# 1275468127/Medical-SAM2

Measured on AMD Instinct MI355X. Metric: slices/sec @1024^2 (Hiera-S), higher is better.
Workload: dtype bf16; 1 GPU; configs[1]: sam2_hiera_s 2D (train_2d SAM2 sub-sequence, forward), b=4 x 1024x1024 per GPU, 16-entry memory bank with 4 sampled memories per slice, one click per slice; forward_image -> memory_attention -> prompt encoder -> mask decoder -> memory encoder; hip_graph=True, weights=random name-keyed init

## Files before the change

include/msam2_hip.h:

```cpp
#ifndef MSAM2_HIP_H
#define MSAM2_HIP_H

#include <stddef.h>
#include <stdint.h>

#ifdef __cplusplus
extern "C" {
#endif

const char* msam2_last_error(void);

int msam2_version(void);

int msam2_operand_is_fp16(void);

int msam2_graph_begin(void* stream);

int msam2_graph_end(void* stream, void** graph_exec_out);

int msam2_graph_launch(void* graph_exec, void* stream);

int msam2_graph_destroy(void* graph_exec);

int msam2_event_create(void** ev);

int msam2_event_record(void* ev, void* stream);

int msam2_event_elapsed_ms(void* start, void* stop, float* ms);

int msam2_event_destroy(void* ev);

int msam2_gemm_nt(const void* A, int64_t lda, const void* B, int64_t ldb, const float* bias, const void* residual, int64_t ldr, void* C, int64_t ldc, int out_is_16bit, int64_t M, int64_t N, int64_t K, void* stream);

int msam2_gemm(const void* A, int64_t lda, const void* W, int64_t ldw, const float* bias, const float* colscale, const void* residual, int64_t ldr, int res_is_16bit, int64_t res_mod, void* C, int64_t ldc, int out_is_16bit, int64_t M, int64_t N, int64_t K, int act, void* stream);

int msam2_gemm_tokens(const float* A, int64_t lda, const float* A2, int64_t add_cols, const void* W, int64_t ldw, const float* bias, const float* residual, int64_t ldr, void* C, int64_t ldc, int out_is_16bit, int64_t M, int64_t N, int64_t K, int act, void* stream);

int msam2_gemm_pool2x2(const void* A, int64_t lda, const void* W, int64_t ldw, const float* bias, float* C, int64_t ldc, int64_t B, int64_t H, int64_t Wimg, int64_t N, int64_t K, void* stream);

int msam2_gemm_qkv_pool2x2(const void* A, int64_t lda, const void* W, int64_t ldw, const float* bias, void* QKV, int64_t ldc, void* Q2, int64_t ldq, int64_t B, int64_t H, int64_t Wimg, int64_t N, int64_t K, int64_t q_cols, void* stream);

int msam2_gemm_rope(const void* A, int64_t lda, const void* W, int64_t ldw, const float* bias, void* C, int64_t ldc, int64_t M, int64_t N, int64_t K, const float* rope_cos, const float* rope_sin, int64_t rope_cols, int64_t head_dim, int64_t rows_per_batch, int64_t n_rope, int64_t n_pos, void* stream);

int msam2_gemm_residual_layernorm_supported(int64_t N, int64_t K);

int msam2_gemm_residual_layernorm(const void* A, int64_t lda, const void* W, int64_t ldw, const float* bias, const float* R32, int64_t ldr, float* C32, int64_t ldc, const float* ln_w, const float* ln_b, float eps, void* Y16, int64_t ldy, int64_t M, int64_t N, int64_t K, void* stream);

size_t msam2_attention_workspace_bytes(int64_t Bz, int64_t H, int64_t Lq, int64_t D, int splits);

int msam2_attention_merge(void* o, const int64_t* o_strides, int64_t B, int64_t H, int64_t Lq, int64_t Lk, int64_t D, int splits, void* workspace, size_t workspace_bytes, void* stream);

int msam2_attention_fwd(const void* q, const int64_t* q_strides, const void* k, const int64_t* k_strides, const void* v, const int64_t* v_strides, void* o, const int64_t* o_strides, int64_t B, int64_t H, int64_t Lq, int64_t Lk, int64_t D, float scale, int splits, void* workspace, size_t workspace_bytes, void* stream);

int msam2_attention_fwd_lse(const void* q, const int64_t* q_strides, const void* k, const int64_t* k_strides, const void* v, const int64_t* v_strides, void* o, const int64_t* o_strides, int64_t B, int64_t H, int64_t Lq, int64_t Lk, int64_t D, float scale, int splits, void* workspace, size_t workspace_bytes, float* lse, void* stream);

int msam2_attention_fwd_lse_dropout(const void* q, const int64_t* q_strides, const void* k, const int64_t* k_strides, const void* v, const int64_t* v_strides, void* o, const int64_t* o_strides, int64_t B, int64_t H, int64_t Lq, int64_t Lk, int64_t D, float scale, int splits, void* workspace, size_t workspace_bytes, float* lse, float p, uint64_t seed, uint64_t offset, const void* seed_dev, void* stream);

int msam2_attention_kv64_fwd(const void* q, const int64_t* q_strides, const void* k, const int64_t* k_strides, const void* v, const int64_t* v_strides, void* o, const int64_t* o_strides, int64_t B, int64_t H, int64_t Lq, int64_t Lk, float scale, int splits, void* workspace, size_t workspace_bytes, void* stream);

int msam2_attention_effective_splits(int64_t Lk, int splits);

int msam2_attention_kv64_partial(const void* q, const int64_t* q_strides, const void* k, const int64_t* k_strides, const void* v, const int64_t* v_strides, int64_t B, int64_t H, int64_t Lq, int64_t Lk, float scale, int splits, int split_begin, int split_count, void* workspace, size_t workspace_bytes, void* stream);

int msam2_attention_kv64_dyn_fwd(const void* q, const int64_t* q_strides, const void* k, const int64_t* k_strides, const void* v, const int64_t* v_strides, void* o, const int64_t* o_strides, int64_t B, int64_t H, int64_t Lq, int64_t Lk, const void* key_count_dev, float scale, int splits, void* workspace, size_t workspace_bytes, void* stream);

int msam2_attention_kv64_dyn_partial(const void* q, const int64_t* q_strides, const void* k, const int64_t* k_strides, const void* v, const int64_t* v_strides, int64_t B, int64_t H, int64_t Lq, int64_t Lk, const void* key_count_dev, float scale, int splits, int split_begin, int split_count, void* workspace, size_t workspace_bytes, void* stream);

int msam2_window_attention_fwd(const void* q, int64_t q_token_stride, int64_t q_head_stride, int64_t hq, int64_t wq, int64_t ws_q, const void* k, const void* v, int64_t kv_token_stride, int64_t kv_head_stride, int64_t hk, int64_t wk, int64_t ws_k, const float* kpad, const float* vpad, void* o, int64_t o_token_stride, int64_t o_head_stride, int64_t B, int64_t H, int64_t D, float scale, void* stream);

int msam2_attention_small_fwd(const void* q, int64_t q_bs, int64_t q_ts, const void* k, int64_t k_bs, int64_t k_ts, const void* v, int64_t v_bs, int64_t v_ts, void* o, int64_t o_bs, int64_t o_ts, int64_t B, int64_t H, int64_t Lq, int64_t Lk, int64_t D, float scale, void* stream);

int msam2_window_qkv_attention_supported(int64_t dim, int64_t dim_out, int64_t heads, int64_t ws, int pool, int64_t H, int64_t W);

int msam2_window_qkv_attention_fwd(const void* xn, const void* w, const float* bias, void* o, int64_t B, int64_t H, int64_t W, int64_t dim, int64_t heads, int64_t ws, int pool, float scale, void* stream);

size_t msam2_attention_bwd_workspace_bytes(int64_t B, int64_t H, int64_t Lq, int64_t D);

int msam2_attention_bwd(const void* q, const int64_t* q_strides, const void* k, const int64_t* k_strides, const void* v, const int64_t* v_strides, const void* o, const int64_t* o_strides, const float* lse, const float* d_o, const int64_t* do_strides, float* dq, const int64_t* dq_strides, float* dk, const int64_t* dk_strides, float* dv, const int64_t* dv_strides, void* workspace, size_t workspace_bytes, int64_t B, int64_t H, int64_t Lq, int64_t Lk, int64_t D, float scale, void* stream);

int msam2_attention_bwd_dropout(const void* q, const int64_t* q_strides, const void* k, const int64_t* k_strides, const void* v, const int64_t* v_strides, const void* o, const int64_t* o_strides, const float* lse, const float* d_o, const int64_t* do_strides, float* dq, const int64_t* dq_strides, float* dk, const int64_t* dk_strides, float* dv, const int64_t* dv_strides, void* workspace, size_t workspace_bytes, int64_t B, int64_t H, int64_t Lq, int64_t Lk, int64_t D, float scale, float p, uint64_t seed, uint64_t offset, const void* seed_dev, void* stream);

int msam2_layernorm(const void* x, int in_is_16bit, int64_t ldx, const float* weight, const float* bias, void* y, int out_is_16bit, int64_t ldy, int64_t rows, int64_t C, float eps, int act, void* stream);

int msam2_layernorm_dual(const float* x, int64_t ldx, const float* weight, const float* bias, float* y, int64_t ldy, void* y16, int64_t ldy16, int64_t rows, int64_t C, float eps, void* stream);

int msam2_add_cast(const void* a, int a_is_16bit, int64_t a_s0, int64_t a_s1, const void* b, int b_is_16bit, int64_t b_s0, int64_t b_s1, float alpha, void* out, int out_is_16bit, int64_t D0, int64_t D1, int64_t C, void* stream);

int msam2_maxpool2x2(const void* x, int in_is_16bit, int64_t ldx, void* y, int out_is_16bit, int64_t ldy, int64_t B, int64_t H, int64_t W, int64_t C, void* stream);

int msam2_upsample2x_add(void* y, const void* top, int64_t B, int64_t H, int64_t W, int64_t C, void* stream);

int msam2_rope_table(float* cos_out, float* sin_out, int64_t side, int64_t D, float theta, void* stream);

int msam2_rope_inplace(void* x, int64_t batch_stride, int64_t ld, int64_t B, int64_t L, int64_t n_rope, int64_t n_pos, int64_t D, const float* cos_t, const float* sin_t, void* stream);

int msam2_bilinear_upsample(const float* x, float* y, int64_t planes, int64_t h, int64_t w, int64_t H, int64_t W, void* stream);

int msam2_sine_pos_2d(float* out, int64_t h, int64_t w, int64_t C, float temperature, void* stream);

int msam2_fourier_pe_grid(float* out, const float* gauss, int64_t h, int64_t w, int64_t C, void* stream);

int msam2_hiera_pos_embed(float* out, const float* pos_embed, const float* pos_embed_window, int64_t C, int64_t bh, int64_t bw, int64_t h, int64_t w, int64_t window, void* stream);

int msam2_aa_downsample(const float* x, float* y, int64_t planes, int64_t H, int64_t W, int64_t factor, float in_scale, float in_bias, void* stream);

int msam2_gate_rows(float* x, const float* score, float value, int64_t B, int64_t row_len, void* stream);

int msam2_any_positive(const float* x, float* out, int64_t B, int64_t row_len, void* stream);

int msam2_image_prep(const uint8_t* img_hwc, float* out_chw, int64_t H, int64_t W, int64_t S, const float* mean3, const float* std3, void* stream);

int msam2_non_overlap(const float* masks, float* out, int64_t n_obj, int64_t pixels, void* stream);

int msam2_seg_counts(const float* pred, const float* gt, const float* thresholds, int64_t n_thresholds, int64_t planes, int64_t pixels, int* counts, void* stream);

int msam2_im2col_patch7x7s4(const float* img, void* out, int64_t B, int64_t S, void* stream);

int msam2_patch_embed7x7s4(const float* img, const void* w_perm, const float* bias, const float* pos, float* out, int64_t B, int64_t S, int64_t E, void* stream);

int msam2_im2col3x3s2(const void* x, void* out, int64_t B, int64_t H, int64_t W, int64_t C, int64_t ld, void* stream);

int msam2_conv3x3s2_ln_gelu(const void* x, int in_is_16bit, const float* weight, const float* bias, const float* ln_w, const float* ln_b, void* y, int64_t B, int64_t H, int64_t W, int64_t Cin, int64_t Cout, int mask_mode, float mask_scale, float mask_bias, void* stream);

int msam2_dwconv7x7_ln(const float* x, const float* weight_tap_major, const float* bias, const float* ln_w, const float* ln_b, void* y, int64_t B, int64_t H, int64_t W, int64_t C, void* stream);

int msam2_convt2x2_shuffle(const void* gemm_out, const float* bias, const void* skip, const float* ln_w, const float* ln_b, void* y, int64_t B, int64_t h, int64_t w, int64_t C, void* stream);

int msam2_convt2x2_shuffle_f32skip(const void* gemm_out, const float* bias, const float* skip, const float* ln_w, const float* ln_b, void* y, int64_t B, int64_t h, int64_t w, int64_t C, void* stream);

int msam2_convt2x2_shuffle_shared(const void* gemm_out, const float* bias, const void* skip, int skip_is_16bit, const float* ln_w, const float* ln_b, void* y, int64_t B, int64_t h, int64_t w, int64_t C, int64_t skip_batch_stride, void* stream);

int msam2_hyper_masks(const float* hyper, const void* upscaled, float* masks, int64_t n, int64_t K, int64_t P, int64_t C, void* stream);

int msam2_prompt_points(const float* xy, const int* labels, const float* gauss, const float* point_emb, const float* not_a_point, float* out, int64_t n_points, int64_t C, float image_size, void* stream);

int msam2_prompt_points_padded(const float* xy, const int* labels, const float* gauss, const float* point_emb, const float* not_a_point, float* out, int64_t n_sets, int64_t P, int64_t n_pad, int64_t C, float image_size, void* stream);

int msam2_select_mask(const float* masks, const float* ious, const float* obj_scores, float* low_res, int* sel, float* iou_sel, int64_t n, int64_t P, int multimask, int dynamic_stability, float delta, float thresh, void* stream);

int msam2_gather_rows(const float* x, const int* sel, float* y, int64_t n, int64_t T, int64_t C, int64_t offset, void* stream);

int msam2_obj_ptr_mix(float* ptr, const float* obj_scores, const float* no_obj_ptr, int64_t n, int64_t C, void* stream);

int msam2_space_to_depth(const void* x, int in_is_16bit, void* out, int64_t B, int64_t H, int64_t W, int64_t C, int64_t k, int64_t ld, void* stream);

int msam2_token_mlp3(const float* hs, int64_t hs_batch_stride, int64_t hs_token_stride, const int* token_index, const void* w1, const float* b1, const void* w2, const float* b2, const void* w3, const float* b3, const int* out_dim, const int* sigmoid_flag, float* out, int64_t G, int64_t B, int64_t C, void* stream);

int msam2_token_mlp3_packed(const float* hs, int64_t hs_batch_stride, int64_t hs_token_stride, const int* token_index, const void* w1, const float* b1, const void* w2, const float* b2, const void* w3, const float* b3, const int* out_dim, const int* sigmoid_flag, float* out, const int* out_offset, const int* out_stride, int64_t G, int64_t B, int64_t C, void* stream);

int msam2_conv3x3s2_mfma_ln_gelu_supported(int64_t cin, int64_t cout);

int msam2_conv3x3s2_mfma_ln_gelu(const void* x, const void* w_packed, int64_t ldw, const float* bias, const float* ln_w, const float* ln_b, float eps, void* y, int64_t ldy, int64_t B, int64_t H, int64_t W, int64_t cin, int64_t cout, void* stream);

size_t msam2_cc_workspace_bytes(int64_t N, int64_t H, int64_t W);

int msam2_cc_label(const uint8_t* img, int32_t* labels, int32_t* counts, int64_t N, int64_t H, int64_t W, void* workspace, size_t workspace_bytes, void* stream);

size_t msam2_fill_holes_workspace_bytes(int64_t N, int64_t H, int64_t W);

int msam2_fill_components(float* mask, int64_t N, int64_t H, int64_t W, int max_area, float threshold, int above, float fill_value, void* workspace, size_t workspace_bytes, void* stream);

int msam2_fill_holes(float* mask, int64_t N, int64_t H, int64_t W, int max_area, void* workspace, size_t workspace_bytes, void* stream);

int msam2_transpose16(const void* in, int64_t ldi, void* out, int64_t ldo, int64_t rows, int64_t cols, void* stream);

int msam2_gemm_tt(const void* A, int64_t lda, const void* B, int64_t ldb, float* C, int64_t ldc, float* a_colsum, int64_t M, int64_t N, int64_t K, void* stream);

int msam2_gemm_tt_acc(const void* A, int64_t lda, const void* B, int64_t ldb, float* C, int64_t ldc, float* a_colsum, int64_t M, int64_t N, int64_t K, void* stream);

int msam2_colsum(const void* x, int x_is_16bit, int64_t ldx, float* out, int64_t rows, int64_t cols, void* stream);

int msam2_act_bwd(const void* pre, int pre_is_16bit, const void* dy, int dy_is_16bit, void* out, int64_t n, int act, void* stream);

int msam2_layernorm_bwd(const float* x, int64_t ldx, const void* dy, int dy_is_16bit, int64_t ldd, const float* gamma, float* dx, int64_t ldo, float* dgamma, float* dbeta, int64_t rows, int64_t C, float eps, const float* add, int64_t ld_add, void* stream);

int msam2_softmax_rows(const float* s, int64_t ld_s, void* p, int64_t ld_p, int64_t rows, int64_t cols, float scale, void* stream);

int msam2_softmax_bwd_rows(const void* p, int64_t ld_p, const float* dp, int64_t ld_dp, void* ds, int64_t ld_ds, int64_t rows, int64_t cols, float scale, void* stream);

int msam2_convt2x2_gather(const void* gemm_out, const float* bias, const void* skip, float* z, int64_t B, int64_t h, int64_t w, int64_t C, void* stream);

int msam2_convt2x2_scatter_grad(const void* dz, int dz_is_16bit, void* dg, int64_t B, int64_t h, int64_t w, int64_t C, void* stream);

int msam2_dwconv7x7(const float* x, const float* w_tap_major, const float* bias, float* y, int64_t B, int64_t H, int64_t W, int64_t C, int flip, void* stream);

int msam2_dwconv7x7_wgrad(const float* x, const float* dy, float* dw_tap_major, int64_t B, int64_t H, int64_t W, int64_t C, void* stream);

int msam2_col2im3x3s2(const float* dcols, int64_t ld, float* dx, int64_t B, int64_t H, int64_t W, int64_t C, void* stream);

int msam2_bilinear_upsample_bwd(const float* dy, float* dx, int64_t planes, int64_t h, int64_t w, int64_t H, int64_t W, void* stream);

int msam2_bce_logits(const float* logits, const float* target, float* dlogits, float* loss, int64_t n, float pos_weight, void* stream);

int msam2_adam_step(float* param, const float* grad, float* exp_avg, float* exp_avg_sq, int64_t n, float lr, float beta1, float beta2, float eps, int64_t step, void* stream);

int msam2_adam_step_multi(void* const* params, const void* const* grads, void* const* exp_avg, void* const* exp_avg_sq, const int64_t* numel, int64_t count, float lr, float beta1, float beta2, float eps, int64_t step, float grad_scale, float weight_decay, void* step_counter, void* skipped_counter, void* stream);

int msam2_attention_small_bwd(const void* q, int64_t q_bs, int64_t q_ts, const void* k, int64_t k_bs, int64_t k_ts, const void* v, int64_t v_bs, int64_t v_ts, const float* d_o, float* dq, float* dk, float* dv, int64_t B, int64_t H, int64_t Lq, int64_t Lk, int64_t D, float scale, void* stream);

int msam2_maxpool2x2_bwd(const void* x, int x_is_16bit, int64_t ldx, const float* dy, int64_t lddy, float* dx, int64_t lddx, int64_t B, int64_t H, int64_t W, int64_t C, void* stream);

int msam2_window_move(void* img, int64_t ld_img, void* win, const void* fill, int64_t B, int64_t H, int64_t W, int64_t heads, int64_t D, int64_t ws, int elem_bytes, int to_windows, void* stream);

int msam2_window_unpartition_cvt(void* img16, int64_t ld_img, const float* win, int64_t B, int64_t H, int64_t W, int64_t heads, int64_t D, int64_t ws, void* stream);

int msam2_window_pad_colsum(const float* win, float* out, int64_t B, int64_t H, int64_t W, int64_t heads, int64_t D, int64_t ws, void* stream);

int msam2_sumpool2x2(const float* dy, float* out, int64_t B, int64_t H, int64_t W, int64_t C, void* stream);

size_t msam2_hiera_pos_embed_bwd_workspace_bytes(int64_t C, int64_t bw, int64_t h, int64_t window);

int msam2_hiera_pos_embed_bwd(const float* d_table, float* d_pos_embed, float* d_pos_embed_window, int64_t C, int64_t bh, int64_t bw, int64_t h, int64_t w, int64_t window, void* workspace, size_t workspace_bytes, void* stream);

int msam2_dropout(const void* x, int x_is_16bit, int64_t ldx, const float* residual, int64_t ldr, void* y, int y_is_16bit, int64_t ldy, int64_t rows, int64_t cols, float p, uint64_t seed, uint64_t offset, const void* seed_dev, void* stream);

int msam2_counter_bump(void* counter_u64, void* snapshot_u64, void* stream);

int msam2_mlp_fused_permute_w2(const void* w2, void* w2p, int64_t dim, int64_t hidden, void* stream);

int msam2_ln_mlp_residual_supported(int64_t dim);

int msam2_ln_mlp_residual_fwd(const float* x, int64_t T, int64_t dim, const float* ln_w, const float* ln_b, float eps, const void* w1, const float* b1, const void* w2p, const float* b2, float* out, void* stream);

int msam2_ln_mlp_residual_fwd_dual(const float* x, int64_t T, int64_t dim, const float* ln_w, const float* ln_b, float eps, const void* w1, const float* b1, const void* w2p, const float* b2, float* out, void* out16, void* stream);

int msam2_proj_ln_mlp_residual_supported(int64_t dim);

int msam2_mlp_fused_permute_w1(const void* w1, void* w1p, int64_t hidden, int64_t dim, void* stream);

int msam2_proj_ln_mlp_residual_fwd(const void* o, const void* wp, const float* bp, const float* res, int64_t T, int64_t dim, const float* ln_w, const float* ln_b, float eps, const void* w1p, const float* b1, const void* w2p, const float* b2, float* out, void* out16, const float* nln_w, const float* nln_b, float neps, void* xn16, void* stream);

size_t msam2_mask_stats_workspace_bytes(int64_t M);

int msam2_mask_stats(const float* logits, int64_t M, int64_t lh, int64_t lw, int64_t h, int64_t w, float thr, float thr_hi, float thr_lo, int* counts, int* boxes, void* workspace, size_t workspace_bytes, void* stream);

int msam2_mask_rle_runs(const float* logits, int64_t M, int64_t lh, int64_t lw, int64_t h, int64_t w, int64_t x0, int64_t y0, int64_t H, int64_t W, float thr, int* runs, void* stream);

int msam2_mask_rle(const float* logits, int64_t M, int64_t lh, int64_t lw, int64_t h, int64_t w, int64_t x0, int64_t y0, int64_t H, int64_t W, float thr, const int64_t* offsets, int* counts, void* stream);

size_t msam2_box_nms_workspace_bytes(int64_t K);

int msam2_box_nms(const float* boxes, const float* scores, int64_t K, float iou_thr, int64_t* keep, int* n_keep, void* workspace, size_t workspace_bytes, void* stream);

int msam2_bank_dots_chain(int64_t K, int vec);

size_t msam2_bank_dots_workspace_bytes(int64_t R, int64_t Cn);

int msam2_bank_dots(const float* x, const int64_t* x_strides, int64_t R, const float* ya, const int64_t* ya_strides, int64_t rows_a, const float* yb, const int64_t* yb_strides, int64_t rows_b, int64_t n_ch, int64_t n_px, float* dots, float* xx, float* yy, void* workspace, size_t workspace_bytes, void* stream);

int msam2_bank_sample(const float* dots, int64_t ld, const float* xx, const float* yy, const int* order, int64_t N, int64_t cap, const float* u, int64_t B, int64_t S, int* indices, float* probs, void* stream);

int msam2_bank_gather(const float* feats, const float* pos, const int* order, const int* indices, int64_t B, int64_t S, int64_t HW, int64_t C, int64_t N, int64_t cap, float* memory, float* memory_pos, void* stream);

int msam2_bank_decide(float* gram, float* iou_bank, int* order, int64_t N, int64_t cap, const float* dots, const float* iou_pred, int64_t B, int64_t M, int fill, int* accept, int* slot_cand, float* iou_out, void* stream);

int msam2_bank_commit(const int* slot_cand, int64_t cap, const float* feats, const int64_t* feats_strides, const float* pos, const int64_t* pos_strides, int64_t C, const float* embed, const int64_t* embed_strides, int64_t Ce, int64_t HW, int64_t B, float* feats_store, float* pos_store, float* embed_store, void* stream);

int msam2_label_slices(const float* logits, const uint8_t* ids, int64_t T, int64_t n, int64_t lh, int64_t lw, int64_t H, int64_t W, float label_thr, const float* thresholds, int64_t K, const uint8_t* gt, int exclusive, uint8_t* labels, int* counts, void* stream);

int msam2_label_stats(const uint8_t* labels, const uint8_t* ids, int64_t D, int64_t H, int64_t W, int64_t n, int* stats, int* rows, void* stream);

int msam2_label_pick(const uint8_t* labels, const uint8_t* ids, const int* stats, const int* rows, const int* k, const uint32_t* u, int64_t D, int64_t H, int64_t W, int64_t n, int* xy, void* stream);

size_t msam2_label_components_workspace_bytes(int64_t D, int64_t H, int64_t W);

int msam2_label_components(const uint8_t* labels, int64_t D, int64_t H, int64_t W, int connectivity, int32_t* comp, int32_t* size, void* workspace, size_t workspace_bytes, void* stream);

size_t msam2_label_clean_workspace_bytes(int64_t n);

int msam2_label_clean(const uint8_t* labels, const int32_t* comp, const int32_t* size, const uint8_t* ids, int64_t n, const int32_t* min_voxels, uint32_t largest_mask, uint8_t* out, int32_t* info, void* workspace, size_t workspace_bytes, int64_t D, int64_t H, int64_t W, void* stream);

int msam2_label_overlap(const uint8_t* pred, const uint8_t* gt, const uint8_t* ids, int64_t D, int64_t H, int64_t W, int64_t n, int32_t* counts, void* stream);

size_t msam2_label_fill_holes_workspace_bytes(int64_t D, int64_t H, int64_t W, const int32_t* boxes, int64_t n, int connectivity, int in_place, int all_at_once);

int msam2_label_fill_holes(const uint8_t* labels, int64_t D, int64_t H, int64_t W, const uint8_t* ids, const int32_t* boxes, int64_t n, int connectivity, const int32_t* max_voxels, int claim, uint8_t* out, int32_t* info, void* workspace, size_t workspace_bytes, void* stream);

size_t msam2_label_edt_workspace_bytes(int64_t bd, int64_t bh, int64_t bw);

int msam2_label_edt(const uint8_t* labels, int64_t D, int64_t H, int64_t W, int value, int features, const int32_t* box, double sz, double sy, double sx, double* d2, void* workspace, size_t workspace_bytes, void* stream);

size_t msam2_label_surface_distances_workspace_bytes(const int32_t* boxes, int64_t n);

int msam2_label_surface_distances(const uint8_t* pred, const uint8_t* gt, int64_t D, int64_t H, int64_t W, const uint8_t* ids, const int32_t* boxes, const int64_t* seg_offsets, const int32_t* capacity, int64_t n, double sz, double sy, double sx, double* dist, int64_t dist_len, int32_t* counts, void* workspace, size_t workspace_bytes, void* stream);

size_t msam2_label_morph_workspace_bytes(int64_t D, int64_t H, int64_t W, const int32_t* boxes, int64_t n, int op, const double* r2, double sz, double sy, double sx, int in_place, int all_at_once);

int msam2_label_morph(const uint8_t* labels, int64_t D, int64_t H, int64_t W, const uint8_t* values, const int32_t* boxes, int64_t n, int op, const double* r2, double sz, double sy, double sx, int claim, uint8_t* out, int32_t* info, void* workspace, size_t workspace_bytes, void* stream);

size_t msam2_label_error_clicks_workspace_bytes(int64_t D, int64_t H, int64_t W, int64_t n, int mode);

int msam2_label_error_clicks(const uint8_t* pred, const uint8_t* gt, const uint8_t* ids, const int* k, const uint32_t* u, int64_t D, int64_t H, int64_t W, int64_t n, int mode, int* clicks, void* workspace, size_t workspace_bytes, void* stream);

size_t msam2_volume_prep_workspace_bytes(int64_t T, int64_t H0, int64_t W0, int64_t S);

int msam2_volume_prep(const void* src, int src_type, int64_t T, int64_t Cin, int64_t H0, int64_t W0, int64_t S, const double* windows, const int* kx, const int* bx, int64_t ksize_x, const int* ky, const int* by, int64_t ksize_y, const float* mean3, const float* std3, uint8_t* grey_out, float* out, void* workspace, size_t workspace_bytes, void* stream);

int msam2_label_resize(const void* src, int src_type, int64_t T, int64_t H0, int64_t W0, int64_t S, const int* ymap, const int* xmap, const uint32_t* keep8, uint8_t* out, void* stream);

#ifdef __cplusplus
}
#endif
#endif
```

medical-sam2_amd/_lib.py:

```python
from __future__ import annotations

import ctypes
import os
import subprocess

_HERE = os.path.dirname(os.path.abspath(__file__))
LIB_PATH = os.environ.get("MSAM2_LIB_PATH") or os.path.join(_HERE, "libmsam2_hip.so")

c_p = ctypes.c_void_p
c_i = ctypes.c_int
c_l = ctypes.c_int64
c_f = ctypes.c_float
c_z = ctypes.c_size_t
c_d = ctypes.c_double

SIGNATURES = {
    "msam2_version": (c_i, []),
    "msam2_last_error": (ctypes.c_char_p, []),
    "msam2_operand_is_fp16": (c_i, []),
    "msam2_gemm": (c_i, [c_p, c_l, c_p, c_l, c_p, c_p, c_p, c_l, c_i, c_l, c_p, c_l, c_i, c_l, c_l, c_l, c_i, c_p]),
    "msam2_gemm_pool2x2": (c_i, [c_p, c_l, c_p, c_l, c_p, c_p, c_l, c_l, c_l, c_l, c_l, c_l, c_p]),
    "msam2_gemm_qkv_pool2x2": (c_i, [c_p, c_l, c_p, c_l, c_p, c_p, c_l, c_p, c_l, c_l, c_l, c_l, c_l, c_l, c_l, c_p]),
    "msam2_gemm_tokens": (c_i, [c_p, c_l, c_p, c_l, c_p, c_l, c_p, c_p, c_l, c_p, c_l, c_i, c_l, c_l, c_l, c_i, c_p]),
    "msam2_gemm_rope": (c_i, [c_p, c_l, c_p, c_l, c_p, c_p, c_l, c_l, c_l, c_l, c_p, c_p, c_l, c_l, c_l, c_l, c_l, c_p]),
    "msam2_gemm_residual_layernorm_supported": (c_i, [c_l, c_l]),
    "msam2_gemm_residual_layernorm": (c_i, [c_p, c_l, c_p, c_l, c_p, c_p, c_l, c_p, c_l, c_p, c_p, c_f, c_p, c_l, c_l, c_l, c_l, c_p]),
    "msam2_ln_mlp_residual_supported": (c_i, [c_l]),
    "msam2_mlp_fused_permute_w2": (c_i, [c_p, c_p, c_l, c_l, c_p]),
    "msam2_ln_mlp_residual_fwd": (c_i, [c_p, c_l, c_l, c_p, c_p, c_f, c_p, c_p, c_p, c_p, c_p, c_p]),
    "msam2_ln_mlp_residual_fwd_dual": (c_i, [c_p, c_l, c_l, c_p, c_p, c_f, c_p, c_p, c_p, c_p, c_p, c_p, c_p]),
    "msam2_proj_ln_mlp_residual_supported": (c_i, [c_l]),
    "msam2_mlp_fused_permute_w1": (c_i, [c_p, c_p, c_l, c_l, c_p]),
    "msam2_proj_ln_mlp_residual_fwd": (c_i, [c_p, c_p, c_p, c_p, c_l, c_l, c_p, c_p, c_f, c_p, c_p, c_p, c_p, c_p, c_p, c_p, c_p, c_f, c_p, c_p]),
    "msam2_layernorm": (c_i, [c_p, c_i, c_l, c_p, c_p, c_p, c_i, c_l, c_l, c_l, c_f, c_i, c_p]),
    "msam2_layernorm_dual": (c_i, [c_p, c_l, c_p, c_p, c_p, c_l, c_p, c_l, c_l, c_l, c_f, c_p]),
    "msam2_attention_workspace_bytes": (c_z, [c_l, c_l, c_l, c_l, c_i]),
    "msam2_attention_fwd": (c_i, [c_p, c_p, c_p, c_p, c_p, c_p, c_p, c_p, c_l, c_l, c_l, c_l, c_l, c_f, c_i, c_p, c_z, c_p]),
    "msam2_attention_fwd_lse": (c_i, [c_p, c_p, c_p, c_p, c_p, c_p, c_p, c_p, c_l, c_l, c_l, c_l, c_l, c_f, c_i, c_p, c_z, c_p, c_p]),
    "msam2_attention_fwd_lse_dropout": (c_i, [c_p, c_p, c_p, c_p, c_p, c_p, c_p, c_p, c_l, c_l, c_l, c_l, c_l, c_f, c_i, c_p, c_z, c_p, c_f,
                                              ctypes.c_uint64, ctypes.c_uint64, c_p, c_p]),
    "msam2_attention_kv64_fwd": (c_i, [c_p, c_p, c_p, c_p, c_p, c_p, c_p, c_p, c_l, c_l, c_l, c_l, c_f, c_i, c_p, c_z, c_p]),
    "msam2_attention_kv64_partial": (c_i, [c_p, c_p, c_p, c_p, c_p, c_p, c_l, c_l, c_l, c_l, c_f, c_i, c_i, c_i, c_p, c_z, c_p]),
    "msam2_attention_kv64_dyn_fwd": (c_i, [c_p, c_p, c_p, c_p, c_p, c_p, c_p, c_p, c_l, c_l, c_l, c_l, c_p, c_f, c_i, c_p, c_z, c_p]),
    "msam2_attention_kv64_dyn_partial": (c_i, [c_p, c_p, c_p, c_p, c_p, c_p, c_l, c_l, c_l, c_l, c_p, c_f, c_i, c_i, c_i, c_p, c_z, c_p]),
    "msam2_attention_effective_splits": (c_i, [c_l, c_i]),
    "msam2_attention_merge": (c_i, [c_p, c_p, c_l, c_l, c_l, c_l, c_l, c_i, c_p, c_z, c_p]),
    "msam2_window_attention_fwd": (c_i, [c_p, c_l, c_l, c_l, c_l, c_l, c_p, c_p, c_l, c_l, c_l, c_l, c_l, c_p, c_p, c_p, c_l, c_l,
                                         c_l, c_l, c_l, c_f, c_p]),
    "msam2_window_qkv_attention_supported": (c_i, [c_l, c_l, c_l, c_l, c_i, c_l, c_l]),
    "msam2_window_qkv_attention_fwd": (c_i, [c_p, c_p, c_p, c_p, c_l, c_l, c_l, c_l, c_l, c_l, c_i, c_f, c_p]),
    "msam2_attention_small_fwd": (c_i, [c_p, c_l, c_l, c_p, c_l, c_l, c_p, c_l, c_l, c_p, c_l, c_l, c_l, c_l, c_l, c_l, c_l, c_f,
                                        c_p]),
    "msam2_add_cast": (c_i, [c_p, c_i, c_l, c_l, c_p, c_i, c_l, c_l, c_f, c_p, c_i, c_l, c_l, c_l, c_p]),
    "msam2_maxpool2x2": (c_i, [c_p, c_i, c_l, c_p, c_i, c_l, c_l, c_l, c_l, c_l, c_p]),
    "msam2_upsample2x_add": (c_i, [c_p, c_p, c_l, c_l, c_l, c_l, c_p]),
    "msam2_rope_table": (c_i, [c_p, c_p, c_l, c_l, c_f, c_p]),
    "msam2_rope_inplace": (c_i, [c_p, c_l, c_l, c_l, c_l, c_l, c_l, c_l, c_p, c_p, c_p]),
    "msam2_bilinear_upsample": (c_i, [c_p, c_p, c_l, c_l, c_l, c_l, c_l, c_p]),
    "msam2_sine_pos_2d": (c_i, [c_p, c_l, c_l, c_l, c_f, c_p]),
    "msam2_fourier_pe_grid": (c_i, [c_p, c_p, c_l, c_l, c_l, c_p]),
    "msam2_hiera_pos_embed": (c_i, [c_p, c_p, c_p, c_l, c_l, c_l, c_l, c_l, c_l, c_p]),
    "msam2_im2col_patch7x7s4": (c_i, [c_p, c_p, c_l, c_l, c_p]),
    "msam2_patch_embed7x7s4": (c_i, [c_p, c_p, c_p, c_p, c_p, c_l, c_l, c_l, c_p]),
    "msam2_im2col3x3s2": (c_i, [c_p, c_p, c_l, c_l, c_l, c_l, c_l, c_p]),
    "msam2_conv3x3s2_ln_gelu": (c_i, [c_p, c_i, c_p, c_p, c_p, c_p, c_p, c_l, c_l, c_l, c_l, c_l, c_i, c_f, c_f, c_p]),
    "msam2_conv3x3s2_mfma_ln_gelu_supported": (c_i, [c_l, c_l]),
    "msam2_conv3x3s2_mfma_ln_gelu": (c_i, [c_p, c_p, c_l, c_p, c_p, c_p, c_f, c_p, c_l, c_l, c_l, c_l, c_l, c_l, c_p]),
    "msam2_dwconv7x7_ln": (c_i, [c_p, c_p, c_p, c_p, c_p, c_p, c_l, c_l, c_l, c_l, c_p]),
    "msam2_convt2x2_shuffle": (c_i, [c_p, c_p, c_p, c_p, c_p, c_p, c_l, c_l, c_l, c_l, c_p]),
    "msam2_convt2x2_shuffle_f32skip": (c_i, [c_p, c_p, c_p, c_p, c_p, c_p, c_l, c_l, c_l, c_l, c_p]),
    "msam2_space_to_depth": (c_i, [c_p, c_i, c_p, c_l, c_l, c_l, c_l, c_l, c_l, c_p]),
    "msam2_aa_downsample": (c_i, [c_p, c_p, c_l, c_l, c_l, c_l, c_f, c_f, c_p]),
    "msam2_gate_rows": (c_i, [c_p, c_p, c_f, c_l, c_l, c_p]),
    "msam2_any_positive": (c_i, [c_p, c_p, c_l, c_l, c_p]),
    "msam2_transpose16": (c_i, [c_p, c_l, c_p, c_l, c_l, c_l, c_p]),
    "msam2_colsum": (c_i, [c_p, c_i, c_l, c_p, c_l, c_l, c_p]),
    "msam2_act_bwd": (c_i, [c_p, c_i, c_p, c_i, c_p, c_l, c_i, c_p]),
    "msam2_layernorm_bwd": (c_i, [c_p, c_l, c_p, c_i, c_l, c_p, c_p, c_l, c_p, c_p, c_l, c_l, c_f, c_p, c_l, c_p]),
    "msam2_softmax_rows": (c_i, [c_p, c_l, c_p, c_l, c_l, c_l, c_f, c_p]),
    "msam2_softmax_bwd_rows": (c_i, [c_p, c_l, c_p, c_l, c_p, c_l, c_l, c_l, c_f, c_p]),
    "msam2_convt2x2_gather": (c_i, [c_p, c_p, c_p, c_p, c_l, c_l, c_l, c_l, c_p]),
    "msam2_convt2x2_scatter_grad": (c_i, [c_p, c_i, c_p, c_l, c_l, c_l, c_l, c_p]),
    "msam2_bce_logits": (c_i, [c_p, c_p, c_p, c_p, c_l, c_f, c_p]),
    "msam2_attention_bwd_workspace_bytes": (c_z, [c_l, c_l, c_l, c_l]),
    "msam2_attention_bwd": (c_i, [c_p, c_p, c_p, c_p, c_p, c_p, c_p, c_p, c_p, c_p, c_p, c_p, c_p, c_p, c_p, c_p, c_p, c_p, c_z,
                                  c_l, c_l, c_l, c_l, c_l, c_f, c_p]),
    "msam2_attention_bwd_dropout": (c_i, [c_p, c_p, c_p, c_p, c_p, c_p, c_p, c_p, c_p, c_p, c_p, c_p, c_p, c_p, c_p, c_p, c_p, c_p, c_z,
                                          c_l, c_l, c_l, c_l, c_l, c_f, c_f, ctypes.c_uint64, ctypes.c_uint64, c_p, c_p]),
    "msam2_dwconv7x7": (c_i, [c_p, c_p, c_p, c_p, c_l, c_l, c_l, c_l, c_i, c_p]),
    "msam2_dwconv7x7_wgrad": (c_i, [c_p, c_p, c_p, c_l, c_l, c_l, c_l, c_p]),
    "msam2_col2im3x3s2": (c_i, [c_p, c_l, c_p, c_l, c_l, c_l, c_l, c_p]),
    "msam2_gemm_nt": (c_i, [c_p, c_l, c_p, c_l, c_p, c_p, c_l, c_p, c_l, c_i, c_l, c_l, c_l, c_p]),
    "msam2_gemm_tt": (c_i, [c_p, c_l, c_p, c_l, c_p, c_l, c_p, c_l, c_l, c_l, c_p]),
    "msam2_window_unpartition_cvt": (c_i, [c_p, c_l, c_p, c_l, c_l, c_l, c_l, c_l, c_l, c_p]),
    "msam2_window_pad_colsum": (c_i, [c_p, c_p, c_l, c_l, c_l, c_l, c_l, c_l, c_p]),
    "msam2_gemm_tt_acc": (c_i, [c_p, c_l, c_p, c_l, c_p, c_l, c_p, c_l, c_l, c_l, c_p]),
    "msam2_bilinear_upsample_bwd": (c_i, [c_p, c_p, c_l, c_l, c_l, c_l, c_l, c_p]),
    "msam2_maxpool2x2_bwd": (c_i, [c_p, c_i, c_l, c_p, c_l, c_p, c_l, c_l, c_l, c_l, c_l, c_p]),
    "msam2_window_move": (c_i, [c_p, c_l, c_p, c_p, c_l, c_l, c_l, c_l, c_l, c_l, c_i, c_i, c_p]),
    "msam2_sumpool2x2": (c_i, [c_p, c_p, c_l, c_l, c_l, c_l, c_p]),
    "msam2_hiera_pos_embed_bwd": (c_i, [c_p, c_p, c_p, c_l, c_l, c_l, c_l, c_l, c_l, c_p, c_z, c_p]),
    "msam2_hiera_pos_embed_bwd_workspace_bytes": (c_z, [c_l, c_l, c_l, c_l]),
    "msam2_dropout": (c_i, [c_p, c_i, c_l, c_p, c_l, c_p, c_i, c_l, c_l, c_l, c_f, ctypes.c_uint64, ctypes.c_uint64, c_p, c_p]),
    "msam2_counter_bump": (c_i, [c_p, c_p, c_p]),
    "msam2_adam_step": (c_i, [c_p, c_p, c_p, c_p, c_l, c_f, c_f, c_f, c_f, c_l, c_p]),
    "msam2_adam_step_multi": (c_i, [c_p, c_p, c_p, c_p, c_p, c_l, c_f, c_f, c_f, c_f, c_l, c_f, c_f, c_p, c_p, c_p]),
    "msam2_attention_small_bwd": (c_i, [c_p, c_l, c_l, c_p, c_l, c_l, c_p, c_l, c_l, c_p, c_p, c_p, c_p, c_l, c_l, c_l, c_l, c_l, c_f, c_p]),
    "msam2_seg_counts": (c_i, [c_p, c_p, c_p, c_l, c_l, c_l, c_p, c_p]),
    "msam2_non_overlap": (c_i, [c_p, c_p, c_l, c_l, c_p]),
    "msam2_token_mlp3": (c_i, [c_p, c_l, c_l, c_p, c_p, c_p, c_p, c_p, c_p, c_p, c_p, c_p, c_p, c_l, c_l, c_l, c_p]),
    "msam2_hyper_masks": (c_i, [c_p, c_p, c_p, c_l, c_l, c_l, c_l, c_p]),
    "msam2_prompt_points": (c_i, [c_p, c_p, c_p, c_p, c_p, c_p, c_l, c_l, c_f, c_p]),
    "msam2_prompt_points_padded": (c_i, [c_p, c_p, c_p, c_p, c_p, c_p, c_l, c_l, c_l, c_l, c_f, c_p]),
    "msam2_token_mlp3_packed": (c_i, [c_p, c_l, c_l, c_p, c_p, c_p, c_p, c_p, c_p, c_p, c_p, c_p, c_p, c_p, c_p, c_l, c_l, c_l, c_p]),
    "msam2_select_mask": (c_i, [c_p, c_p, c_p, c_p, c_p, c_p, c_l, c_l, c_i, c_i, c_f, c_f, c_p]),
    "msam2_gather_rows": (c_i, [c_p, c_p, c_p, c_l, c_l, c_l, c_l, c_p]),
    "msam2_obj_ptr_mix": (c_i, [c_p, c_p, c_p, c_l, c_l, c_p]),
    "msam2_convt2x2_shuffle_shared": (c_i, [c_p, c_p, c_p, c_i, c_p, c_p, c_p, c_l, c_l, c_l, c_l, c_l, c_p]),
    "msam2_mask_stats_workspace_bytes": (c_z, [c_l]),
    "msam2_mask_stats": (c_i, [c_p, c_l, c_l, c_l, c_l, c_l, c_f, c_f, c_f, c_p, c_p, c_p, c_z, c_p]),
    "msam2_mask_rle_runs": (c_i, [c_p, c_l, c_l, c_l, c_l, c_l, c_l, c_l, c_l, c_l, c_f, c_p, c_p]),
    "msam2_mask_rle": (c_i, [c_p, c_l, c_l, c_l, c_l, c_l, c_l, c_l, c_l, c_l, c_f, c_p, c_p, c_p]),
    "msam2_box_nms_workspace_bytes": (c_z, [c_l]),
    "msam2_box_nms": (c_i, [c_p, c_p, c_l, c_f, c_p, c_p, c_p, c_z, c_p]),
    "msam2_bank_dots_chain": (c_i, [c_l, c_i]),
    "msam2_bank_dots_workspace_bytes": (c_z, [c_l, c_l]),
    "msam2_bank_dots": (c_i, [c_p, c_p, c_l, c_p, c_p, c_l, c_p, c_p, c_l, c_l, c_l, c_p, c_p, c_p, c_p, c_z, c_p]),
    "msam2_bank_sample": (c_i, [c_p, c_l, c_p, c_p, c_p, c_l, c_l, c_p, c_l, c_l, c_p, c_p, c_p]),
    "msam2_bank_gather": (c_i, [c_p, c_p, c_p, c_p, c_l, c_l, c_l, c_l, c_l, c_l, c_p, c_p, c_p]),
    "msam2_bank_decide": (c_i, [c_p, c_p, c_p, c_l, c_l, c_p, c_p, c_l, c_l, c_i, c_p, c_p, c_p, c_p]),
    "msam2_bank_commit": (c_i, [c_p, c_l, c_p, c_p, c_p, c_p, c_l, c_p, c_p, c_l, c_l, c_l, c_p, c_p, c_p, c_p]),
    "msam2_label_slices": (c_i, [c_p, c_p, c_l, c_l, c_l, c_l, c_l, c_l, c_f, c_p, c_l, c_p, c_i, c_p, c_p, c_p]),
    "msam2_label_stats": (c_i, [c_p, c_p, c_l, c_l, c_l, c_l, c_p, c_p, c_p]),
    "msam2_label_pick": (c_i, [c_p, c_p, c_p, c_p, c_p, c_p, c_l, c_l, c_l, c_l, c_p, c_p]),
    "msam2_label_components_workspace_bytes": (c_z, [c_l, c_l, c_l]),
    "msam2_label_components": (c_i, [c_p, c_l, c_l, c_l, c_i, c_p, c_p, c_p, c_z, c_p]),
    "msam2_label_clean_workspace_bytes": (c_z, [c_l]),
    "msam2_label_clean": (c_i, [c_p, c_p, c_p, c_p, c_l, c_p, ctypes.c_uint32, c_p, c_p, c_p, c_z, c_l, c_l, c_l, c_p]),
    "msam2_label_overlap": (c_i, [c_p, c_p, c_p, c_l, c_l, c_l, c_l, c_p, c_p]),
    "msam2_label_fill_holes_workspace_bytes": (c_z, [c_l, c_l, c_l, c_p, c_l, c_i, c_i, c_i]),
    "msam2_label_fill_holes": (c_i, [c_p, c_l, c_l, c_l, c_p, c_p, c_l, c_i, c_p, c_i, c_p, c_p, c_p, c_z, c_p]),
    "msam2_label_edt_workspace_bytes": (c_z, [c_l, c_l, c_l]),
    "msam2_label_edt": (c_i, [c_p, c_l, c_l, c_l, c_i, c_i, c_p, c_d, c_d, c_d, c_p, c_p, c_z, c_p]),
    "msam2_label_surface_distances_workspace_bytes": (c_z, [c_p, c_l]),
    "msam2_label_surface_distances": (c_i, [c_p, c_p, c_l, c_l, c_l, c_p, c_p, c_p, c_p, c_l, c_d, c_d, c_d, c_p, c_l, c_p, c_p, c_z, c_p]),
    "msam2_label_morph_workspace_bytes": (c_z, [c_l, c_l, c_l, c_p, c_l, c_i, c_p, c_d, c_d, c_d, c_i, c_i]),
    "msam2_label_morph": (c_i, [c_p, c_l, c_l, c_l, c_p, c_p, c_l, c_i, c_p, c_d, c_d, c_d, c_i, c_p, c_p, c_p, c_z, c_p]),
    "msam2_label_error_clicks_workspace_bytes": (c_z, [c_l, c_l, c_l, c_l, c_i]),
    "msam2_label_error_clicks": (c_i, [c_p, c_p, c_p, c_p, c_p, c_l, c_l, c_l, c_l, c_i, c_p, c_p, c_z, c_p]),
    "msam2_volume_prep_workspace_bytes": (c_z, [c_l, c_l, c_l, c_l]),
    "msam2_volume_prep": (c_i, [c_p, c_i, c_l, c_l, c_l, c_l, c_l, ctypes.POINTER(c_d), c_p, c_p, c_l, c_p, c_p, c_l, ctypes.POINTER(c_f),
                                ctypes.POINTER(c_f), c_p, c_p, c_p, c_z, c_p]),
    "msam2_label_resize": (c_i, [c_p, c_i, c_l, c_l, c_l, c_l, c_p, c_p, ctypes.POINTER(ctypes.c_uint32), c_p, c_p]),
    "msam2_cc_workspace_bytes": (c_z, [c_l, c_l, c_l]),
    "msam2_cc_label": (c_i, [c_p, c_p, c_p, c_l, c_l, c_l, c_p, c_z, c_p]),
    "msam2_fill_holes_workspace_bytes": (c_z, [c_l, c_l, c_l]),
    "msam2_fill_holes": (c_i, [c_p, c_l, c_l, c_l, c_i, c_p, c_z, c_p]),
    "msam2_fill_components": (c_i, [c_p, c_l, c_l, c_l, c_i, c_f, c_i, c_f, c_p, c_z, c_p]),
    "msam2_image_prep": (c_i, [c_p, c_p, c_l, c_l, c_l, ctypes.POINTER(c_f), ctypes.POINTER(c_f), c_p]),
    "msam2_graph_begin": (c_i, [c_p]),
    "msam2_graph_end": (c_i, [c_p, ctypes.POINTER(c_p)]),
    "msam2_graph_launch": (c_i, [c_p, c_p]),
    "msam2_graph_destroy": (c_i, [c_p]),
    "msam2_event_create": (c_i, [ctypes.POINTER(c_p)]),
    "msam2_event_record": (c_i, [c_p, c_p]),
    "msam2_event_elapsed_ms": (c_i, [c_p, c_p, ctypes.POINTER(c_f)]),
    "msam2_event_destroy": (c_i, [c_p]),
}


def build(force: bool = False) -> str:
    if force and os.path.exists(LIB_PATH):
        os.remove(LIB_PATH)
    subprocess.check_call(["make", "-s", "-C", os.path.join(_HERE, "csrc")])
    return LIB_PATH


_lib = None


def lib() -> ctypes.CDLL:
    global _lib
    if _lib is None:
        if not os.path.exists(LIB_PATH):
            raise RuntimeError(
                f"{LIB_PATH} is missing: the MI355X HIP library is the only compute path of this package. "
                "Build it with `python -c 'import __graft_entry__ as g; g.build()'` (or `make -C medical-sam2_amd/csrc`).")
        L = ctypes.CDLL(LIB_PATH)
        for name, (res, args) in SIGNATURES.items():
            fn = getattr(L, name)
            fn.restype = res
            fn.argtypes = args
        _lib = L
    return _lib


class Msam2Error(RuntimeError):
    pass


def check(rc: int) -> None:
    if rc != 0:
        raise Msam2Error(lib().msam2_last_error().decode())
```

medical-sam2_amd/csrc/attention.hip:

```cpp
#include "common.h"
#ifdef MSAM2_STAMP
__device__ unsigned long long g_stamp[16];
__device__ unsigned long long g_wgtime[4096][4];
#define STAMP(var)                                                                     \
  do {                                                                                 \
    __builtin_amdgcn_sched_barrier(0);                                                 \
    asm volatile("s_memtime %0\n\ts_waitcnt lgkmcnt(0)" : "=s"(var)::"memory");         \
    __builtin_amdgcn_sched_barrier(0);                                                 \
  } while (0)
#define STAMP_DECL unsigned long long t0_ = 0, t1_ = 0, t2_ = 0, t3_ = 0, t4_ = 0, t5_ = 0, acc_[5] = {0, 0, 0, 0, 0}
#else
#define STAMP(var)
#define STAMP_DECL
#endif
#include <stdlib.h>
#include <type_traits>

#ifndef MSAM2_RESCALE_SLACK
#define MSAM2_RESCALE_SLACK 8.f
#endif

struct AttnParams {
  const op16 *q, *k, *v;
  op16* o;
// ... 1859 lines not shown
  MSAM2_REQUIRE(splits >= 1 && splits <= 64, "attention_kv64: bad split count %d", splits);
  for (int i = 0; i < 3; ++i)
    MSAM2_REQUIRE(q_strides[i] % 8 == 0 && k_strides[i] % 8 == 0 && v_strides[i] % 8 == 0 && (!o || o_strides[i] % 4 == 0),
                  "attention_kv64: strides must keep 16-byte row alignment");
  MSAM2_REQUIRE(Lk * k_strides[2] * 2 < (1ll << 31) && Lk * v_strides[2] * 2 < (1ll << 31), "attention_kv64: key range beyond the 2 GiB buffer window");
  const int eff = attn_effective_splits(Lk, splits);
  if (split_cnt >= 0) {
    MSAM2_REQUIRE(eff == splits && eff > 1, "attention_kv64_partial: pass msam2_attention_effective_splits(Lk, splits) (> 1) as the split count");
    MSAM2_REQUIRE(split_begin >= 0 && split_cnt >= 0 && split_begin + split_cnt <= eff, "attention_kv64_partial: bad split range");
    defer = true;
    if (split_cnt == 0) return MSAM2_OK;
  } else {
    split_begin = 0;
    split_cnt = eff;
  }
  splits = eff;
  MSAM2_REQUIRE(workspace_bytes >= msam2_attention_workspace_bytes(B, H, Lq, 64, splits), "attention_kv64: workspace too small");
  MSAM2_REQUIRE(!defer || splits > 1, "attention_kv64: a deferred merge needs an effective split count > 1");
  MSAM2_REQUIRE(splits == 1 || workspace, "attention_kv64: split-KV needs a workspace");
  AttnParams p = {};
  set_qkvo(p, q, q_strides, k, k_strides, v, v_strides, o, o ? o_strides : nullptr);
  p.B = (int)B; p.H = (int)H; p.Lq = (int)Lq; p.Lk = (int)Lk;
  p.scale_log2 = scale * 1.4426950408889634f;
  set_workspace(p, workspace, splits, B, H, Lq, 64);
  p.split_begin = split_begin;
  p.split_cnt = split_cnt;
  p.lk_dev = lk_dev;
  p.defer_merge = defer ? 1 : 0;
  return launch_attn_kv64(p, (int)B, (hipStream_t)stream);
}

extern "C" int msam2_attention_kv64_fwd(const void* q, const int64_t* q_strides, const void* k, const int64_t* k_strides,
                                        const void* v, const int64_t* v_strides, void* o, const int64_t* o_strides, int64_t B,
                                        int64_t H, int64_t Lq, int64_t Lk, float scale, int splits, void* workspace,
                                        size_t workspace_bytes, void* stream) {
  MSAM2_REQUIRE(o, "attention_kv64: null output");
  return attention_kv64_impl(q, q_strides, k, k_strides, v, v_strides, o, o_strides, B, H, Lq, Lk, scale, splits, 0, -1, workspace, workspace_bytes, stream);
}

extern "C" int msam2_attention_effective_splits(int64_t Lk, int splits) {
  parse_splits(splits);
  return attn_effective_splits(Lk, splits);
}

extern "C" int msam2_attention_kv64_partial(const void* q, const int64_t* q_strides, const void* k, const int64_t* k_strides,
                                            const void* v, const int64_t* v_strides, int64_t B, int64_t H, int64_t Lq, int64_t Lk,
                                            float scale, int splits, int split_begin, int split_count, void* workspace,
                                            size_t workspace_bytes, void* stream) {
  MSAM2_REQUIRE(split_count >= 0, "attention_kv64_partial: negative split count");
  return attention_kv64_impl(q, q_strides, k, k_strides, v, v_strides, nullptr, nullptr, B, H, Lq, Lk, scale, splits, split_begin, split_count,
                             workspace, workspace_bytes, stream);
}

extern "C" int msam2_attention_kv64_dyn_fwd(const void* q, const int64_t* q_strides, const void* k, const int64_t* k_strides,
                                            const void* v, const int64_t* v_strides, void* o, const int64_t* o_strides, int64_t B,
                                            int64_t H, int64_t Lq, int64_t Lk, const void* key_count_dev, float scale, int splits,
                                            void* workspace, size_t workspace_bytes, void* stream) {
  MSAM2_REQUIRE(o && key_count_dev, "attention_kv64_dyn: null output / key count");
  return attention_kv64_impl(q, q_strides, k, k_strides, v, v_strides, o, o_strides, B, H, Lq, Lk, scale, splits, 0, -1, workspace, workspace_bytes,
                             stream, (const int*)key_count_dev);
}

extern "C" int msam2_attention_kv64_dyn_partial(const void* q, const int64_t* q_strides, const void* k, const int64_t* k_strides,
                                                const void* v, const int64_t* v_strides, int64_t B, int64_t H, int64_t Lq, int64_t Lk,
                                                const void* key_count_dev, float scale, int splits, int split_begin, int split_count,
                                                void* workspace, size_t workspace_bytes, void* stream) {
  MSAM2_REQUIRE(split_count >= 0 && key_count_dev, "attention_kv64_dyn_partial: negative split count / null key count");
  return attention_kv64_impl(q, q_strides, k, k_strides, v, v_strides, nullptr, nullptr, B, H, Lq, Lk, scale, splits, split_begin, split_count,
                             workspace, workspace_bytes, stream, (const int*)key_count_dev);
}

extern "C" int msam2_window_attention_fwd(const void* q, int64_t q_token_stride, int64_t q_head_stride, int64_t hq, int64_t wq,
                                          int64_t ws_q, const void* k, const void* v, int64_t kv_token_stride,
                                          int64_t kv_head_stride, int64_t hk, int64_t wk, int64_t ws_k, const float* kpad,
                                          const float* vpad, void* o, int64_t o_token_stride, int64_t o_head_stride, int64_t B,
                                          int64_t H, int64_t D, float scale, void* stream) {
  MSAM2_REQUIRE(q && k && v && o && kpad && vpad, "window_attention: null tensor");
  MSAM2_REQUIRE(D == 96 || D == 64 || D == 128, "window_attention: head dim %lld not built", (long long)D);
  MSAM2_REQUIRE(ws_q > 0 && ws_k > 0 && hq > 0 && wq > 0 && hk > 0 && wk > 0, "window_attention: bad geometry");
  const int nwy = (int)((hk + ws_k - 1) / ws_k), nwx = (int)((wk + ws_k - 1) / ws_k);
  MSAM2_REQUIRE((hq + ws_q - 1) / ws_q == nwy && (wq + ws_q - 1) / ws_q == nwx, "window_attention: q/kv window grids differ");
  MSAM2_REQUIRE(q_token_stride % 8 == 0 && kv_token_stride % 8 == 0 && q_head_stride % 8 == 0 && kv_head_stride % 8 == 0 &&
                    o_token_stride % 4 == 0 && o_head_stride % 4 == 0, "window_attention: strides must keep 16-byte alignment");
  AttnParams p = {};
  p.q = (const op16*)q; p.k = (const op16*)k; p.v = (const op16*)v; p.o = (op16*)o;
  p.q_bs = hq * wq * q_token_stride; p.q_hs = q_head_stride; p.q_ts = q_token_stride;
  p.k_bs = hk * wk * kv_token_stride; p.k_hs = kv_head_stride; p.k_ts = kv_token_stride;
  p.v_bs = p.k_bs; p.v_hs = kv_head_stride; p.v_ts = kv_token_stride;
  p.o_bs = hq * wq * o_token_stride; p.o_hs = o_head_stride; p.o_ts = o_token_stride;
  p.B = (int)B; p.H = (int)H; p.Lq = (int)(ws_q * ws_q); p.Lk = (int)(ws_k * ws_k);
  p.scale_log2 = scale * 1.4426950408889634f;
  p.win = 1; p.ws_q = (int)ws_q; p.ws_k = (int)ws_k; p.hq = (int)hq; p.wq = (int)wq; p.hk = (int)hk; p.wk = (int)wk;
  p.nwy = nwy; p.nwx = nwx; p.kpad = kpad; p.vpad = vpad; p.splits = 1;
  hipStream_t s = (hipStream_t)stream;
  const int Bz = (int)B * nwy * nwx;
  switch (D) {
    case 96:
      if (attn_win_applies(p)) return launch_attn_win(p, Bz, s);
      return attn_tinywin_applies(p) ? launch_attn_tinywin(p, Bz, s) : dispatch_nw<96, true>(p, Bz, s);
    case 64: return dispatch_nw<64, true>(p, Bz, s);
    default: return dispatch_nw<128, true>(p, Bz, s);
  }
}

template <int D>
__global__ void attn_small_kernel(const op16* q, const op16* k, const op16* v, op16* o, int64_t q_bs, int64_t q_ts,
                                  int64_t k_bs, int64_t k_ts, int64_t v_bs, int64_t v_ts, int64_t o_bs, int64_t o_ts, int B,
                                  int H, int Lq, int Lk, float scale_log2) {
  const int64_t gw = ((int64_t)blockIdx.x * blockDim.x + threadIdx.x) >> 6;
  const int lane = threadIdx.x & 63;
  if (gw >= (int64_t)B * H * Lq) return;
  const int qi = gw % Lq;
  const int head = (gw / Lq) % H;
  const int b = gw / ((int64_t)Lq * H);
  float qv[D];
  const op16* qp = q + b * q_bs + (int64_t)qi * q_ts + head * D;
#pragma unroll
  for (int d = 0; d < D; d += 8) {
    const op16x8 t = *reinterpret_cast<const op16x8*>(qp + d);
#pragma unroll
    for (int e = 0; e < 8; ++e) qv[d + e] = op2f(t[e]) * scale_log2;
  }
  float m = -INFINITY, l = 0.f, acc[D];
#pragma unroll
  for (int d = 0; d < D; ++d) acc[d] = 0.f;
  for (int key = lane; key < Lk; key += 64) {
    const op16* kp = k + b * k_bs + (int64_t)key * k_ts + head * D;
    const op16* vp = v + b * v_bs + (int64_t)key * v_ts + head * D;
    float s = 0.f;
    float vv[D];
#pragma unroll
    for (int d = 0; d < D; d += 8) {
      const op16x8 t = *reinterpret_cast<const op16x8*>(kp + d);
      const op16x8 u = *reinterpret_cast<const op16x8*>(vp + d);
#pragma unroll
      for (int e = 0; e < 8; ++e) {
        s += qv[d + e] * op2f(t[e]);
        vv[d + e] = op2f(u[e]);
      }
    }
    const float mn = fmaxf(m, s);
    const float a = (m == -INFINITY) ? 0.f : __builtin_amdgcn_exp2f(m - mn);
    const float pe = __builtin_amdgcn_exp2f(s - mn);
    l = l * a + pe;
#pragma unroll
    for (int d = 0; d < D; ++d) acc[d] = acc[d] * a + pe * vv[d];
    m = mn;
  }
#pragma unroll
  for (int off = 32; off > 0; off >>= 1) {
    const float m2 = __shfl_xor(m, off, 64), l2 = __shfl_xor(l, off, 64);
    const float mn = fmaxf(m, m2);
    const float a1 = (m == -INFINITY) ? 0.f : __builtin_amdgcn_exp2f(m - mn);
    const float a2 = (m2 == -INFINITY) ? 0.f : __builtin_amdgcn_exp2f(m2 - mn);
    l = l * a1 + l2 * a2;
#pragma unroll
    for (int d = 0; d < D; ++d) acc[d] = acc[d] * a1 + __shfl_xor(acc[d], off, 64) * a2;
    m = mn;
  }
  if (lane == 0) {
    op16* op = o + b * o_bs + (int64_t)qi * o_ts + head * D;
    const float inv = 1.f / l;
#pragma unroll
    for (int d = 0; d < D; ++d) op[d] = f2op(acc[d] * inv);
  }
}

template <int D>
__global__ __launch_bounds__(1024) void attn_fewq_kernel(const op16* q, const op16* k, const op16* v, op16* o, int64_t q_bs, int64_t q_ts,
                                                         int64_t k_bs, int64_t k_ts, int64_t v_bs, int64_t v_ts, int64_t o_bs, int64_t o_ts,
                                                         int B, int H, int Lq, int Lk, float scale_log2) {
  __shared__ float part[16][D + 2];
  const int gw = blockIdx.x;
  const int lane = threadIdx.x & 63, wave = threadIdx.x >> 6;
  const int qi = gw % Lq;
  const int head = (gw / Lq) % H;
  const int b = gw / (Lq * H);
  float qv[D];
  const op16* qp = q + b * q_bs + (int64_t)qi * q_ts + head * D;
#pragma unroll
  for (int d = 0; d < D; d += 8) {
    const op16x8 t = *reinterpret_cast<const op16x8*>(qp + d);
#pragma unroll
    for (int e = 0; e < 8; ++e) qv[d + e] = op2f(t[e]) * scale_log2;
  }
  float m = -INFINITY, l = 0.f, acc[D];
#pragma unroll
  for (int d = 0; d < D; ++d) acc[d] = 0.f;
  const op16* kb = k + b * k_bs + head * D;
  const op16* vb = v + b * v_bs + head * D;
#pragma unroll 4
  for (int key = threadIdx.x; key < Lk; key += 1024) {
    const op16* kp = kb + (int64_t)key * k_ts;
    const op16* vp = vb + (int64_t)key * v_ts;
    float s = 0.f;
    float vv[D];
#pragma unroll
    for (int d = 0; d < D; d += 8) {
      const op16x8 t = *reinterpret_cast<const op16x8*>(kp + d);
      const op16x8 u = *reinterpret_cast<const op16x8*>(vp + d);
#pragma unroll
      for (int e = 0; e < 8; ++e) {
        s += qv[d + e] * op2f(t[e]);
        vv[d + e] = op2f(u[e]);
      }
    }
    const float mn = fmaxf(m, s);
    const float a = (m == -INFINITY) ? 0.f : __builtin_amdgcn_exp2f(m - mn);
    const float pe = __builtin_amdgcn_exp2f(s - mn);
    l = l * a + pe;
#pragma unroll
    for (int d = 0; d < D; ++d) acc[d] = acc[d] * a + pe * vv[d];
    m = mn;
  }
  auto merge = [&](int off) {
    const float m2 = __shfl_xor(m, off, 64), l2 = __shfl_xor(l, off, 64);
    const float mn = fmaxf(m, m2);
    const float a1 = (m == -INFINITY) ? 0.f : __builtin_amdgcn_exp2f(m - mn);
    const float a2 = (m2 == -INFINITY) ? 0.f : __builtin_amdgcn_exp2f(m2 - mn);
    l = l * a1 + l2 * a2;
#pragma unroll
    for (int d = 0; d < D; ++d) acc[d] = acc[d] * a1 + __shfl_xor(acc[d], off, 64) * a2;
    m = mn;
  };
#pragma unroll
  for (int off = 32; off > 0; off >>= 1) merge(off);
  if (lane == 0) {
    part[wave][0] = m;
    part[wave][1] = l;
#pragma unroll
    for (int d = 0; d < D; ++d) part[wave][2 + d] = acc[d];
  }
  __syncthreads();
  if (wave == 0) {
    const int w = lane & 15;
    m = part[w][0];
    l = part[w][1];
#pragma unroll
    for (int d = 0; d < D; ++d) acc[d] = part[w][2 + d];
#pragma unroll
    for (int off = 8; off > 0; off >>= 1) merge(off);
    if (lane == 0) {
      op16* op = o + b * o_bs + (int64_t)qi * o_ts + head * D;
      const float inv = 1.f / l;
#pragma unroll
      for (int d = 0; d < D; ++d) op[d] = f2op(acc[d] * inv);
    }
  }
}

template <int D>
__global__ void attn_fewkeys_kernel(const op16* q, const op16* k, const op16* v, op16* o, int64_t q_bs, int64_t q_ts, int64_t k_bs,
                                    int64_t k_ts, int64_t v_bs, int64_t v_ts, int64_t o_bs, int64_t o_ts, int B, int H, int Lq, int Lk,
                                    float scale_log2) {
  const int64_t gid = (int64_t)blockIdx.x * blockDim.x + threadIdx.x;
  if (gid >= (int64_t)B * H * Lq) return;
  const int head = gid % H;
  const int qi = (gid / H) % Lq;
  const int b = gid / ((int64_t)H * Lq);
  float qv[D];
  const op16* qp = q + b * q_bs + (int64_t)qi * q_ts + head * D;
#pragma unroll
  for (int d = 0; d < D; d += 8) {
    const op16x8 t = *reinterpret_cast<const op16x8*>(qp + d);
#pragma unroll
    for (int e = 0; e < 8; ++e) qv[d + e] = op2f(t[e]) * scale_log2;
  }
  float m = -INFINITY, l = 0.f, acc[D];
#pragma unroll
  for (int d = 0; d < D; ++d) acc[d] = 0.f;
  for (int key = 0; key < Lk; ++key) {
    const op16* kp = k + b * k_bs + (int64_t)key * k_ts + head * D;
    const op16* vp = v + b * v_bs + (int64_t)key * v_ts + head * D;
    float sc = 0.f;
#pragma unroll
    for (int d = 0; d < D; d += 8) {
      const op16x8 t = *reinterpret_cast<const op16x8*>(kp + d);
#pragma unroll
      for (int e = 0; e < 8; ++e) sc += qv[d + e] * op2f(t[e]);
    }
    const float mn = fmaxf(m, sc);
    const float al = (m == -INFINITY) ? 0.f : __builtin_amdgcn_exp2f(m - mn);
    const float pe = __builtin_amdgcn_exp2f(sc - mn);
    l = l * al + pe;
#pragma unroll
    for (int d = 0; d < D; d += 8) {
      const op16x8 u = *reinterpret_cast<const op16x8*>(vp + d);
#pragma unroll
      for (int e = 0; e < 8; ++e) acc[d + e] = acc[d + e] * al + pe * op2f(u[e]);
    }
    m = mn;
  }
  const float inv = 1.f / l;
  op16* op = o + b * o_bs + (int64_t)qi * o_ts + head * D;
#pragma unroll
  for (int d = 0; d < D; d += 8) {
    op16x8 w;
#pragma unroll
    for (int e = 0; e < 8; ++e) w[e] = f2op(acc[d + e] * inv);
    *reinterpret_cast<op16x8*>(op + d) = w;
  }
}

__global__ __launch_bounds__(1024) void attn_fewq16_kernel(const op16* __restrict__ q, const op16* __restrict__ k, const op16* __restrict__ v,
                                                           op16* __restrict__ o, int64_t q_bs, int64_t q_ts, int64_t k_bs, int64_t k_ts,
                                                           int64_t v_bs, int64_t v_ts, int64_t o_bs, int64_t o_ts, int H, int Lq, int Lk,
                                                           float scale_log2) {
  constexpr int D = 16, RB = 64, BK = 32, NW = 16, MAXS = 8;
  __shared__ __attribute__((aligned(16))) unsigned char vt[NW][BK * RB];
  __shared__ float part[NW][32][18];
  const int tid = threadIdx.x, wave = tid >> 6, lane = tid & 63;
  const int r = lane & 31, h = lane >> 5;
  const int b = blockIdx.x / H, head = blockIdx.x - b * H;
  const op16* qb = q + (int64_t)b * q_bs + head * D;
  const op16* kb = k + (int64_t)b * k_bs + head * D;
  const op16* vb = v + (int64_t)b * v_bs + head * D;
  {
    unsigned char* t = vt[wave];
    *reinterpret_cast<uint4*>(t + (lane >> 1) * RB + 32 + (lane & 1) * 16) = make_uint4(0, 0, 0, 0);
  }
  op16x8 qf;
  {
    uint4 t = make_uint4(0, 0, 0, 0);
    const uint4 ld = *reinterpret_cast<const uint4*>(qb + (int64_t)min(r, Lq - 1) * q_ts + h * 8);
    if (r < Lq) t = ld;
    qf = __builtin_bit_cast(op16x8, t);
  }
  const int per = (Lk + NW - 1) / NW;
  const int key_lo = wave * per, key_hi = min(Lk, key_lo + per);
  const int nsteps = max(0, (key_hi - key_lo + BK - 1) / BK);
  uint4 kfr[MAXS], vch[MAXS];
#pragma unroll
  for (int st = 0; st < MAXS; ++st) {
    const int kk = min(key_lo + st * BK + r, Lk - 1);
    kfr[st] = *reinterpret_cast<const uint4*>(kb + (int64_t)kk * k_ts + h * 8);
    const int kv = min(key_lo + st * BK + (lane >> 1), Lk - 1);
    vch[st] = *reinterpret_cast<const uint4*>(vb + (int64_t)kv * v_ts + (lane & 1) * 8);
  }
  f32x16 oacc;
#pragma unroll
  for (int e = 0; e < 16; ++e) oacc[e] = 0.f;
  float m_run = -INFINITY, l_run = 0.f;
  const int li = lane & 15;
  const int v_off = (4 * h + (li >> 2)) * RB + (16 * ((lane >> 4) & 1) + 4 * (li & 3)) * 2;
#pragma unroll
  for (int st = 0; st < MAXS; ++st) {
    if (st < nsteps) {
      const int key0 = key_lo + st * BK;
      *reinterpret_cast<uint4*>(vt[wave] + (lane >> 1) * RB + (lane & 1) * 16) = vch[st];
      f32x16 sacc;
#pragma unroll
      for (int e = 0; e < 16; ++e) sacc[e] = 0.f;
      sacc = MSAM2_MFMA_32x32x16(__builtin_bit_cast(op16x8, kfr[st]), qf, sacc, 0, 0, 0);
      float mx = -INFINITY;
#pragma unroll
      for (int e = 0; e < 16; ++e) {
        if (key0 + s_frag_key(e, h) >= key_hi) sacc[e] = -INFINITY;
        mx = fmaxf(mx, sacc[e]);
      }
      mx = half_max(mx) * scale_log2;
      const float m_new = fmaxf(m_run, mx);
      const float alpha = (m_run == -INFINITY) ? 0.f : __builtin_amdgcn_exp2f(m_run - m_new);
      l_run *= alpha;
#pragma unroll
      for (int e = 0; e < 16; ++e) oacc[e] *= alpha;
      m_run = m_new;
      float psum = 0.f;
      op16x8 pf[2];
#pragma unroll
      for (int e = 0; e < 16; ++e) {
        const float pe = __builtin_amdgcn_exp2f(__builtin_fmaf(sacc[e], scale_log2, -m_run));
        psum += pe;
        pf[e >> 3][e & 7] = f2op_fast(pe);
      }
      l_run += psum;
      asm volatile("s_waitcnt lgkmcnt(0)" ::: "memory");
#pragma unroll
      for (int s2 = 0; s2 < 2; ++s2)
        oacc = MSAM2_MFMA_32x32x16(lds_read_tr16_pair(vt[wave] + (16 * s2) * RB + v_off, 8 * RB), pf[s2], oacc, 0, 0, 0);
      asm volatile("s_waitcnt lgkmcnt(0)" ::: "memory");
    }
  }
  const float l_tot = half_sum(l_run);
  {
    float* pp = part[wave][r];
    if (h == 0) { pp[0] = m_run; pp[1] = l_tot; }
#pragma unroll
    for (int e = 0; e < 8; ++e) pp[2 + (e & 3) + 8 * (e >> 2) + 4 * h] = oacc[e];
  }
  __syncthreads();
  if (tid < Lq * D) {
    const int qi = tid / D, d = tid - qi * D;
    float M = -INFINITY;
#pragma unroll
    for (int w = 0; w < NW; ++w) M = fmaxf(M, part[w][qi][0]);
    float L = 0.f, acc = 0.f;
#pragma unroll
    for (int w = 0; w < NW; ++w) {
      const float mw = part[w][qi][0];
      const float wgt = (mw == -INFINITY) ? 0.f : __builtin_amdgcn_exp2f(mw - M);
      L += part[w][qi][1] * wgt;
      acc += part[w][qi][2 + d] * wgt;
    }
    o[(int64_t)b * o_bs + (int64_t)qi * o_ts + head * D + d] = f2op(acc / L);
  }
}


extern "C" int msam2_attention_small_fwd(const void* q, int64_t q_bs, int64_t q_ts, const void* k, int64_t k_bs, int64_t k_ts,
                                         const void* v, int64_t v_bs, int64_t v_ts, void* o, int64_t o_bs, int64_t o_ts,
                                         int64_t B, int64_t H, int64_t Lq, int64_t Lk, int64_t D, float scale, void* stream) {
  MSAM2_REQUIRE(q && k && v && o, "attention_small: null tensor");
  MSAM2_REQUIRE(D == 16 || D == 32, "attention_small: head dim %lld not built (16/32)", (long long)D);
  MSAM2_REQUIRE(B > 0 && H > 0 && Lq > 0 && Lk > 0, "attention_small: empty problem");
  MSAM2_REQUIRE(q_ts % 8 == 0 && k_ts % 8 == 0 && v_ts % 8 == 0 && q_bs % 8 == 0 && k_bs % 8 == 0 && v_bs % 8 == 0,
                "attention_small: strides must keep 16-byte alignment");
  const float sl = scale * 1.4426950408889634f;
  hipStream_t s = (hipStream_t)stream;
  if (Lk <= 32 && Lq >= 64 && o_ts % 8 == 0 && o_bs % 8 == 0) {
    dim3 g1(cdiv(B * H * Lq, 256));
    if (D == 16)
      hipLaunchKernelGGL((attn_fewkeys_kernel<16>), g1, dim3(256), 0, s, (const op16*)q, (const op16*)k, (const op16*)v, (op16*)o, q_bs,
                         q_ts, k_bs, k_ts, v_bs, v_ts, o_bs, o_ts, (int)B, (int)H, (int)Lq, (int)Lk, sl);
    else
      hipLaunchKernelGGL((attn_fewkeys_kernel<32>), g1, dim3(256), 0, s, (const op16*)q, (const op16*)k, (const op16*)v, (op16*)o, q_bs,
                         q_ts, k_bs, k_ts, v_bs, v_ts, o_bs, o_ts, (int)B, (int)H, (int)Lq, (int)Lk, sl);
    return msam2_check_launch("attention_small(fewkeys)");
  }
  {
    const char* off = getenv("MSAM2_NO_FEWQ16");
    if (D == 16 && Lq <= 32 && Lk >= 1024 && Lk <= 4096 && !(off && off[0] == '1') && q_ts % 8 == 0 && k_ts % 8 == 0 && v_ts % 8 == 0 &&
        q_bs % 8 == 0 && k_bs % 8 == 0 && v_bs % 8 == 0 && (((uintptr_t)q | (uintptr_t)k | (uintptr_t)v) & 15) == 0) {
      hipLaunchKernelGGL(attn_fewq16_kernel, dim3((unsigned)(B * H)), dim3(1024), 0, s, (const op16*)q, (const op16*)k, (const op16*)v, (op16*)o,
                         q_bs, q_ts, k_bs, k_ts, v_bs, v_ts, o_bs, o_ts, (int)H, (int)Lq, (int)Lk, sl);
      return msam2_check_launch("attention_small(fewq, matrix pipe)");
    }
  }
  if (Lk >= 1024 && B * H * Lq <= 4096) {
    dim3 g2((unsigned)(B * H * Lq));
    if (D == 16)
      hipLaunchKernelGGL((attn_fewq_kernel<16>), g2, dim3(1024), 0, s, (const op16*)q, (const op16*)k, (const op16*)v, (op16*)o, q_bs, q_ts,
                         k_bs, k_ts, v_bs, v_ts, o_bs, o_ts, (int)B, (int)H, (int)Lq, (int)Lk, sl);
    else
      hipLaunchKernelGGL((attn_fewq_kernel<32>), g2, dim3(1024), 0, s, (const op16*)q, (const op16*)k, (const op16*)v, (op16*)o, q_bs, q_ts,
                         k_bs, k_ts, v_bs, v_ts, o_bs, o_ts, (int)B, (int)H, (int)Lq, (int)Lk, sl);
    return msam2_check_launch("attention_small(fewq)");
  }
  const int64_t waves = B * H * Lq;
  dim3 grid(cdiv(waves * 64, 256));
  if (D == 16)
    hipLaunchKernelGGL((attn_small_kernel<16>), grid, dim3(256), 0, s, (const op16*)q, (const op16*)k, (const op16*)v, (op16*)o,
                       q_bs, q_ts, k_bs, k_ts, v_bs, v_ts, o_bs, o_ts, (int)B, (int)H, (int)Lq, (int)Lk, sl);
  else
    hipLaunchKernelGGL((attn_small_kernel<32>), grid, dim3(256), 0, s, (const op16*)q, (const op16*)k, (const op16*)v, (op16*)o,
                       q_bs, q_ts, k_bs, k_ts, v_bs, v_ts, o_bs, o_ts, (int)B, (int)H, (int)Lq, (int)Lk, sl);
  return msam2_check_launch("attention_small");
}
```

medical-sam2_amd/modeling/sam_heads.py:

```python
from __future__ import annotations

from typing import List, Optional, Tuple, Type

import torch
import torch.nn as nn

from .. import ops
from .common import OP16, F32, WeightCache, nchw_view, to_bf16, tokens_of, v_f32, w_bf16
from .encoder import MLP
from .memory import Attention, LayerNorm2d
from .position import PositionEmbeddingRandom


class PromptEncoder(nn.Module):

    def __init__(self, embed_dim: int, image_embedding_size: Tuple[int, int], input_image_size: Tuple[int, int],
                 mask_in_chans: int, activation: Type[nn.Module] = nn.GELU) -> None:
        super().__init__()
        self.embed_dim = embed_dim
        self.input_image_size = input_image_size
        self.image_embedding_size = image_embedding_size
        self.pe_layer = PositionEmbeddingRandom(embed_dim // 2)
        self.num_point_embeddings: int = 4
        self.point_embeddings = nn.ModuleList([nn.Embedding(1, embed_dim) for _ in range(self.num_point_embeddings)])
        self.not_a_point_embed = nn.Embedding(1, embed_dim)
        self.mask_input_size = (4 * image_embedding_size[0], 4 * image_embedding_size[1])
        self.mask_downscaling = nn.Sequential(
            nn.Conv2d(1, mask_in_chans // 4, kernel_size=2, stride=2), LayerNorm2d(mask_in_chans // 4), activation(),
            nn.Conv2d(mask_in_chans // 4, mask_in_chans, kernel_size=2, stride=2), LayerNorm2d(mask_in_chans), activation(),
            nn.Conv2d(mask_in_chans, embed_dim, kernel_size=1))
        self.no_mask_embed = nn.Embedding(1, embed_dim)
        self._wc = WeightCache()

    def dense_pe_tokens(self) -> torch.Tensor:
        g = self.pe_layer.positional_encoding_gaussian_matrix
        return self._wc.get("dense_pe", [g], lambda: self.pe_layer.grid_tokens(self.image_embedding_size))

    def get_dense_pe(self) -> torch.Tensor:
        h, w = self.image_embedding_size
        return nchw_view(self.dense_pe_tokens(), 1, h, w)

    def _points(self, xy: torch.Tensor, labels: torch.Tensor, n_pad: int = 0) -> torch.Tensor:
        assert self.input_image_size[0] == self.input_image_size[1]
        wc = self._wc
        emb = wc.get("pemb", [m.weight for m in self.point_embeddings],
                     lambda: torch.cat([m.weight.detach() for m in self.point_embeddings], 0).float().contiguous())
        return ops.prompt_points(xy.to(F32), labels.to(torch.int32), self.pe_layer.positional_encoding_gaussian_matrix.to(F32), emb,
                                 v_f32(wc, "nap", self.not_a_point_embed.weight), float(self.input_image_size[0]), n_pad=n_pad)

    def _embed_masks_tokens(self, masks: torch.Tensor) -> torch.Tensor:
        n, _, H, W = masks.shape
        wc, md = self._wc, self.mask_downscaling
        f = lambda key, p: v_f32(wc, key, p)

        def patch_w(conv, key):
            def build():
                w = conv.weight.detach().permute(0, 2, 3, 1).reshape(conv.weight.shape[0], -1)
                ld = (w.shape[1] + 7) // 8 * 8
                out = torch.zeros(w.shape[0], ld, dtype=OP16, device=w.device)
                out[:, : w.shape[1]] = w.to(OP16)
                return out
            return wc.get(key, [conv.weight], build)

        h = ops.space_to_depth(masks.to(F32).contiguous().reshape(n * H * W, 1), n, H, W, 2)
        h = ops.gemm(h, patch_w(md[0], "w0"), f("b0", md[0].bias), out_dtype=F32)
        h = ops.layernorm(h, f("lw0", md[1].weight), f("lb0", md[1].bias), md[1].eps, act=ops.ACT_GELU)
        h = ops.space_to_depth(h, n, H // 2, W // 2, 2)
        h = ops.gemm(h, patch_w(md[3], "w1"), f("b1", md[3].bias), out_dtype=F32)
        h = ops.layernorm(h, f("lw1", md[4].weight), f("lb1", md[4].bias), md[4].eps, act=ops.ACT_GELU)
        return ops.gemm(h, w_bf16(wc, "w2", md[6].weight), f("b2", md[6].bias), out_dtype=F32)

    def _get_batch_size(self, points, boxes, masks) -> int:
        if points is not None:
            return points[0].shape[0]
        if boxes is not None:
            return boxes.shape[0]
        if masks is not None:
            return masks.shape[0]
        return 1

    def forward(self, points: Optional[Tuple[torch.Tensor, torch.Tensor]], boxes: Optional[torch.Tensor],
                masks: Optional[torch.Tensor], batch_size=-1) -> Tuple[torch.Tensor, torch.Tensor]:
        bs = self._get_batch_size(points, boxes, masks)
        dev = self.no_mask_embed.weight.device
        xy_parts, lab_parts = [], []
        n_pad = 0
        if points is not None:
            coords, labels = points
            xy_parts.append(coords.to(F32))
            lab_parts.append(labels.to(torch.int32))
            if boxes is None:
                n_pad = 1
        if boxes is not None:
            xy_parts.append(boxes.to(F32).reshape(-1, 2, 2))
            lab_parts.append(torch.tensor([[2, 3]], dtype=torch.int32, device=dev).expand(bs, 2))
        if len(xy_parts) == 1:
            sparse = self._points(xy_parts[0].contiguous(), lab_parts[0].contiguous(), n_pad)
        elif xy_parts:
            sparse = self._points(torch.cat(xy_parts, 1).contiguous(), torch.cat(lab_parts, 1).contiguous())
        else:
            sparse = torch.empty((bs, 0, self.embed_dim), device=dev)
        h, w = self.image_embedding_size
        if masks is not None:
            dense = nchw_view(self._embed_masks_tokens(masks), bs, h, w)
        else:
            dense = self.no_mask_embed.weight.reshape(1, -1, 1, 1).expand(bs, -1, h, w)
        return sparse, dense


def _image_side_projections(wc: WeightCache, key: str, keys_b: torch.Tensor, key_pe: torch.Tensor, L: int, lins, with_pe):
    ws = [l.weight for l in lins]
    W = w_bf16(wc, key + "w", *ws)
    b = v_f32(wc, key + "b", *[l.bias for l in lins])

    def build_pe():
        R = ops.gemm(to_bf16(key_pe.contiguous()), W, None, out_dtype=F32)
        col = 0
        for l, use in zip(lins, with_pe):
            if not use:
                R[:, col: col + l.out_features] = 0.0
            col += l.out_features
        return R
    R = wc.get(key + "pe", ws + [key_pe], build_pe)
    return ops.gemm(keys_b, W, b, residual=R, res_mod=L)


class TwoWayAttentionBlock(nn.Module):

    def __init__(self, embedding_dim: int, num_heads: int, mlp_dim: int = 2048, activation: Type[nn.Module] = nn.ReLU,
                 attention_downsample_rate: int = 2, skip_first_layer_pe: bool = False) -> None:
        super().__init__()
        self.self_attn = Attention(embedding_dim, num_heads)
        self.norm1 = nn.LayerNorm(embedding_dim)
        self.cross_attn_token_to_image = Attention(embedding_dim, num_heads, downsample_rate=attention_downsample_rate)
        self.norm2 = nn.LayerNorm(embedding_dim)
        self.mlp = MLP(embedding_dim, mlp_dim, embedding_dim, num_layers=2, activation=activation)
        self.norm3 = nn.LayerNorm(embedding_dim)
        self.norm4 = nn.LayerNorm(embedding_dim)
        self.cross_attn_image_to_token = Attention(embedding_dim, num_heads, downsample_rate=attention_downsample_rate)
        self.skip_first_layer_pe = skip_first_layer_pe
        self._wc = WeightCache()

    def _ln(self, name, x):
        n = getattr(self, name)
        return ops.layernorm(x, v_f32(self._wc, name + "w", n.weight), v_f32(self._wc, name + "b", n.bias), n.eps, out_dtype=F32)

    def run(self, queries, keys, query_pe, key_pe, B, T, L, keys_b=None):
        C = queries.shape[1]
        q3 = lambda t, n: t.view(B, n, -1)
        sa, ca, ia, wc = self.self_attn, self.cross_attn_token_to_image, self.cross_attn_image_to_token, self._wc
        fused = B * T <= 32 and C % 32 == 0 and sa.internal_dim % 32 == 0 and ia.internal_dim % 32 == 0
        if fused:
            Ci = sa.internal_dim
            qkv = ops.gemm_tokens(queries, w_bf16(wc, "sqkv", sa.q_proj.weight, sa.k_proj.weight, sa.v_proj.weight),
                                  v_f32(wc, "sqkvb", sa.q_proj.bias, sa.k_proj.bias, sa.v_proj.bias),
                                  addend=None if self.skip_first_layer_pe else query_pe, add_cols=2 * Ci).view(B, T, 3 * Ci)
            o = sa.core(qkv[:, :, :Ci], qkv[:, :, Ci:2 * Ci], qkv[:, :, 2 * Ci:])
            queries = sa.out(o, None if self.skip_first_layer_pe else queries)
        elif self.skip_first_layer_pe:
            qb = to_bf16(queries)
            queries = sa.out(sa.core(q3(sa.proj("q", qb), T), q3(sa.proj("k", qb), T), q3(sa.proj("v", qb), T)), None)
        else:
            qb = ops.add_cast(queries.view(1, B * T, C), query_pe.view(1, B * T, C), 1.0, OP16)[0]
            queries = sa.out(sa.core(q3(sa.proj("q", qb), T), q3(sa.proj("k", qb), T), q3(sa.proj("v", to_bf16(queries)), T)), queries)
        queries = self._ln("norm1", queries)
        if keys_b is None:
            keys_b = to_bf16(keys)
        Cc, Ci2 = ca.internal_dim, ia.internal_dim
        kvq = _image_side_projections(wc, "ikvq", keys_b, key_pe, L, [ca.k_proj, ca.v_proj, ia.q_proj], [True, False, True])
        k_img, v_img, q_img = kvq[:, :Cc], kvq[:, Cc:2 * Cc], kvq[:, 2 * Cc:2 * Cc + Ci2]
        if fused:
            qp = ops.gemm_tokens(queries, w_bf16(wc, "cqw", ca.q_proj.weight), v_f32(wc, "cqb", ca.q_proj.bias), addend=query_pe,
                                 add_cols=ca.internal_dim)
        else:
            qp = ca.proj("q", ops.add_cast(queries.view(1, B * T, C), query_pe.view(1, B * T, C), 1.0, OP16)[0])
        o = ca.core(q3(qp, T), q3(k_img, L), q3(v_img, L))
        queries = self._ln("norm2", ca.out(o, queries))
        if fused and self.mlp.num_layers == 2:
            l1, l2 = self.mlp.layers
            hmid = ops.gemm_tokens(queries, w_bf16(wc, "m1w", l1.weight), v_f32(wc, "m1b", l1.bias), act=self.mlp._act_code)
            queries = self._ln("norm3", ops.gemm(hmid, w_bf16(wc, "m2w", l2.weight), v_f32(wc, "m2b", l2.bias), residual=queries, out_dtype=F32))
        else:
            queries = self._ln("norm3", self.mlp.run(to_bf16(queries), residual=queries, out_dtype=F32))
        if fused:
            Cd = ia.internal_dim
            kv = ops.gemm_tokens(queries, w_bf16(wc, "ikv", ia.k_proj.weight, ia.v_proj.weight), v_f32(wc, "ikvb", ia.k_proj.bias, ia.v_proj.bias),
                                 addend=query_pe, add_cols=Cd).view(B, T, 2 * Cd)
            o = ia.core(q3(q_img, L), kv[:, :, :Cd], kv[:, :, Cd:])
        else:
            qb = ops.add_cast(queries.view(1, B * T, C), query_pe.view(1, B * T, C), 1.0, OP16)[0]
            o = ia.core(q3(q_img, L), q3(ia.proj("k", qb), T), q3(ia.proj("v", to_bf16(queries)), T))
        n4 = self.norm4
        keys, keys16 = ops.layernorm_dual(ia.out(o, keys), v_f32(wc, "norm4w", n4.weight), v_f32(wc, "norm4b", n4.bias), n4.eps)
        return queries, keys, keys16

    def forward(self, queries, keys, query_pe, key_pe):
        B, T, C = queries.shape
        L = keys.shape[1]
        assert key_pe.shape[0] == 1 or B == 1, "key_pe is the batch-shared dense position encoding"
        q, k, _ = self.run(queries.to(F32).reshape(B * T, C).contiguous(), keys.to(F32).reshape(B * L, C).contiguous(),
                           query_pe.to(F32).reshape(B * T, C).contiguous(), key_pe.to(F32).reshape(-1, C)[:L].contiguous(), B, T, L)
        return q.view(B, T, C), k.view(B, L, C)


class TwoWayTransformer(nn.Module):

    def __init__(self, depth: int, embedding_dim: int, num_heads: int, mlp_dim: int, activation: Type[nn.Module] = nn.ReLU,
                 attention_downsample_rate: int = 2) -> None:
        super().__init__()
        self.depth, self.embedding_dim, self.num_heads, self.mlp_dim = depth, embedding_dim, num_heads, mlp_dim
        self.layers = nn.ModuleList([
            TwoWayAttentionBlock(embedding_dim=embedding_dim, num_heads=num_heads, mlp_dim=mlp_dim, activation=activation,
                                 attention_downsample_rate=attention_downsample_rate, skip_first_layer_pe=(i == 0))
            for i in range(depth)])
        self.final_attn_token_to_image = Attention(embedding_dim, num_heads, downsample_rate=attention_downsample_rate)
        self.norm_final_attn = nn.LayerNorm(embedding_dim)
        self._wc = WeightCache()

    def run(self, keys, key_pe, tokens, B, T, L):
        C = tokens.shape[1]
        queries, qpe = tokens, tokens
        keys16 = None
        for layer in self.layers:
            queries, keys, keys16 = layer.run(queries, keys, qpe, key_pe, B, T, L, keys16)
        if keys16 is None:
            keys16 = to_bf16(keys)
        self._keys16 = keys16
        fa = self.final_attn_token_to_image
        kv_img = _image_side_projections(self._wc, "fkv", keys16, key_pe, L, [fa.k_proj, fa.v_proj], [True, False])
        Cf = fa.internal_dim
        q3 = lambda t, n: t.view(B, n, -1)
        if B * T <= 32 and fa.internal_dim % 32 == 0:
            qp = ops.gemm_tokens(queries, w_bf16(self._wc, "fqw", fa.q_proj.weight), v_f32(self._wc, "fqb", fa.q_proj.bias), addend=qpe,
                                 add_cols=fa.internal_dim)
        else:
            qp = fa.proj("q", ops.add_cast(queries.view(1, B * T, C), qpe.view(1, B * T, C), 1.0, OP16)[0])
        o = fa.core(q3(qp, T), q3(kv_img[:, :Cf], L), q3(kv_img[:, Cf:], L))
        n = self.norm_final_attn
        queries = ops.layernorm(fa.out(o, queries), v_f32(self._wc, "nw", n.weight), v_f32(self._wc, "nb", n.bias), n.eps, out_dtype=F32)
        return queries, keys

    def forward(self, image_embedding, image_pe, point_embedding):
        B, C, h, w = image_embedding.shape
        T = point_embedding.shape[1]
        keys = tokens_of(image_embedding.to(F32))
        pe = tokens_of(image_pe.to(F32))[: h * w]
        q, k = self.run(keys, pe, point_embedding.to(F32).reshape(B * T, C).contiguous(), B, T, h * w)
        return q.view(B, T, C), k.view(B, h * w, C)


class MaskDecoder(nn.Module):

    def __init__(self, *, transformer_dim: int, transformer: nn.Module, num_multimask_outputs: int = 3,
                 activation: Type[nn.Module] = nn.GELU, iou_head_depth: int = 3, iou_head_hidden_dim: int = 256,
                 use_high_res_features: bool = False, iou_prediction_use_sigmoid=False, dynamic_multimask_via_stability=False,
                 dynamic_multimask_stability_delta=0.05, dynamic_multimask_stability_thresh=0.98, pred_obj_scores: bool = False,
                 pred_obj_scores_mlp: bool = False, use_multimask_token_for_obj_ptr: bool = False) -> None:
        super().__init__()
        assert num_multimask_outputs == 3 and use_high_res_features and pred_obj_scores and pred_obj_scores_mlp, \
            "HIP path implements the SAM2 YAML decoder (3 multimasks, high-res skips, object-score MLP)"
        self.transformer_dim, self.transformer = transformer_dim, transformer
        self.num_multimask_outputs = num_multimask_outputs
        self.iou_token = nn.Embedding(1, transformer_dim)
        self.num_mask_tokens = num_multimask_outputs + 1
        self.mask_tokens = nn.Embedding(self.num_mask_tokens, transformer_dim)
        self.pred_obj_scores = pred_obj_scores
        self.obj_score_token = nn.Embedding(1, transformer_dim)
        self.use_multimask_token_for_obj_ptr = use_multimask_token_for_obj_ptr
        self.output_upscaling = nn.Sequential(
            nn.ConvTranspose2d(transformer_dim, transformer_dim // 4, kernel_size=2, stride=2), LayerNorm2d(transformer_dim // 4),
            activation(), nn.ConvTranspose2d(transformer_dim // 4, transformer_dim // 8, kernel_size=2, stride=2), activation())
        self.use_high_res_features = use_high_res_features
        self.conv_s0 = nn.Conv2d(transformer_dim, transformer_dim // 8, kernel_size=1, stride=1)
        self.conv_s1 = nn.Conv2d(transformer_dim, transformer_dim // 4, kernel_size=1, stride=1)
        self.output_hypernetworks_mlps = nn.ModuleList(
            [MLP(transformer_dim, transformer_dim, transformer_dim // 8, 3) for _ in range(self.num_mask_tokens)])
        self.iou_prediction_head = MLP(transformer_dim, iou_head_hidden_dim, self.num_mask_tokens, iou_head_depth,
                                       sigmoid_output=iou_prediction_use_sigmoid)
        self.pred_obj_score_head = MLP(transformer_dim, transformer_dim, 1, 3)
        self.dynamic_multimask_via_stability = dynamic_multimask_via_stability
        self.dynamic_multimask_stability_delta = dynamic_multimask_stability_delta
        self.dynamic_multimask_stability_thresh = dynamic_multimask_stability_thresh
        self._wc = WeightCache()

    def conv_s(self, which: int, tokens_bf16: torch.Tensor, out_dtype=OP16) -> torch.Tensor:
        c = self.conv_s0 if which == 0 else self.conv_s1
        return ops.gemm(tokens_bf16, w_bf16(self._wc, f"cs{which}w", c.weight), v_f32(self._wc, f"cs{which}b", c.bias), out_dtype=out_dtype)

    def predict_masks_tokens(self, src_tokens: torch.Tensor, pe_tokens: torch.Tensor, sparse: torch.Tensor, feat_s0: torch.Tensor,
                             feat_s1: torch.Tensor, B: int, h: int, w: int, shared_skips: bool = False):
        wc = self._wc
        C = self.transformer_dim
        out_tok = wc.get("otok", [self.obj_score_token.weight, self.iou_token.weight, self.mask_tokens.weight],
                         lambda: torch.cat([self.obj_score_token.weight, self.iou_token.weight, self.mask_tokens.weight], 0).detach().float())
        T = out_tok.shape[0] + sparse.shape[1]
        tokens = torch.cat([out_tok.unsqueeze(0).expand(B, -1, -1), sparse], 1)
        hs, keys = self.transformer.run(src_tokens, pe_tokens, tokens.view(B * T, C), B, T, h * w)
        hs = hs.view(B, T, C)
        up = self.output_upscaling
        dc1_w = wc.get("dc1", [up[0].weight], lambda: up[0].weight.detach().permute(2, 3, 1, 0).reshape(-1, C).to(OP16).contiguous())
        keys16 = getattr(self.transformer, "_keys16", None)
        if keys16 is None or keys16.shape != keys.shape:
            keys16 = to_bf16(keys)
        self.transformer._keys16 = None
        g = ops.gemm(keys16, dc1_w)
        shuffle = ops.convt2x2_shuffle_shared if shared_skips else ops.convt2x2_shuffle
        u = shuffle(g, v_f32(wc, "dc1b", up[0].bias), feat_s1, v_f32(wc, "lnw", up[1].weight), v_f32(wc, "lnb", up[1].bias), B, h, w)
        dc2_w = wc.get("dc2", [up[3].weight], lambda: up[3].weight.detach().permute(2, 3, 1, 0).reshape(-1, C // 4).to(OP16).contiguous())
        g = ops.gemm(u, dc2_w)
        u = shuffle(g, v_f32(wc, "dc2b", up[3].bias), feat_s0, None, None, B, 2 * h, 2 * w)
        heads = list(self.output_hypernetworks_mlps) + [self.iou_prediction_head, self.pred_obj_score_head]
        fusable = C == 256 and self.pred_obj_scores and all(
            m.num_layers == 3 and m._act_code == ops.ACT_RELU and m.layers[0].in_features == C and m.layers[0].out_features == C
            and m.layers[1].out_features == C and m.layers[2].out_features <= C for m in heads)
        if fusable:
            G = len(heads)
            params = [t for m in heads for l in m.layers for t in (l.weight, l.bias)]

            def pack():
                dev = hs.device
                w1 = torch.stack([m.layers[0].weight.detach() for m in heads]).to(OP16).contiguous()
                w2 = torch.stack([m.layers[1].weight.detach() for m in heads]).to(OP16).contiguous()
                w3 = torch.zeros(G, C, C, dtype=OP16, device=dev)
                b3 = torch.zeros(G, C, dtype=F32, device=dev)
                for gi, m in enumerate(heads):
                    n = m.layers[2].out_features
                    w3[gi, :n] = m.layers[2].weight.detach().to(OP16)
                    b3[gi, :n] = m.layers[2].bias.detach().float()
                b1 = torch.stack([m.layers[0].bias.detach() for m in heads]).float().contiguous()
                b2 = torch.stack([m.layers[1].bias.detach() for m in heads]).float().contiguous()
                return w1, b1, w2, b2, w3, b3

            def consts():
                dev = hs.device
                nm_ = self.num_mask_tokens
                return (torch.tensor([2 + i for i in range(nm_)] + [1, 0], dtype=torch.int32, device=dev),
                        torch.tensor([m.layers[2].out_features for m in heads], dtype=torch.int32, device=dev),
                        torch.tensor([int(m.sigmoid_output) for m in heads], dtype=torch.int32, device=dev))
            tok, od, sg = wc.get("heads_const", [], consts)
            w1, b1, w2, b2, w3, b3 = wc.get("heads", params, pack)
            nm = self.num_mask_tokens
            n_hyper, n_iou, n_obj = C // 8, heads[nm].layers[2].out_features, heads[nm + 1].layers[2].out_features

            def layout():
                dev = hs.device
                off = [g * n_hyper for g in range(nm)] + [B * nm * n_hyper, B * nm * n_hyper + B * n_iou]
                ld = [nm * n_hyper] * nm + [n_iou, n_obj]
                return torch.tensor(off, dtype=torch.int32, device=dev), torch.tensor(ld, dtype=torch.int32, device=dev)
            off, ld = wc.get(f"heads_layout{B}", [], layout)
            y = ops.token_mlp3(hs, tok, w1, b1, w2, b2, w3, b3, od, sg, packed=(off, ld, B * (nm * n_hyper + n_iou + n_obj)))
            hyper = y[: B * nm * n_hyper].view(B, nm, n_hyper)
            iou = y[B * nm * n_hyper: B * (nm * n_hyper + n_iou)].view(B, n_iou)
            obj = y[B * (nm * n_hyper + n_iou):].view(B, n_obj)
        else:
            hyper = torch.empty(B, self.num_mask_tokens, C // 8, dtype=F32, device=u.device)
            for i, m in enumerate(self.output_hypernetworks_mlps):
                hyper[:, i] = m.run(to_bf16(hs[:, 2 + i].contiguous()))
            iou = self.iou_prediction_head.run(to_bf16(hs[:, 1].contiguous()))
            obj = self.pred_obj_score_head.run(to_bf16(hs[:, 0].contiguous()))
        masks = ops.hyper_masks(hyper, u, B, 16 * h * w).view(B, self.num_mask_tokens, 4 * h, 4 * w)
        return masks, iou, hs[:, 2:2 + self.num_mask_tokens], obj

    def predict_masks(self, image_embeddings, image_pe, sparse_prompt_embeddings, dense_prompt_embeddings, repeat_image,
                      cell_nums=None, high_res_features=None):
        n_sets = sparse_prompt_embeddings.shape[0]
        from .. import autograd as ag
        shared = (n_sets > 1 and image_embeddings.shape[0] == 1 and high_res_features is not None
                  and all(f.shape[0] == 1 for f in high_res_features) and self.transformer_dim // 8 in (32, 64)
                  and (cell_nums is None or torch.as_tensor(cell_nums).reshape(-1).tolist() == [n_sets]) and not ag.active(self))
        if shared:
            _, C, h, w = image_embeddings.shape
            B = n_sets
            e3 = tokens_of(image_embeddings.to(F32)).view(1, h * w, C).expand(B, h * w, C)
            dense = dense_prompt_embeddings.to(F32).expand(B, C, h, w)
            if dense.stride(2) == 0 and dense.stride(3) == 0:
                d3 = dense[:, :, 0, 0].unsqueeze(1).expand(B, h * w, C)
            else:
                d3 = tokens_of(dense).view(B, h * w, C)
            src = ops.add_cast(e3, d3, 1.0, F32).view(B * h * w, C)
            pe = tokens_of(image_pe.to(F32))[: h * w]
            f0, f1 = high_res_features
            skip = lambda f: tokens_of(f) if (f.dtype == F32 and f.shape[1] in (32, 64)) else to_bf16(tokens_of(f))
            return self.predict_masks_tokens(src, pe, sparse_prompt_embeddings.to(F32), skip(f0), skip(f1), B, h, w, shared_skips=True)
        if image_embeddings.shape[0] != n_sets:
            if cell_nums is not None:
                cn = torch.as_tensor(cell_nums, device=image_embeddings.device).reshape(-1).long()
                if cn.numel() != image_embeddings.shape[0] or int(cn.sum()) != n_sets:
                    raise RuntimeError(f"cell_nums {cn.tolist()} does not split {n_sets} prompt sets over {image_embeddings.shape[0]} images")
                image_embeddings = torch.repeat_interleave(image_embeddings, cn, dim=0)
            elif image_embeddings.shape[0] == 1:
                image_embeddings = image_embeddings.expand(n_sets, -1, -1, -1)
            else:
                raise RuntimeError(f"The size of tensor a ({image_embeddings.shape[0]}) must match the size of tensor b ({n_sets}) at non-singleton dimension 0")
            hr = []
            for f in high_res_features:
                if f.shape[0] == 1:
                    f = f.expand(n_sets, -1, -1, -1)
                elif f.shape[0] != n_sets:
                    raise RuntimeError(f"The size of tensor a ({n_sets}) must match the size of tensor b ({f.shape[0]}) at non-singleton dimension 0")
                hr.append(f)
            high_res_features = hr
        B, C, h, w = image_embeddings.shape
        assert sparse_prompt_embeddings.shape[0] == B, "one prompt set per (repeated) image embedding"
        if ag.active(self):
            src = tokens_of(image_embeddings.to(F32)).view(B, h * w, C) + tokens_of(dense_prompt_embeddings.to(F32).expand(B, C, h, w)).view(B, h * w, C)
            f0, f1 = high_res_features
            return ag.mask_decoder(self, src.reshape(B * h * w, C), tokens_of(image_pe.to(F32))[: h * w].detach(), sparse_prompt_embeddings.to(F32),
                                   tokens_of(f0), tokens_of(f1), B, h, w)
        emb = image_embeddings.to(F32)
        dense = dense_prompt_embeddings.to(F32).expand(B, C, h, w)
        e3 = tokens_of(emb).view(B, h * w, C)
        if dense.stride(2) == 0 and dense.stride(3) == 0:
            d3 = dense[:, :, 0, 0].unsqueeze(1).expand(B, h * w, C)
        else:
            d3 = tokens_of(dense).view(B, h * w, C)
        src = ops.add_cast(e3, d3, 1.0, F32).view(B * h * w, C)
        pe = tokens_of(image_pe.to(F32))[: h * w]
        f0, f1 = high_res_features
        skip = lambda f: tokens_of(f) if (f.dtype == F32 and f.shape[1] in (32, 64)) else to_bf16(tokens_of(f))
        return self.predict_masks_tokens(src, pe, sparse_prompt_embeddings.to(F32), skip(f0), skip(f1), B, h, w)

    def forward(self, image_embeddings, image_pe, sparse_prompt_embeddings, dense_prompt_embeddings, multimask_output: bool,
                repeat_image: bool, cell_nums=None, high_res_features: Optional[List[torch.Tensor]] = None):
        masks, iou_pred, mask_tokens_out, object_score_logits = self.predict_masks(
            image_embeddings, image_pe, sparse_prompt_embeddings, dense_prompt_embeddings, repeat_image, cell_nums, high_res_features)
        if multimask_output:
            masks, iou_pred = masks[:, 1:, :, :], iou_pred[:, 1:]
        elif self.dynamic_multimask_via_stability and not self.training:
            nb = object_score_logits.shape[0]
            obj_pos = self._wc.get(f"ones{nb}", [], lambda: torch.ones(nb, dtype=F32, device=object_score_logits.device))
            low, sel, iou_sel = ops.select_mask(masks.contiguous(), iou_pred.contiguous(), obj_pos, False, True,
                                                self.dynamic_multimask_stability_delta, self.dynamic_multimask_stability_thresh)
            masks, iou_pred = low, iou_sel
        else:
            masks, iou_pred = masks[:, 0:1, :, :], iou_pred[:, 0:1]
        if multimask_output and self.use_multimask_token_for_obj_ptr:
            sam_tokens_out = mask_tokens_out[:, 1:]
        else:
            sam_tokens_out = mask_tokens_out[:, 0:1]
        return masks, iou_pred, sam_tokens_out, object_score_logits
```

medical-sam2_amd/ops.py:

```python
from __future__ import annotations

import ctypes
import math
from typing import Optional, Tuple

import torch

from ._lib import check, lib

OP16 = torch.float16 if lib().msam2_operand_is_fp16() else torch.bfloat16

F32 = torch.float32
ACT_NONE, ACT_GELU, ACT_RELU, ACT_SIGMOID = 0, 1, 2, 3


def _stream() -> int:
    return torch.cuda.current_stream().cuda_stream


def _p(t: Optional[torch.Tensor]):
    return None if t is None else t.data_ptr()


def _is_bf16(t: torch.Tensor) -> int:
    if t.dtype == OP16:
        return 1
    if t.dtype == F32:
        return 0
    raise TypeError(f"expected {OP16} or fp32 tensor, got {t.dtype}")


def _req(cond: bool, msg: str):
    if not cond:
        raise ValueError(msg)


def gemm(a: torch.Tensor, w: torch.Tensor, bias: Optional[torch.Tensor] = None, *, act: int = ACT_NONE,
         colscale: Optional[torch.Tensor] = None, residual: Optional[torch.Tensor] = None, res_mod: int = 0,
         out_dtype: torch.dtype = OP16, out: Optional[torch.Tensor] = None) -> torch.Tensor:
    _req(a.dim() == 2 and w.dim() == 2 and a.shape[1] == w.shape[1], f"gemm shapes {tuple(a.shape)} x {tuple(w.shape)}")
    _req(a.dtype == OP16 and w.dtype == OP16, "gemm operands must be 16-bit (ops.OP16)")
    _req(a.stride(1) == 1 and w.stride(1) == 1, "gemm operands must be K-contiguous")
    M, K = a.shape
    N = w.shape[0]
    if out is None:
        out = torch.empty(M, N, dtype=out_dtype, device=a.device)
    _req(out.stride(1) == 1 and out.shape == (M, N), "gemm out must be [M,N] row-major")
    if residual is not None:
        _req(residual.dim() == 2 and residual.stride(1) == 1 and residual.shape[1] == N, "gemm residual must be [*,N]")
    check(lib().msam2_gemm(_p(a), a.stride(0), _p(w), w.stride(0), _p(bias), _p(colscale), _p(residual),
                                residual.stride(0) if residual is not None else 0,
                                _is_bf16(residual) if residual is not None else 0, res_mod, _p(out), out.stride(0),
                                _is_bf16(out), M, N, K, act, _stream()))
    return out


def gemm_tokens(a: torch.Tensor, w: torch.Tensor, bias: Optional[torch.Tensor] = None, *, addend: Optional[torch.Tensor] = None,
                add_cols: int = 0, act: int = ACT_NONE, residual: Optional[torch.Tensor] = None, out_dtype: torch.dtype = OP16) -> torch.Tensor:
    _req(a.dim() == 2 and a.dtype == F32 and a.stride(1) == 1 and a.shape[0] <= 32, "gemm_tokens: a must be fp32 [M<=32, K]")
    _req(w.dtype == OP16 and w.stride(1) == 1 and w.shape[1] == a.shape[1], "gemm_tokens: w must be 16-bit [N, K]")
    if addend is not None:
        _req(addend.dtype == F32 and addend.shape == a.shape and addend.stride(1) == 1 and addend.stride(0) == a.stride(0),
             "gemm_tokens: addend must match a")
    M, K = a.shape
    N = w.shape[0]
    out = torch.empty(M, N, dtype=out_dtype, device=a.device)
    if residual is not None:
        _req(residual.dtype == F32 and residual.shape == (M, N) and residual.stride(1) == 1, "gemm_tokens: residual must be fp32 [M,N]")
    check(lib().msam2_gemm_tokens(_p(a), a.stride(0), _p(addend), add_cols if addend is not None else 0, _p(w), w.stride(0), _p(bias),
                                  _p(residual), residual.stride(0) if residual is not None else 0, _p(out), out.stride(0), _is_bf16(out),
                                  M, N, K, act, _stream()))
    return out


def gemm_pool2x2(a: torch.Tensor, w: torch.Tensor, bias: Optional[torch.Tensor], B: int, H: int, W: int) -> torch.Tensor:
    _req(a.dim() == 2 and w.dim() == 2 and a.shape[1] == w.shape[1] and a.shape[0] == B * H * W, "gemm_pool2x2 shapes")
    _req(a.dtype == OP16 and w.dtype == OP16 and a.stride(1) == 1 and w.stride(1) == 1, "gemm_pool2x2 operands: 16-bit, K-contiguous")
    N, K = w.shape
    out = torch.empty(B * (H // 2) * (W // 2), N, dtype=F32, device=a.device)
    check(lib().msam2_gemm_pool2x2(_p(a), a.stride(0), _p(w), w.stride(0), _p(bias), _p(out), out.stride(0), B, H, W, N, K, _stream()))
    return out


def gemm_qkv_pool2x2(a: torch.Tensor, w: torch.Tensor, bias: Optional[torch.Tensor], B: int, H: int, W: int, q_cols: int):
    _req(a.dim() == 2 and w.dim() == 2 and a.shape[1] == w.shape[1] and a.shape[0] == B * H * W, "gemm_qkv_pool2x2 shapes")
    _req(a.dtype == OP16 and w.dtype == OP16 and a.stride(1) == 1 and w.stride(1) == 1, "gemm_qkv_pool2x2 operands: 16-bit, K-contiguous")
    N, K = w.shape
    qkv = torch.empty(B * H * W, N, dtype=OP16, device=a.device)
    q2 = torch.empty(B * (H // 2) * (W // 2), q_cols, dtype=OP16, device=a.device)
    check(lib().msam2_gemm_qkv_pool2x2(_p(a), a.stride(0), _p(w), w.stride(0), _p(bias), _p(qkv), qkv.stride(0), _p(q2), q2.stride(0),
                                       B, H, W, N, K, q_cols, _stream()))
    return qkv, q2


def gemm_rope(a: torch.Tensor, w: torch.Tensor, bias: Optional[torch.Tensor], table: Tuple[torch.Tensor, torch.Tensor], *,
              rope_cols: int, head_dim: int, rows_per_batch: int, n_rope: int, out: Optional[torch.Tensor] = None) -> torch.Tensor:
    _req(a.dim() == 2 and w.dim() == 2 and a.shape[1] == w.shape[1], f"gemm_rope shapes {tuple(a.shape)} x {tuple(w.shape)}")
    _req(a.dtype == OP16 and w.dtype == OP16 and a.stride(1) == 1 and w.stride(1) == 1, "gemm_rope operands: 16-bit, K-contiguous")
    cs, sn = table
    _req(cs.dtype == F32 and cs.is_contiguous() and sn.is_contiguous() and cs.shape == sn.shape and cs.shape[1] * 2 == head_dim,
         "gemm_rope: table must be cos/sin fp32 [n_pos, head_dim/2]")
    M, K = a.shape
    N = w.shape[0]
    if out is None:
        out = torch.empty(M, N, dtype=OP16, device=a.device)
    _req(out.dtype == OP16 and out.shape == (M, N) and out.stride(1) == 1, "gemm_rope: out must be 16-bit [M, N] row-major")
    check(lib().msam2_gemm_rope(_p(a), a.stride(0), _p(w), w.stride(0), _p(bias), _p(out), out.stride(0), M, N, K, _p(cs), _p(sn),
                                rope_cols, head_dim, rows_per_batch, n_rope, cs.shape[0], _stream()))
    return out


def layernorm(x: torch.Tensor, weight: torch.Tensor, bias: torch.Tensor, eps: float, *, act: int = ACT_NONE,
              out_dtype: torch.dtype = OP16) -> torch.Tensor:
    C = x.shape[-1]
    x2 = x.reshape(-1, C)
    _req(x2.stride(1) == 1, "layernorm input rows must be contiguous")
    y = torch.empty(x2.shape, dtype=out_dtype, device=x.device)
    check(lib().msam2_layernorm(_p(x2), _is_bf16(x2), x2.stride(0), _p(weight), _p(bias), _p(y), _is_bf16(y), y.stride(0),
                                x2.shape[0], C, eps, act, _stream()))
    return y.reshape(x.shape)


def layernorm_dual(x: torch.Tensor, weight: torch.Tensor, bias: torch.Tensor, eps: float):
    C = x.shape[-1]
    x2 = x.reshape(-1, C)
    _req(x2.dtype == F32 and x2.stride(1) == 1 and C % 4 == 0, "layernorm_dual: fp32 rows, C % 4 == 0")
    y = torch.empty(x2.shape, dtype=F32, device=x.device)
    y16 = torch.empty(x2.shape, dtype=OP16, device=x.device)
    check(lib().msam2_layernorm_dual(_p(x2), x2.stride(0), _p(weight), _p(bias), _p(y), y.stride(0), _p(y16), y16.stride(0), x2.shape[0], C, eps,
                                     _stream()))
    return y.reshape(x.shape), y16.reshape(x.shape)


def gemm_residual_layernorm_supported(N: int, K: int) -> bool:
    return bool(lib().msam2_gemm_residual_layernorm_supported(N, K))


def gemm_residual_layernorm(a: torch.Tensor, w: torch.Tensor, bias: Optional[torch.Tensor], residual: torch.Tensor, ln_w: torch.Tensor,
                            ln_b: torch.Tensor, eps: float, *, out: Optional[torch.Tensor] = None, out16: Optional[torch.Tensor] = None):
    _req(a.dim() == 2 and w.dim() == 2 and a.shape[1] == w.shape[1], f"gemm_residual_layernorm shapes {tuple(a.shape)} x {tuple(w.shape)}")
    _req(a.dtype == OP16 and w.dtype == OP16 and a.stride(1) == 1 and w.stride(1) == 1, "gemm_residual_layernorm operands: 16-bit, K-contiguous")
    M, K = a.shape
    N = w.shape[0]
    _req(gemm_residual_layernorm_supported(N, K), f"gemm_residual_layernorm: N = {N}, K = {K} is not built (N = 384, K % 64 == 0)")
    _req(residual.dtype == F32 and residual.shape == (M, N) and residual.stride(1) == 1, "gemm_residual_layernorm: residual must be fp32 [M, N]")
    _req(ln_w.dtype == F32 and ln_b.dtype == F32 and ln_w.numel() == N and ln_b.numel() == N and ln_w.is_contiguous() and ln_b.is_contiguous()
         and (bias is None or (bias.dtype == F32 and bias.numel() == N and bias.is_contiguous())),
         "gemm_residual_layernorm: bias, ln_w, ln_b are fp32 [N]")
    if out is None:
        out = torch.empty(M, N, dtype=F32, device=a.device)
    if out16 is None:
        out16 = torch.empty(M, N, dtype=OP16, device=a.device)
    _req(out.dtype == F32 and out.shape == (M, N) and out.stride(1) == 1 and out16.dtype == OP16 and out16.shape == (M, N) and out16.stride(1) == 1,
         "gemm_residual_layernorm: out is fp32 [M, N], out16 16-bit [M, N], rows contiguous")
    check(lib().msam2_gemm_residual_layernorm(_p(a), a.stride(0), _p(w), w.stride(0), _p(bias), _p(residual), residual.stride(0), _p(out),
                                              out.stride(0), _p(ln_w), _p(ln_b), float(eps), _p(out16), out16.stride(0), M, N, K, _stream()))
    return out, out16


def ln_mlp_residual_supported(dim: int) -> bool:
    return bool(lib().msam2_ln_mlp_residual_supported(dim))


def mlp_fused_permute_w2(w2: torch.Tensor) -> torch.Tensor:
    _req(w2.dim() == 2 and w2.dtype == OP16 and w2.is_contiguous() and w2.shape[1] % 32 == 0, "mlp_fused_permute_w2: 16-bit [dim, hidden]")
    out = torch.empty_like(w2)
    check(lib().msam2_mlp_fused_permute_w2(_p(w2), _p(out), w2.shape[0], w2.shape[1], _stream()))
    return out


def ln_mlp_residual(x: torch.Tensor, ln_w: torch.Tensor, ln_b: torch.Tensor, eps: float, w1: torch.Tensor, b1: torch.Tensor, w2p: torch.Tensor,
                    b2: torch.Tensor, also16: bool = False):
    T, dim = x.shape
    _req(x.dtype == F32 and x.is_contiguous() and w1.dtype == OP16 and w2p.dtype == OP16 and w1.shape == (4 * dim, dim) and w2p.shape == (dim, 4 * dim)
         and w1.is_contiguous() and w2p.is_contiguous(), "ln_mlp_residual: x fp32 [T, dim], w1 [4 dim, dim], w2p [dim, 4 dim] 16-bit contiguous")
    out = torch.empty_like(x)
    if also16:
        out16 = torch.empty(x.shape, dtype=OP16, device=x.device)
        check(lib().msam2_ln_mlp_residual_fwd_dual(_p(x), T, dim, _p(ln_w), _p(ln_b), float(eps), _p(w1), _p(b1), _p(w2p), _p(b2), _p(out), _p(out16),
                                                   _stream()))
        return out, out16
    check(lib().msam2_ln_mlp_residual_fwd(_p(x), T, dim, _p(ln_w), _p(ln_b), float(eps), _p(w1), _p(b1), _p(w2p), _p(b2), _p(out), _stream()))
    return out


def proj_ln_mlp_residual_supported(dim: int) -> bool:
    return bool(lib().msam2_proj_ln_mlp_residual_supported(dim))


def mlp_fused_permute_w1(w1: torch.Tensor) -> torch.Tensor:
    _req(w1.dim() == 2 and w1.dtype == OP16 and w1.is_contiguous() and w1.shape[1] % 32 == 0, "mlp_fused_permute_w1: 16-bit [hidden, dim]")
    out = torch.empty_like(w1)
    check(lib().msam2_mlp_fused_permute_w1(_p(w1), _p(out), w1.shape[0], w1.shape[1], _stream()))
    return out


def mlp_fused_w1_order(dim: int) -> torch.Tensor:
    i = torch.arange(dim)
    q = i & 31
    s, h, j = q >> 4, (q >> 3) & 1, q & 7
    return (i & ~31) + 16 * s + 8 * (j >> 2) + 4 * h + (j & 3)


def proj_ln_mlp_residual(o: torch.Tensor, wp: torch.Tensor, bp: torch.Tensor, res: torch.Tensor, ln_w: torch.Tensor, ln_b: torch.Tensor, eps: float,
                         w1p: torch.Tensor, b1: torch.Tensor, w2p: torch.Tensor, b2: torch.Tensor, also16: bool = False, next_ln=None):
    T, dim = res.shape
    _req(res.dtype == F32 and res.is_contiguous() and o.dtype == OP16 and o.is_contiguous() and o.shape == (T, dim) and wp.dtype == OP16
         and wp.is_contiguous() and wp.shape == (dim, dim), "proj_ln_mlp_residual: res fp32 [T, dim], o 16-bit [T, dim], wp 16-bit [dim, dim] contiguous")
    _req(w1p.dtype == OP16 and w2p.dtype == OP16 and w1p.shape == (4 * dim, dim) and w2p.shape == (dim, 4 * dim) and w1p.is_contiguous()
         and w2p.is_contiguous(), "proj_ln_mlp_residual: w1p [4 dim, dim], w2p [dim, 4 dim] 16-bit contiguous")
    out = torch.empty_like(res)
    out16 = torch.empty(res.shape, dtype=OP16, device=res.device) if also16 else None
    xn16 = torch.empty(res.shape, dtype=OP16, device=res.device) if next_ln is not None else None
    nw, nb, neps = next_ln if next_ln is not None else (None, None, 0.0)
    check(lib().msam2_proj_ln_mlp_residual_fwd(_p(o), _p(wp), _p(bp), _p(res), T, dim, _p(ln_w), _p(ln_b), float(eps), _p(w1p), _p(b1), _p(w2p), _p(b2),
                                               _p(out), _p(out16), _p(nw), _p(nb), float(neps), _p(xn16), _stream()))
    return out, out16, xn16


def _strides3(t: torch.Tensor) -> "ctypes.Array":
    return (ctypes.c_int64 * 3)(t.stride(0), t.stride(1), t.stride(2))


def attention(q: torch.Tensor, k: torch.Tensor, v: torch.Tensor, *, splits: int = 1,
              out: Optional[torch.Tensor] = None, scale: Optional[float] = None, workspace: Optional[torch.Tensor] = None,
              defer_merge: bool = False, lse: Optional[torch.Tensor] = None, dropout: Optional[tuple] = None) -> torch.Tensor:
    B, H, Lq, D = q.shape
    Lk = k.shape[2]
    for t in (q, k, v):
        _req(t.dtype == OP16 and t.stride(3) == 1, "attention tensors must be 16-bit (ops.OP16) with contiguous head dim")
    if out is None:
        out = torch.empty(B, Lq, H, D, dtype=OP16, device=q.device).permute(0, 2, 1, 3)
    if lse is not None:
        _req(lse.dtype == F32 and lse.is_contiguous() and lse.numel() == B * H * Lq and not defer_merge, "attention: lse must be fp32 [B,H,Lq]")
        splits = max(splits, 2)
    ws_bytes = lib().msam2_attention_workspace_bytes(B, H, Lq, D, splits)
    ws = workspace if workspace is not None else (torch.empty(max(ws_bytes, 1), dtype=torch.uint8, device=q.device) if splits > 1 else None)
    _req(not defer_merge or (workspace is not None and splits > 1), "defer_merge needs splits > 1 and a caller-owned workspace")
    _req(ws is None or ws.numel() * ws.element_size() >= ws_bytes, "attention workspace too small")
    sc = scale if scale is not None else 1.0 / math.sqrt(D)
    if dropout is not None and dropout[0] > 0:
        _req(lse is not None, "attention: dropout is a training feature (pass lse)")
        pd, seed, offset = dropout
        seed_dev = None
        if isinstance(seed, DeviceSeed):
            seed, seed_dev = seed.base, seed.dev
        check(lib().msam2_attention_fwd_lse_dropout(_p(q), _strides3(q), _p(k), _strides3(k), _p(v), _strides3(v), _p(out), _strides3(out),
                                                    B, H, Lq, Lk, D, sc, splits, _p(ws), ws_bytes if ws is not None else 0, _p(lse), float(pd),
                                                    int(seed) & (2 ** 64 - 1), int(offset) & (2 ** 64 - 1), _p(seed_dev), _stream()))
        return out
    if lse is not None:
        check(lib().msam2_attention_fwd_lse(_p(q), _strides3(q), _p(k), _strides3(k), _p(v), _strides3(v), _p(out), _strides3(out),
                                            B, H, Lq, Lk, D, sc, splits, _p(ws), ws_bytes if ws is not None else 0, _p(lse), _stream()))
        return out
    check(lib().msam2_attention_fwd(_p(q), _strides3(q), _p(k), _strides3(k), _p(v), _strides3(v), _p(out), _strides3(out),
                                    B, H, Lq, Lk, D, sc, -splits if defer_merge else splits, _p(ws), ws_bytes if ws is not None else 0, _stream()))
    return out


def attention_kv64(q: torch.Tensor, k: torch.Tensor, v: torch.Tensor, *, splits: int = 1, scale: Optional[float] = None,
                   workspace: Optional[torch.Tensor] = None, defer_merge: bool = False,
                   key_count: Optional[torch.Tensor] = None, out: Optional[torch.Tensor] = None) -> torch.Tensor:
    B, H, Lq, D = q.shape
    Lk = k.shape[2]
    _req(D == 256 and k.shape[3] == 256 and v.shape[3] == 64 and v.shape[2] == Lk, "attention_kv64: q/k rows of 256, v rows of 64")
    _req(key_count is None or (key_count.dtype == torch.int32 and key_count.numel() == 1 and key_count.device == q.device),
         "attention_kv64: key_count is one int32 on the tensors' device")
    for t in (q, k, v):
        _req(t.dtype == OP16 and t.stride(3) == 1, "attention tensors must be 16-bit (ops.OP16) with contiguous head dim")
    if out is None:
        out = torch.empty(B, Lq, H, 64, dtype=OP16, device=q.device).permute(0, 2, 1, 3)
    _req(out.dtype == OP16 and out.shape == (B, H, Lq, 64) and out.stride(3) == 1, "attention_kv64: out is a 16-bit [B,H,Lq,64] view")
    ws_bytes = lib().msam2_attention_workspace_bytes(B, H, Lq, 64, splits)
    ws = workspace if workspace is not None else (torch.empty(max(ws_bytes, 1), dtype=torch.uint8, device=q.device) if splits > 1 else None)
    _req(not defer_merge or (workspace is not None and splits > 1), "defer_merge needs splits > 1 and a caller-owned workspace")
    _req(ws is None or ws.numel() * ws.element_size() >= ws_bytes, "attention workspace too small")
    sc = scale if scale is not None else 1.0 / math.sqrt(D)
    if key_count is not None:
        check(lib().msam2_attention_kv64_dyn_fwd(_p(q), _strides3(q), _p(k), _strides3(k), _p(v), _strides3(v), _p(out), _strides3(out),
                                                 B, H, Lq, Lk, _p(key_count), sc, -splits if defer_merge else splits, _p(ws),
                                                 ws_bytes if ws is not None else 0, _stream()))
        return out
    check(lib().msam2_attention_kv64_fwd(_p(q), _strides3(q), _p(k), _strides3(k), _p(v), _strides3(v), _p(out), _strides3(out),
                                         B, H, Lq, Lk, sc, -splits if defer_merge else splits, _p(ws), ws_bytes if ws is not None else 0, _stream()))
    return out


def attention_effective_splits(Lk: int, splits: int) -> int:
    return int(lib().msam2_attention_effective_splits(Lk, splits))


def attention_kv64_partial(q: torch.Tensor, k: torch.Tensor, v: torch.Tensor, *, splits: int, split_begin: int, split_count: int,
                           workspace: torch.Tensor, scale: Optional[float] = None, key_count: Optional[torch.Tensor] = None) -> None:
    B, H, Lq, D = q.shape
    Lk = k.shape[2]
    for t in (q, k, v):
        _req(t.dtype == OP16 and t.stride(3) == 1, "attention tensors must be 16-bit (ops.OP16) with contiguous head dim")
    sc = scale if scale is not None else 1.0 / math.sqrt(D)
    if key_count is not None:
        _req(key_count.dtype == torch.int32 and key_count.numel() == 1, "attention_kv64_partial: key_count is one int32 on the device")
        check(lib().msam2_attention_kv64_dyn_partial(_p(q), _strides3(q), _p(k), _strides3(k), _p(v), _strides3(v), B, H, Lq, Lk, _p(key_count),
                                                     sc, splits, split_begin, split_count, _p(workspace),
                                                     workspace.numel() * workspace.element_size(), _stream()))
        return
    check(lib().msam2_attention_kv64_partial(_p(q), _strides3(q), _p(k), _strides3(k), _p(v), _strides3(v), B, H, Lq, Lk, sc, splits,
                                             split_begin, split_count, _p(workspace), workspace.numel() * workspace.element_size(), _stream()))


def attention_workspace(B: int, H: int, Lq: int, D: int, splits: int, device) -> torch.Tensor:
    return torch.empty(max(lib().msam2_attention_workspace_bytes(B, H, Lq, D, splits), 1), dtype=torch.uint8, device=device)


def attention_merge(out: torch.Tensor, Lk: int, splits: int, workspace: torch.Tensor) -> torch.Tensor:
    B, H, Lq, D = out.shape
    check(lib().msam2_attention_merge(_p(out), _strides3(out), B, H, Lq, Lk, D, splits, _p(workspace),
                                      workspace.numel() * workspace.element_size(), _stream()))
    return out


def window_attention(qkv: torch.Tensor, B: int, H: int, W: int, heads: int, ws: int, qkv_bias: torch.Tensor,
                     q_pooled: Optional[torch.Tensor] = None, scale: Optional[float] = None,
                     out: Optional[torch.Tensor] = None) -> torch.Tensor:
    dim_out = qkv.shape[1] // 3
    D = dim_out // heads
    _req(qkv.dtype == OP16 and qkv.stride(1) == 1, "qkv must be 16-bit (ops.OP16) row-major")
    if q_pooled is None:
        qt, q_ts, hq, wq, ws_q = qkv, qkv.stride(0), H, W, ws
    else:
        qt, q_ts, hq, wq, ws_q = q_pooled, q_pooled.stride(0), H // 2, W // 2, ws // 2
    o = out if out is not None else torch.empty(B * hq * wq, dim_out, dtype=OP16, device=qkv.device)
    _req(o.dtype == OP16 and o.shape == (B * hq * wq, dim_out) and o.stride(1) == 1, "window_attention: out is 16-bit [B*Hq*Wq, heads*D] rows")
    kpad = qkv_bias[dim_out:2 * dim_out]
    vpad = qkv_bias[2 * dim_out:]
    kptr = qkv.data_ptr() + dim_out * 2
    vptr = qkv.data_ptr() + 2 * dim_out * 2
    check(lib().msam2_window_attention_fwd(_p(qt), q_ts, D, hq, wq, ws_q, kptr, vptr, qkv.stride(0), D, H, W, ws, _p(kpad),
                                           _p(vpad), _p(o), o.stride(0), D, B, heads, D, scale if scale is not None else 1.0 / math.sqrt(D), _stream()))
    return o


def window_qkv_attention_supported(dim: int, dim_out: int, heads: int, ws: int, pool: bool, H: int, W: int) -> bool:
    return bool(lib().msam2_window_qkv_attention_supported(dim, dim_out, heads, ws, int(bool(pool)), H, W))


def window_qkv_attention(xn: torch.Tensor, w: torch.Tensor, bias: torch.Tensor, B: int, H: int, W: int, heads: int, ws: int,
                         pool: bool = False, scale: Optional[float] = None) -> torch.Tensor:
    _req(xn.dim() == 2 and w.dim() == 2 and xn.shape[0] == B * H * W and xn.shape[1] == w.shape[1] and w.shape[0] == 3 * heads * 96,
         "window_qkv_attention shapes")
    _req(xn.dtype == OP16 and w.dtype == OP16 and xn.is_contiguous() and w.is_contiguous(), "window_qkv_attention operands: 16-bit, contiguous")
    _req(bias.dtype == F32 and bias.is_contiguous() and bias.numel() == w.shape[0], "window_qkv_attention: bias is fp32 [3*heads*96]")
    hq, wq = (H // 2, W // 2) if pool else (H, W)
    o = torch.empty(B * hq * wq, heads * 96, dtype=OP16, device=xn.device)
    check(lib().msam2_window_qkv_attention_fwd(_p(xn), _p(w), _p(bias), _p(o), B, H, W, xn.shape[1], heads, ws, int(bool(pool)),
                                               scale if scale is not None else 1.0 / math.sqrt(96), _stream()))
    return o


def attention_small(q: torch.Tensor, k: torch.Tensor, v: torch.Tensor, heads: int, out: Optional[torch.Tensor] = None) -> torch.Tensor:
    B, Lq, C = q.shape
    Lk = k.shape[1]
    D = C // heads
    for t in (q, k, v):
        _req(t.dtype == OP16 and t.stride(2) == 1, "attention_small tensors must be 16-bit (ops.OP16), channel-contiguous")
    o = out if out is not None else torch.empty(B, Lq, C, dtype=OP16, device=q.device)
    _req(o.dtype == OP16 and o.shape == (B, Lq, C) and o.stride(2) == 1, "attention_small: out is 16-bit [B,Lq,C] with contiguous channels")
    check(lib().msam2_attention_small_fwd(_p(q), q.stride(0), q.stride(1), _p(k), k.stride(0), k.stride(1), _p(v), v.stride(0),
                                          v.stride(1), _p(o), o.stride(0), o.stride(1), B, heads, Lq, Lk, D,
                                          1.0 / math.sqrt(D), _stream()))
    return o


def add_cast(a: torch.Tensor, b: Optional[torch.Tensor] = None, alpha: float = 1.0, out_dtype: torch.dtype = OP16,
             out: Optional[torch.Tensor] = None) -> torch.Tensor:
    _req(a.dim() == 3 and (a.stride(2) == 1 or a.shape[2] == 1), "add_cast: a must be [D0,D1,C] with contiguous C")
# ... 1012 lines not shown
```

Before: 757.3 slices/s.

## Fuse mask-decoder token path into dedicated kernels with key-split few-query attention

Adds a new decoder_tokens module that fuses the two-way transformer's token-side work into a few kernels per layer: self-attention with residual and LayerNorm, the attention output projection plus MLP and LayerNorms, and the tail projection. Weights are held in registers and multiplied with MFMA. It also adds a key-split variant of the few-query attention kernel that writes per-split partial max, sum and accumulator values, which the fused kernels merge. Together these replace many small GEMM, LayerNorm and elementwise launches and spread the token-to-image attention over more blocks when B*heads is small. The cost is a lot of new specialised code tied to fixed shapes (C=256, 8 heads, 2048 hidden), with a fallback for other shapes.

Result: faster. 767.7 slices/s (median of 6 runs) (+1.4%).

```diff
diff --git a/include/msam2_hip.h b/include/msam2_hip.h
--- a/include/msam2_hip.h
+++ b/include/msam2_hip.h
@@ -70,6 +70,10 @@
 
 int msam2_attention_small_fwd(const void* q, int64_t q_bs, int64_t q_ts, const void* k, int64_t k_bs, int64_t k_ts, const void* v, int64_t v_bs, int64_t v_ts, void* o, int64_t o_bs, int64_t o_ts, int64_t B, int64_t H, int64_t Lq, int64_t Lk, int64_t D, float scale, void* stream);
 
+int msam2_attention_fewq_keysplit_splits(int64_t B, int64_t H);
+
+int msam2_attention_fewq_keysplit(const void* q, int64_t q_bs, int64_t q_ts, const void* k, int64_t k_bs, int64_t k_ts, const void* v, int64_t v_bs, int64_t v_ts, float* part, int64_t B, int64_t H, int64_t Lq, int64_t Lk, int64_t D, int64_t splits, float scale, void* stream);
+
 int msam2_window_qkv_attention_supported(int64_t dim, int64_t dim_out, int64_t heads, int64_t ws, int pool, int64_t H, int64_t W);
 
 int msam2_window_qkv_attention_fwd(const void* xn, const void* w, const float* bias, void* o, int64_t B, int64_t H, int64_t W, int64_t dim, int64_t heads, int64_t ws, int pool, float scale, void* stream);
@@ -297,6 +301,16 @@
 int msam2_volume_prep(const void* src, int src_type, int64_t T, int64_t Cin, int64_t H0, int64_t W0, int64_t S, const double* windows, const int* kx, const int* bx, int64_t ksize_x, const int* ky, const int* by, int64_t ksize_y, const float* mean3, const float* std3, uint8_t* grey_out, float* out, void* workspace, size_t workspace_bytes, void* stream);
 
 int msam2_label_resize(const void* src, int src_type, int64_t T, int64_t H0, int64_t W0, int64_t S, const int* ymap, const int* xmap, const uint32_t* keep8, uint8_t* out, void* stream);
+
+int msam2_decoder_tokens_supported(int64_t C, int64_t heads, int64_t self_dim, int64_t cross_dim, int64_t mlp_hidden, int64_t mlp_layers, int mlp_act, int64_t B, int64_t T);
+
+int msam2_decoder_tokens_self(const float* queries, const float* query_pe, int skip_first_layer_pe, const void* w_qkv, const float* b_qkv, const void* w_out, const float* b_out, const float* ln_w, const float* ln_b, float eps, const void* w_cq, const float* b_cq, float* queries_out, void* qp, int64_t B, int64_t T, int64_t C, int64_t heads, void* stream);
+
+size_t msam2_decoder_tokens_workspace_bytes(int64_t B, int64_t T);
+
+int msam2_decoder_tokens_mlp(const void* o, const float* o_partials, int64_t splits, const float* queries, const void* w_out, const float* b_out, const float* ln2_w, const float* ln2_b, float eps2, const void* w1, const float* b1, const void* w2, const float* b2, const float* ln3_w, const float* ln3_b, float eps3, const float* query_pe, const void* w_kv, const float* b_kv, const void* w_fq, const float* b_fq, float* queries_mid, float* queries_out, void* kv, void* qp_final, void* workspace, size_t workspace_bytes, int64_t B, int64_t T, int64_t C, int64_t heads, int64_t mlp_hidden, void* stream);
+
+int msam2_decoder_tokens_tail(const void* o, const float* o_partials, int64_t splits, const float* queries, const void* w_out, const float* b_out, const float* ln_w, const float* ln_b, float eps, float* queries_out, int64_t B, int64_t T, int64_t C, int64_t heads, void* stream);
 
 #ifdef __cplusplus
 }
diff --git a/medical-sam2_amd/_lib.py b/medical-sam2_amd/_lib.py
--- a/medical-sam2_amd/_lib.py
+++ b/medical-sam2_amd/_lib.py
@@ -152,6 +152,14 @@
     "msam2_volume_prep": (c_i, [c_p, c_i, c_l, c_l, c_l, c_l, c_l, ctypes.POINTER(c_d), c_p, c_p, c_l, c_p, c_p, c_l, ctypes.POINTER(c_f),
                                 ctypes.POINTER(c_f), c_p, c_p, c_p, c_z, c_p]),
     "msam2_label_resize": (c_i, [c_p, c_i, c_l, c_l, c_l, c_l, c_p, c_p, ctypes.POINTER(ctypes.c_uint32), c_p, c_p]),
+    "msam2_decoder_tokens_supported": (c_i, [c_l, c_l, c_l, c_l, c_l, c_l, c_i, c_l, c_l]),
+    "msam2_decoder_tokens_self": (c_i, [c_p, c_p, c_i, c_p, c_p, c_p, c_p, c_p, c_p, c_f, c_p, c_p, c_p, c_p, c_l, c_l, c_l, c_l, c_p]),
+    "msam2_decoder_tokens_workspace_bytes": (c_z, [c_l, c_l]),
+    "msam2_decoder_tokens_mlp": (c_i, [c_p, c_p, c_l, c_p, c_p, c_p, c_p, c_p, c_f, c_p, c_p, c_p, c_p, c_p, c_p, c_f, c_p, c_p, c_p, c_p, c_p, c_p, c_p,
+                                       c_p, c_p, c_p, c_z, c_l, c_l, c_l, c_l, c_l, c_p]),
+    "msam2_decoder_tokens_tail": (c_i, [c_p, c_p, c_l, c_p, c_p, c_p, c_p, c_p, c_f, c_p, c_l, c_l, c_l, c_l, c_p]),
+    "msam2_attention_fewq_keysplit_splits": (c_i, [c_l, c_l]),
+    "msam2_attention_fewq_keysplit": (c_i, [c_p, c_l, c_l, c_p, c_l, c_l, c_p, c_l, c_l, c_p, c_l, c_l, c_l, c_l, c_l, c_l, c_f, c_p]),
     "msam2_cc_workspace_bytes": (c_z, [c_l, c_l, c_l]),
     "msam2_cc_label": (c_i, [c_p, c_p, c_p, c_l, c_l, c_l, c_p, c_z, c_p]),
     "msam2_fill_holes_workspace_bytes": (c_z, [c_l, c_l, c_l]),
diff --git a/medical-sam2_amd/csrc/attention.hip b/medical-sam2_amd/csrc/attention.hip
--- a/medical-sam2_amd/csrc/attention.hip
+++ b/medical-sam2_amd/csrc/attention.hip
@@ -2185,16 +2185,18 @@
   }
 }
 
-__global__ __launch_bounds__(1024) void attn_fewq16_kernel(const op16* __restrict__ q, const op16* __restrict__ k, const op16* __restrict__ v,
-                                                           op16* __restrict__ o, int64_t q_bs, int64_t q_ts, int64_t k_bs, int64_t k_ts,
-                                                           int64_t v_bs, int64_t v_ts, int64_t o_bs, int64_t o_ts, int H, int Lq, int Lk,
-                                                           float scale_log2) {
-  constexpr int D = 16, RB = 64, BK = 32, NW = 16, MAXS = 8;
+template <int MAXS, bool PARTIAL>
+__device__ __forceinline__ void attn_fewq16_body(const op16* __restrict__ q, const op16* __restrict__ k, const op16* __restrict__ v,
+                                                 op16* __restrict__ o, int64_t q_bs, int64_t q_ts, int64_t k_bs, int64_t k_ts, int64_t v_bs,
+                                                 int64_t v_ts, int64_t o_bs, int64_t o_ts, int H, int Lq, int Lk, float scale_log2,
+                                                 float* __restrict__ part_out, int splits) {
+  constexpr int D = 16, RB = 64, BK = 32, NW = 16;
   __shared__ __attribute__((aligned(16))) unsigned char vt[NW][BK * RB];
   __shared__ float part[NW][32][18];
   const int tid = threadIdx.x, wave = tid >> 6, lane = tid & 63;
   const int r = lane & 31, h = lane >> 5;
-  const int b = blockIdx.x / H, head = blockIdx.x - b * H;
+  const int bh = PARTIAL ? blockIdx.x / splits : blockIdx.x, split = PARTIAL ? blockIdx.x - bh * splits : 0;
+  const int b = bh / H, head = bh - b * H;
   const op16* qb = q + (int64_t)b * q_bs + head * D;
   const op16* kb = k + (int64_t)b * k_bs + head * D;
   const op16* vb = v + (int64_t)b * v_bs + head * D;
@@ -2209,8 +2211,10 @@
     if (r < Lq) t = ld;
     qf = __builtin_bit_cast(op16x8, t);
   }
-  const int per = (Lk + NW - 1) / NW;
-  const int key_lo = wave * per, key_hi = min(Lk, key_lo + per);
+  const int per_split = PARTIAL ? (Lk + splits - 1) / splits : Lk;
+  const int k_lo = split * per_split, k_hi = min(Lk, k_lo + per_split);
+  const int per = (max(0, k_hi - k_lo) + NW - 1) / NW;
+  const int key_lo = k_lo + wave * per, key_hi = min(k_hi, key_lo + per);
   const int nsteps = max(0, (key_hi - key_lo + BK - 1) / BK);
   uint4 kfr[MAXS], vch[MAXS];
 #pragma unroll
@@ -2285,8 +2289,28 @@
       L += part[w][qi][1] * wgt;
       acc += part[w][qi][2 + d] * wgt;
     }
-    o[(int64_t)b * o_bs + (int64_t)qi * o_ts + head * D + d] = f2op(acc / L);
-  }
+    if constexpr (PARTIAL) {
+      float* po = part_out + ((int64_t)blockIdx.x * Lq + qi) * 18;
+      if (d == 0) { po[0] = M; po[1] = L; }
+      po[2 + d] = acc;
+    } else {
+      o[(int64_t)b * o_bs + (int64_t)qi * o_ts + head * D + d] = f2op(acc / L);
+    }
+  }
+}
+
+__global__ __launch_bounds__(1024) void attn_fewq16_kernel(const op16* __restrict__ q, const op16* __restrict__ k, const op16* __restrict__ v,
+                                                           op16* __restrict__ o, int64_t q_bs, int64_t q_ts, int64_t k_bs, int64_t k_ts,
+                                                           int64_t v_bs, int64_t v_ts, int64_t o_bs, int64_t o_ts, int H, int Lq, int Lk,
+                                                           float scale_log2) {
+  attn_fewq16_body<8, false>(q, k, v, o, q_bs, q_ts, k_bs, k_ts, v_bs, v_ts, o_bs, o_ts, H, Lq, Lk, scale_log2, nullptr, 1);
+}
+
+template <int MAXS>
+__global__ __launch_bounds__(1024) void attn_fewq16_part_kernel(const op16* __restrict__ q, const op16* __restrict__ k, const op16* __restrict__ v,
+                                                                int64_t q_bs, int64_t q_ts, int64_t k_bs, int64_t k_ts, int64_t v_bs, int64_t v_ts,
+                                                                int H, int Lq, int Lk, float scale_log2, float* __restrict__ part_out, int splits) {
+  attn_fewq16_body<MAXS, true>(q, k, v, nullptr, q_bs, q_ts, k_bs, k_ts, v_bs, v_ts, 0, 0, H, Lq, Lk, scale_log2, part_out, splits);
 }
 
 
@@ -2339,3 +2363,32 @@
                        q_bs, q_ts, k_bs, k_ts, v_bs, v_ts, o_bs, o_ts, (int)B, (int)H, (int)Lq, (int)Lk, sl);
   return msam2_check_launch("attention_small");
 }
+
+extern "C" int msam2_attention_fewq_keysplit_splits(int64_t B, int64_t H) {
+  if (B < 1 || H < 1) return 1;
+  return (int)max((int64_t)1, min((int64_t)8, 128 / (B * H)));
+}
+
+extern "C" int msam2_attention_fewq_keysplit(const void* q, int64_t q_bs, int64_t q_ts, const void* k, int64_t k_bs, int64_t k_ts, const void* v,
+                                             int64_t v_bs, int64_t v_ts, float* part, int64_t B, int64_t H, int64_t Lq, int64_t Lk, int64_t D,
+                                             int64_t splits, float scale, void* stream) {
+  MSAM2_REQUIRE(q && k && v && part, "attention_fewq_keysplit: null tensor");
+  MSAM2_REQUIRE(D == 16 && B > 0 && H > 0 && B * H <= 65535 && Lq >= 1 && Lq <= 32 && Lk >= 1 && Lk <= 4096 && splits >= 1 && splits <= 8,
+                "attention_fewq_keysplit: head dim 16, 1 .. 32 queries, 1 .. 4096 keys, 1 .. 8 splits (got D %lld, Lq %lld, Lk %lld, splits %lld)",
+                (long long)D, (long long)Lq, (long long)Lk, (long long)splits);
+  MSAM2_REQUIRE(q_ts % 8 == 0 && k_ts % 8 == 0 && v_ts % 8 == 0 && q_bs % 8 == 0 && k_bs % 8 == 0 && v_bs % 8 == 0 &&
+                    (((uintptr_t)q | (uintptr_t)k | (uintptr_t)v) & 15) == 0 && ((uintptr_t)part & 3) == 0,
+                "attention_fewq_keysplit: q / k / v 16-byte aligned with strides that keep it");
+  const float sl = scale * 1.4426950408889634f;
+  const int steps = cdiv(cdiv(cdiv(Lk, splits), 16), 32);
+  const dim3 grid((unsigned)(B * H * splits));
+#define FEWQ_PART(MAXS)                                                                                                                   \
+  hipLaunchKernelGGL((attn_fewq16_part_kernel<MAXS>), grid, dim3(1024), 0, (hipStream_t)stream, (const op16*)q, (const op16*)k, (const op16*)v, \
+                     q_bs, q_ts, k_bs, k_ts, v_bs, v_ts, (int)H, (int)Lq, (int)Lk, sl, part, (int)splits)
+  if (steps <= 1) FEWQ_PART(1);
+  else if (steps <= 2) FEWQ_PART(2);
+  else if (steps <= 4) FEWQ_PART(4);
+  else FEWQ_PART(8);
+#undef FEWQ_PART
+  return msam2_check_launch("attention_fewq_keysplit");
+}
diff --git a/medical-sam2_amd/csrc/decoder_tokens.hip b/medical-sam2_amd/csrc/decoder_tokens.hip
--- /dev/null
+++ b/medical-sam2_amd/csrc/decoder_tokens.hip
@@ -0,0 +1,494 @@
+#include "common.h"
+
+constexpr int DT_C = 256;
+constexpr int DT_H = 8;
+constexpr int DT_CI = 128;
+constexpr int DT_HID = 2048;
+constexpr int DT_SLICE = 128;
+constexpr int DT_NSLICE = DT_HID / DT_SLICE;
+constexpr int DT_MAXT = 16;
+constexpr int DT_MAXR = 32;
+constexpr int DT_THREADS = 512, DT_WAVES = DT_THREADS / 64;
+constexpr int DT_PART = 8192;
+
+constexpr int lds_ld(int K) { return K + 8; }
+
+template <int N, int K, int KP>
+struct TokGemm {
+  static_assert(N % 32 == 0 && K % (16 * KP) == 0 && (KP == 1 || KP * 16 * N <= DT_PART), "TokGemm shape");
+  static constexpr int KS = K / 16 / KP, NU = (N / 32) * KP, UPW = (NU + DT_WAVES - 1) / DT_WAVES, LDA = lds_ld(K);
+  op16x8 w[UPW][KS];
+  __device__ __forceinline__ static int unit(int j) { return min((int)(threadIdx.x >> 6) + j * DT_WAVES, NU - 1); }
+  __device__ __forceinline__ void load(const op16* __restrict__ W, int ldw) {
+    const int lane = threadIdx.x & 63, r = lane & 31, h = lane >> 5;
+#pragma unroll
+    for (int j = 0; j < UPW; ++j) {
+      const int u = unit(j), tile = u / KP, kp = u - tile * KP;
+      const op16* wp = W + (int64_t)(tile * 32 + r) * ldw + kp * KS * 16 + h * 8;
+#pragma unroll
+      for (int s = 0; s < KS; ++s) w[j][s] = *reinterpret_cast<const op16x8*>(wp + s * 16);
+    }
+  }
+  template <typename Epi>
+  __device__ __forceinline__ void mma(const op16* a_lo, const op16* a_hi, int split_col, float* part, Epi&& epi) const {
+    const int wave = threadIdx.x >> 6, lane = threadIdx.x & 63, r = lane & 31, h = lane >> 5;
+#pragma unroll
+    for (int j = 0; j < UPW; ++j) {
+      if (wave + j * DT_WAVES >= NU) break;
+      const int u = wave + j * DT_WAVES, tile = u / KP, kp = u - tile * KP, n0 = tile * 32;
+      const op16* ap = (n0 < split_col ? a_lo : a_hi) + (r & 15) * LDA + kp * KS * 16 + h * 8;
+      constexpr int NQ = (KP == 1 && KS % 4 == 0) ? 4 : 1;
+      f32x16 acc[NQ];
+#pragma unroll
+      for (int qd = 0; qd < NQ; ++qd)
+#pragma unroll
+        for (int e = 0; e < 16; ++e) acc[qd][e] = 0.f;
+#pragma unroll
+      for (int s = 0; s < KS; ++s)
+        acc[s / (KS / NQ)] = MSAM2_MFMA_32x32x16(*reinterpret_cast<const op16x8*>(ap + s * 16), w[j][s], acc[s / (KS / NQ)], 0, 0, 0);
+#pragma unroll
+      for (int e = 0; e < 8; ++e) {
+        const int row = (e & 3) + 8 * (e >> 2) + 4 * h;
+        float v = acc[0][e];
+#pragma unroll
+        for (int qd = 1; qd < NQ; ++qd) v += acc[qd][e];
+        if constexpr (KP == 1) epi(j, row, n0 + r, v);
+        else part[(kp * 16 + row) * N + n0 + r] = v;
+      }
+    }
+  }
+  __device__ __forceinline__ void mma(const op16* a, float* part) const { mma(a, a, 0, part, [](int, int, int, float) {}); }
+};
+
+struct LnPre {
+  f32x4 bias, w, b, res[2], extra[2];
+};
+__device__ __forceinline__ LnPre ln_preload(const float* __restrict__ bias, const float* res, const float* extra, const float* __restrict__ lnw,
+                                            const float* __restrict__ lnb, int T) {
+  const int wave = threadIdx.x >> 6, c = (threadIdx.x & 63) * 4;
+  LnPre p;
+  p.bias = *reinterpret_cast<const f32x4*>(bias + c);
+  p.w = *reinterpret_cast<const f32x4*>(lnw + c);
+  p.b = *reinterpret_cast<const f32x4*>(lnb + c);
+#pragma unroll
+  for (int j = 0; j < 2; ++j) {
+    const int row = min(wave + j * DT_WAVES, T - 1);
+    p.res[j] = res ? *reinterpret_cast<const f32x4*>(res + row * DT_C + c) : f32x4{0.f, 0.f, 0.f, 0.f};
+    p.extra[j] = extra ? *reinterpret_cast<const f32x4*>(extra + row * DT_C + c) : f32x4{0.f, 0.f, 0.f, 0.f};
+  }
+  return p;
+}
+template <int NSLAB, typename Sink>
+__device__ __forceinline__ void sum_res_ln_rows(const float* slabs, int64_t slab_stride, const LnPre& pre, float eps, int T, Sink&& sink) {
+  static_assert(DT_MAXT <= 2 * DT_WAVES, "two rows per wave");
+  const int wave = threadIdx.x >> 6, c = (threadIdx.x & 63) * 4;
+#pragma unroll
+  for (int j = 0; j < 2; ++j) {
+    const int row = wave + j * DT_WAVES;
+    if (row >= T) break;
+    f32x4 t[NSLAB];
+#pragma unroll
+    for (int s = 0; s < NSLAB; ++s) t[s] = *reinterpret_cast<const f32x4*>(slabs + s * slab_stride + row * DT_C + c);
+    f32x4 v = t[0];
+#pragma unroll
+    for (int s = 1; s < NSLAB; ++s) v += t[s];
+    v += pre.bias;
+    v += pre.res[j];
+    const float mean = wave_sum(v[0] + v[1] + v[2] + v[3]) / DT_C;
+    const f32x4 d = v - mean;
+    const float var = wave_sum(d[0] * d[0] + d[1] * d[1] + d[2] * d[2] + d[3] * d[3]) / DT_C;
+    const float rstd = 1.0f / sqrtf(var + eps);
+    sink(row, c, d * rstd * pre.w + pre.b, pre.extra[j]);
+  }
+}
+
+template <int K, typename Sink>
+__device__ __forceinline__ void proj_res_ln(const TokGemm<DT_C, K, 1>& g, const op16* a16, const LnPre& pre, float eps, int T, float* part,
+                                            Sink&& sink) {
+  g.mma(a16, a16, 0, nullptr, [&](int, int row, int col, float v) { part[row * DT_C + col] = v; });
+  __syncthreads();
+  sum_res_ln_rows<1>(part, 0, pre, eps, T, sink);
+  __syncthreads();
+}
+
+__device__ __forceinline__ op16x4 f2op4(f32x4 v) {
+  op16x4 o;
+#pragma unroll
+  for (int e = 0; e < 4; ++e) o[e] = f2op(v[e]);
+  return o;
+}
+
+template <int K>
+__device__ __forceinline__ void zero_dead_rows(op16* a, int T) {
+  for (int i = threadIdx.x; i < (DT_MAXT - T) * (K / 4); i += DT_THREADS) {
+    const int row = T + i / (K / 4), c = (i % (K / 4)) * 4;
+    *reinterpret_cast<op16x4*>(a + row * lds_ld(K) + c) = op16x4{0, 0, 0, 0};
+  }
+}
+
+template <int K>
+__device__ __forceinline__ void load_rows16(op16* a, const op16* __restrict__ src, int T) {
+  for (int i = threadIdx.x; i < T * (K / 8); i += DT_THREADS) {
+    const int row = i / (K / 8), c = (i % (K / 8)) * 8;
+    *reinterpret_cast<op16x8*>(a + row * lds_ld(K) + c) = *reinterpret_cast<const op16x8*>(src + row * K + c);
+  }
+}
+
+__device__ __forceinline__ void load_attn_rows(op16* a_o, const op16* __restrict__ o, const float* __restrict__ part, int splits, int b, int T) {
+  constexpr int D = DT_CI / DT_H, MAXSPLITS = 8;
+  if (!part) {
+    load_rows16<DT_CI>(a_o, o + (int64_t)b * T * DT_CI, T);
+    return;
+  }
+  for (int i = threadIdx.x; i < T * DT_CI; i += DT_THREADS) {
+    const int row = i / DT_CI, c = i % DT_CI, head = c / D, d = c % D;
+    const float* base = part + (((int64_t)(b * DT_H + head) * splits) * T + row) * 18;
+    float m[MAXSPLITS], l[MAXSPLITS], a[MAXSPLITS];
+#pragma unroll
+    for (int s = 0; s < MAXSPLITS; ++s) {
+      const float* ps = base + (int64_t)min(s, splits - 1) * T * 18;
+      m[s] = ps[0];
+      l[s] = ps[1];
+      a[s] = ps[2 + d];
+    }
+    float M = -INFINITY;
+#pragma unroll
+    for (int s = 0; s < MAXSPLITS; ++s) {
+      if (s >= splits) m[s] = -INFINITY;
+      M = fmaxf(M, m[s]);
+    }
+    float L = 0.f, acc = 0.f;
+#pragma unroll
+    for (int s = 0; s < MAXSPLITS; ++s) {
+      const float wgt = (m[s] == -INFINITY) ? 0.f : __builtin_amdgcn_exp2f(m[s] - M);
+      L += l[s] * wgt;
+      acc += a[s] * wgt;
+    }
+    a_o[row * lds_ld(DT_CI) + c] = f2op(acc / L);
+  }
+}
+
+template <int N, int KP>
+__device__ __forceinline__ void store_rows16(op16* out, const float* part, float b, int T) {
+  static_assert(DT_THREADS % N == 0, "one column per thread");
+  for (int i = threadIdx.x; i < T * N; i += DT_THREADS) {
+    const int row = i / N, col = i % N;
+    float v = part[row * N + col];
+#pragma unroll
+    for (int kp = 1; kp < KP; ++kp) v += part[(kp * 16 + row) * N + col];
+    out[row * N + col] = f2op(v + b);
+  }
+}
+
+struct DecSelfParams {
+  const float* x;
+  const float* pe;
+  int skip_pe;
+  const op16* wqkv; const float* bqkv;
+  const op16* wo; const float* bo;
+  const float* lnw; const float* lnb; float eps;
+  const op16* wcq; const float* bcq;
+  float* xout;
+  op16* qp;
+  int T;
+  float scale_log2;
+};
+
+__global__ __launch_bounds__(DT_THREADS) void dec_self_kernel(DecSelfParams p) {
+  constexpr int LDA = lds_ld(DT_C), LDQ = lds_ld(3 * DT_C);
+  __shared__ __attribute__((aligned(16))) op16 a_qk[DT_MAXT * LDA];
+  __shared__ __attribute__((aligned(16))) op16 a_v[DT_MAXT * LDA];
+  __shared__ __attribute__((aligned(16))) float part[DT_PART];
+  op16* const qkv = reinterpret_cast<op16*>(part);
+  static_assert(DT_MAXT * LDQ * 2 <= DT_PART * 4, "q | k | v fit the partial buffer");
+  const int T = p.T, tid = threadIdx.x;
+  const int64_t row0 = (int64_t)blockIdx.x * T;
+  const float* x = p.x + row0 * DT_C;
+  const float* pe = p.pe + row0 * DT_C;
+  TokGemm<3 * DT_C, DT_C, 1> gq;
+  gq.load(p.wqkv, DT_C);
+  float bq[gq.UPW];
+#pragma unroll
+  for (int j = 0; j < gq.UPW; ++j) bq[j] = p.bqkv[gq.unit(j) * 32 + (tid & 31)];
+  for (int i = tid; i < T * (DT_C / 4); i += DT_THREADS) {
+    const int row = i / (DT_C / 4), c = (i % (DT_C / 4)) * 4;
+    const f32x4 xv = *reinterpret_cast<const f32x4*>(x + row * DT_C + c);
+    const f32x4 pv = *reinterpret_cast<const f32x4*>(pe + row * DT_C + c);
+    *reinterpret_cast<op16x4*>(a_qk + row * LDA + c) = f2op4(p.skip_pe ? xv : xv + pv);
+    *reinterpret_cast<op16x4*>(a_v + row * LDA + c) = f2op4(xv);
+  }
+  zero_dead_rows<DT_C>(a_qk, T);
+  zero_dead_rows<DT_C>(a_v, T);
+  __syncthreads();
+  gq.mma(a_qk, a_v, 2 * DT_C, nullptr, [&](int j, int row, int col, float v) { qkv[row * LDQ + col] = f2op(v + bq[j]); });
+  TokGemm<DT_C, DT_C, 1> go;
+  go.load(p.wo, DT_C);
+  TokGemm<DT_CI, DT_C, 4> gc;
+  gc.load(p.wcq, DT_C);
+  const LnPre pre = ln_preload(p.bo, p.skip_pe ? nullptr : x, pe, p.lnw, p.lnb, T);
+  const float bc = p.bcq[tid % DT_CI];
+  __syncthreads();
+  {
+    constexpr int D = DT_C / DT_H;
+    const int l16 = tid & 15, lane = tid & 63;
+    for (int pr = tid >> 4; pr < DT_H * T; pr += DT_THREADS / 16) {
+      const int head = pr % DT_H, qi = pr / DT_H;
+      const bool live = l16 < T;
+      const op16* qp = qkv + qi * LDQ + head * D;
+      const op16* kp = qkv + (live ? l16 : 0) * LDQ + DT_C + head * D;
+      float s = 0.f;
+#pragma unroll
+      for (int d = 0; d < D; d += 8) {
+        const op16x8 tq = *reinterpret_cast<const op16x8*>(qp + d);
+        const op16x8 tk = *reinterpret_cast<const op16x8*>(kp + d);
+#pragma unroll
+        for (int e = 0; e < 8; ++e) s += (op2f(tq[e]) * p.scale_log2) * op2f(tk[e]);
+      }
+      float m = live ? s : -INFINITY;
+#pragma unroll
+      for (int off = 8; off > 0; off >>= 1) m = fmaxf(m, __shfl_xor(m, off, 64));
+      const float pk = live ? __builtin_amdgcn_exp2f(s - m) : 0.f;
+      float l = pk;
+#pragma unroll
+      for (int off = 8; off > 0; off >>= 1) l += __shfl_xor(l, off, 64);
+      const op16* vp = qkv + 2 * DT_C + head * D + 2 * l16;
+      float o0 = 0.f, o1 = 0.f;
+      for (int key = 0; key < T; ++key) {
+        const float pw = __shfl(pk, (lane & 48) | key, 64);
+        const op16x2 v2 = *reinterpret_cast<const op16x2*>(vp + key * LDQ);
+        o0 += pw * op2f(v2[0]);
+        o1 += pw * op2f(v2[1]);
+      }
+      const float inv = 1.f / l;
+      op16x2 o2;
+      o2[0] = f2op(o0 * inv);
+      o2[1] = f2op(o1 * inv);
+      *reinterpret_cast<op16x2*>(a_qk + qi * LDA + head * D + 2 * l16) = o2;
+    }
+  }
+  __syncthreads();
+  float* xout = p.xout + row0 * DT_C;
+  proj_res_ln<DT_C>(go, a_qk, pre, p.eps, T, part, [&](int row, int c, f32x4 y, f32x4 pv) {
+    *reinterpret_cast<f32x4*>(xout + row * DT_C + c) = y;
+    *reinterpret_cast<op16x4*>(a_v + row * LDA + c) = f2op4(y + pv);
+  });
+  gc.mma(a_v, part);
+  __syncthreads();
+  store_rows16<DT_CI, 4>(p.qp + row0 * DT_CI, part, bc, T);
+}
+
+struct DecMlpParams {
+  const op16* o;
+  const float* o_part;
+  int splits;
+  const float* x;
+  const op16* wo; const float* bo;
+  const float* lnw; const float* lnb; float eps;
+  const op16* w1; const float* b1;
+  const op16* w2;
+  float* x2;
+  float* ws;
+  int T, R;
+};
+
+__global__ __launch_bounds__(DT_THREADS) void dec_mlp_kernel(DecMlpParams p) {
+  constexpr int LDO = lds_ld(DT_CI), LDA = lds_ld(DT_C), LDH = lds_ld(DT_SLICE);
+  __shared__ __attribute__((aligned(16))) op16 a_o[DT_MAXT * LDO];
+  __shared__ __attribute__((aligned(16))) op16 a_y[DT_MAXT * LDA];
+  __shared__ __attribute__((aligned(16))) op16 a_h[DT_MAXT * LDH];
+  __shared__ __attribute__((aligned(16))) float part[DT_PART];
+  const int T = p.T, tid = threadIdx.x, slice = blockIdx.x;
+  const int64_t row0 = (int64_t)blockIdx.y * T;
+  TokGemm<DT_C, DT_CI, 1> go;
+  go.load(p.wo, DT_CI);
+  TokGemm<DT_SLICE, DT_C, 4> g1;
+  g1.load(p.w1 + (int64_t)slice * DT_SLICE * DT_C, DT_C);
+  TokGemm<DT_C, DT_SLICE, 1> g2;
+  g2.load(p.w2 + slice * DT_SLICE, DT_HID);
+  const LnPre pre = ln_preload(p.bo, p.x + row0 * DT_C, nullptr, p.lnw, p.lnb, T);
+  const float b1 = p.b1[slice * DT_SLICE + tid % DT_SLICE];
+  load_attn_rows(a_o, p.o, p.o_part, p.splits, blockIdx.y, T);
+  zero_dead_rows<DT_CI>(a_o, T);
+  zero_dead_rows<DT_C>(a_y, T);
+  zero_dead_rows<DT_SLICE>(a_h, T);
+  __syncthreads();
+  float* x2 = p.x2 + row0 * DT_C;
+  proj_res_ln<DT_CI>(go, a_o, pre, p.eps, T, part, [&](int row, int c, f32x4 y, f32x4) {
+    if (slice == 0) *reinterpret_cast<f32x4*>(x2 + row * DT_C + c) = y;
+    *reinterpret_cast<op16x4*>(a_y + row * LDA + c) = f2op4(y);
+  });
+  g1.mma(a_y, part);
+  __syncthreads();
+  for (int i = tid; i < T * DT_SLICE; i += DT_THREADS) {
+    const int row = i / DT_SLICE, col = i % DT_SLICE;
+    float v = part[row * DT_SLICE + col];
+#pragma unroll
+    for (int kp = 1; kp < 4; ++kp) v += part[(kp * 16 + row) * DT_SLICE + col];
+    a_h[row * LDH + col] = f2op(fmaxf(v + b1, 0.f));
+  }
+  __syncthreads();
+  float* ws = p.ws + ((int64_t)slice * p.R + row0) * DT_C;
+  g2.mma(a_h, a_h, 0, nullptr, [&](int, int row, int col, float v) {
+    if (row < T) ws[row * DT_C + col] = v;
+  });
+}
+
+struct DecKvParams {
+  const float* ws;
+  const float* b2;
+  const float* x2;
+  const float* lnw; const float* lnb; float eps;
+  const float* pe;
+  const op16* wkv; const float* bkv;
+  const op16* wfq; const float* bfq;
+  float* xout;
+  op16* kv;
+  op16* qp;
+  int T, R;
+};
+
+__global__ __launch_bounds__(DT_THREADS) void dec_kv_kernel(DecKvParams p) {
+  constexpr int LDA = lds_ld(DT_C);
+  __shared__ __attribute__((aligned(16))) op16 a_k[DT_MAXT * LDA];
+  __shared__ __attribute__((aligned(16))) op16 a_v[DT_MAXT * LDA];
+  __shared__ __attribute__((aligned(16))) float part[DT_PART];
+  const int T = p.T, tid = threadIdx.x;
+  const int64_t row0 = (int64_t)blockIdx.x * T;
+  const bool last = p.wfq != nullptr;
+  TokGemm<DT_C, DT_C, 1> gk;
+  gk.load(p.wkv, DT_C);
+  TokGemm<DT_CI, DT_C, 4> gf;
+  gf.load(last ? p.wfq : p.wkv, DT_C);
+  const LnPre pre = ln_preload(p.b2, p.x2 + row0 * DT_C, p.pe + row0 * DT_C, p.lnw, p.lnb, T);
+  const float bk = p.bkv[tid % DT_C], bf = last ? p.bfq[tid % DT_CI] : 0.f;
+  zero_dead_rows<DT_C>(a_k, T);
+  zero_dead_rows<DT_C>(a_v, T);
+  float* xout = p.xout + row0 * DT_C;
+  sum_res_ln_rows<DT_NSLICE>(p.ws + row0 * DT_C, (int64_t)p.R * DT_C, pre, p.eps, T, [&](int row, int c, f32x4 y, f32x4 pv) {
+    *reinterpret_cast<f32x4*>(xout + row * DT_C + c) = y;
+    *reinterpret_cast<op16x4*>(a_k + row * LDA + c) = f2op4(y + pv);
+    *reinterpret_cast<op16x4*>(a_v + row * LDA + c) = f2op4(y);
+  });
+  __syncthreads();
+  gk.mma(a_k, a_v, DT_CI, nullptr, [&](int, int row, int col, float v) { part[row * DT_C + col] = v; });
+  __syncthreads();
+  store_rows16<DT_C, 1>(p.kv + row0 * DT_C, part, bk, T);
+  if (!last) return;
+  __syncthreads();
+  gf.mma(a_k, part);
+  __syncthreads();
+  store_rows16<DT_CI, 4>(p.qp + row0 * DT_CI, part, bf, T);
+}
+
+struct DecTailParams {
+  const op16* o;
+  const float* o_part;
+  int splits;
+  const float* x;
+  const op16* wo; const float* bo;
+  const float* lnw; const float* lnb; float eps;
+  float* xout;
+  int T;
+};
+
+__global__ __launch_bounds__(DT_THREADS) void dec_tail_kernel(DecTailParams p) {
+  constexpr int LDO = lds_ld(DT_CI);
+  __shared__ __attribute__((aligned(16))) op16 a_o[DT_MAXT * LDO];
+  __shared__ __attribute__((aligned(16))) float part[DT_PART];
+  const int T = p.T;
+  const int64_t row0 = (int64_t)blockIdx.x * T;
+  TokGemm<DT_C, DT_CI, 1> go;
+  go.load(p.wo, DT_CI);
+  const LnPre pre = ln_preload(p.bo, p.x + row0 * DT_C, nullptr, p.lnw, p.lnb, T);
+  load_attn_rows(a_o, p.o, p.o_part, p.splits, blockIdx.x, T);
+  zero_dead_rows<DT_CI>(a_o, T);
+  __syncthreads();
+  float* xout = p.xout + row0 * DT_C;
+  proj_res_ln<DT_CI>(go, a_o, pre, p.eps, T, part, [&](int row, int c, f32x4 y, f32x4) { *reinterpret_cast<f32x4*>(xout + row * DT_C + c) = y; });
+}
+
+static bool config_ok(int64_t C, int64_t heads, int64_t self_dim, int64_t cross_dim, int64_t mlp_hidden, int64_t mlp_layers, int mlp_act) {
+  return C == DT_C && heads == DT_H && self_dim == DT_C && cross_dim == DT_CI && mlp_hidden == DT_HID && mlp_layers == 2 && mlp_act == 2;
+}
+static bool rows_ok(int64_t B, int64_t T) { return B >= 1 && T >= 1 && T <= DT_MAXT && B * T <= DT_MAXR; }
+
+#define DEC_REQUIRE_ROWS(entry, B, T)                                                                                             \
+  MSAM2_REQUIRE(rows_ok(B, T), entry ": B = %lld images of T = %lld tokens (T <= %d, B * T <= %d rows)", (long long)(B), (long long)(T), \
+                DT_MAXT, DT_MAXR)
+
+#define DEC_REQUIRE_ATTN(entry, o, o_partials, splits)                                                                                     \
+  MSAM2_REQUIRE(((o) != nullptr) != ((o_partials) != nullptr) && (!(o_partials) || ((splits) >= 1 && (splits) <= 8)) &&                     \
+                    ((uintptr_t)(o_partials) & 3) == 0,                                                                                    \
+                entry ": exactly one of o and o_partials (with 1 .. 8 splits, got %lld)", (long long)(splits))
+
+extern "C" int msam2_decoder_tokens_supported(int64_t C, int64_t heads, int64_t self_dim, int64_t cross_dim, int64_t mlp_hidden,
+                                              int64_t mlp_layers, int mlp_act, int64_t B, int64_t T) {
+  return config_ok(C, heads, self_dim, cross_dim, mlp_hidden, mlp_layers, mlp_act) && rows_ok(B, T) ? 1 : 0;
+}
+
+extern "C" int msam2_decoder_tokens_self(const float* queries, const float* query_pe, int skip_first_layer_pe, const void* w_qkv,
+                                         const float* b_qkv, const void* w_out, const float* b_out, const float* ln_w, const float* ln_b,
+                                         float eps, const void* w_cq, const float* b_cq, float* queries_out, void* qp, int64_t B, int64_t T,
+                                         int64_t C, int64_t heads, void* stream) {
+  MSAM2_REQUIRE(queries && query_pe && w_qkv && b_qkv && w_out && b_out && ln_w && ln_b && w_cq && b_cq && queries_out && qp,
+                "decoder_tokens_self: null tensor");
+  MSAM2_REQUIRE(config_ok(C, heads, DT_C, DT_CI, DT_HID, 2, 2), "decoder_tokens_self: built for C = 256 and 8 heads (got %lld, %lld)",
+                (long long)C, (long long)heads);
+  DEC_REQUIRE_ROWS("decoder_tokens_self", B, T);
+  MSAM2_REQUIRE(vec_ok(4, 4, queries, query_pe, b_qkv, b_out, ln_w, ln_b, b_cq, queries_out) && vec_ok(8, 2, w_qkv, w_out, w_cq, qp),
+                "decoder_tokens_self: tensors must be 16-byte aligned");
+  DecSelfParams p = {queries, query_pe, skip_first_layer_pe != 0, (const op16*)w_qkv, b_qkv, (const op16*)w_out, b_out, ln_w, ln_b, eps,
+                     (const op16*)w_cq, b_cq, queries_out, (op16*)qp, (int)T, (float)(1.0 / sqrt((double)(DT_C / DT_H))) * 1.4426950408889634f};
+  hipLaunchKernelGGL(dec_self_kernel, dim3((unsigned)B), dim3(DT_THREADS), 0, (hipStream_t)stream, p);
+  return msam2_check_launch("decoder_tokens_self");
+}
+
+extern "C" size_t msam2_decoder_tokens_workspace_bytes(int64_t B, int64_t T) {
+  return rows_ok(B, T) ? (size_t)DT_NSLICE * B * T * DT_C * sizeof(float) : 0;
+}
+
+extern "C" int msam2_decoder_tokens_mlp(const void* o, const float* o_partials, int64_t splits, const float* queries, const void* w_out, const float* b_out, const float* ln2_w,
+                                        const float* ln2_b, float eps2, const void* w1, const float* b1, const void* w2, const float* b2,
+                                        const float* ln3_w, const float* ln3_b, float eps3, const float* query_pe, const void* w_kv,
+                                        const float* b_kv, const void* w_fq, const float* b_fq, float* queries_mid, float* queries_out,
+                                        void* kv, void* qp_final, void* workspace, size_t workspace_bytes, int64_t B, int64_t T, int64_t C,
+                                        int64_t heads, int64_t mlp_hidden, void* stream) {
+  MSAM2_REQUIRE(queries && w_out && b_out && ln2_w && ln2_b && w1 && b1 && w2 && b2 && ln3_w && ln3_b && query_pe && w_kv && b_kv &&
+                    queries_mid && queries_out && kv && workspace,
+                "decoder_tokens_mlp: null tensor");
+  DEC_REQUIRE_ATTN("decoder_tokens_mlp", o, o_partials, splits);
+  MSAM2_REQUIRE((w_fq != nullptr) == (b_fq != nullptr) && (w_fq != nullptr) == (qp_final != nullptr),
+                "decoder_tokens_mlp: w_fq, b_fq and qp_final come together (last block) or not at all");
+  MSAM2_REQUIRE(config_ok(C, heads, DT_C, DT_CI, mlp_hidden, 2, 2),
+                "decoder_tokens_mlp: built for C = 256, 8 heads and 2048 hidden units (got %lld, %lld, %lld)", (long long)C, (long long)heads,
+                (long long)mlp_hidden);
+  DEC_REQUIRE_ROWS("decoder_tokens_mlp", B, T);
+  MSAM2_REQUIRE(workspace_bytes >= msam2_decoder_tokens_workspace_bytes(B, T), "decoder_tokens_mlp: workspace of %zu bytes, %zu needed",
+                workspace_bytes, msam2_decoder_tokens_workspace_bytes(B, T));
+  MSAM2_REQUIRE(vec_ok(4, 4, queries, b_out, ln2_w, ln2_b, b1, b2, ln3_w, ln3_b, query_pe, b_kv, b_fq, queries_mid, queries_out, workspace) &&
+                    vec_ok(8, 2, o, w_out, w1, w2, w_kv, w_fq, kv, qp_final),
+                "decoder_tokens_mlp: tensors must be 16-byte aligned");
+  float* ws = (float*)workspace;
+  DecMlpParams pm = {(const op16*)o, o_partials, (int)splits, queries, (const op16*)w_out, b_out, ln2_w, ln2_b, eps2, (const op16*)w1, b1, (const op16*)w2,
+                     queries_mid, ws, (int)T, (int)(B * T)};
+  hipLaunchKernelGGL(dec_mlp_kernel, dim3(DT_NSLICE, (unsigned)B), dim3(DT_THREADS), 0, (hipStream_t)stream, pm);
+  DecKvParams pk = {ws, b2, queries_mid, ln3_w, ln3_b, eps3, query_pe, (const op16*)w_kv, b_kv, (const op16*)w_fq, b_fq, queries_out,
+                    (op16*)kv, (op16*)qp_final, (int)T, (int)(B * T)};
+  hipLaunchKernelGGL(dec_kv_kernel, dim3((unsigned)B), dim3(DT_THREADS), 0, (hipStream_t)stream, pk);
+  return msam2_check_launch("decoder_tokens_mlp");
+}
+
+extern "C" int msam2_decoder_tokens_tail(const void* o, const float* o_partials, int64_t splits, const float* queries, const void* w_out, const float* b_out, const float* ln_w,
+                                         const float* ln_b, float eps, float* queries_out, int64_t B, int64_t T, int64_t C, int64_t heads,
+                                         void* stream) {
+  MSAM2_REQUIRE(queries && w_out && b_out && ln_w && ln_b && queries_out, "decoder_tokens_tail: null tensor");
+  DEC_REQUIRE_ATTN("decoder_tokens_tail", o, o_partials, splits);
+  MSAM2_REQUIRE(config_ok(C, heads, DT_C, DT_CI, DT_HID, 2, 2), "decoder_tokens_tail: built for C = 256 and 8 heads (got %lld, %lld)",
+                (long long)C, (long long)heads);
+  DEC_REQUIRE_ROWS("decoder_tokens_tail", B, T);
+  MSAM2_REQUIRE(vec_ok(4, 4, queries, b_out, ln_w, ln_b, queries_out) && vec_ok(8, 2, o, w_out),
+                "decoder_tokens_tail: tensors must be 16-byte aligned");
+  DecTailParams p = {(const op16*)o, o_partials, (int)splits, queries, (const op16*)w_out, b_out, ln_w, ln_b, eps, queries_out, (int)T};
+  hipLaunchKernelGGL(dec_tail_kernel, dim3((unsigned)B), dim3(DT_THREADS), 0, (hipStream_t)stream, p);
+  return msam2_check_launch("decoder_tokens_tail");
+}
diff --git a/medical-sam2_amd/modeling/sam_heads.py b/medical-sam2_amd/modeling/sam_heads.py
--- a/medical-sam2_amd/modeling/sam_heads.py
+++ b/medical-sam2_amd/modeling/sam_heads.py
@@ -1,5 +1,6 @@
 from __future__ import annotations
 
+import os
 from typing import List, Optional, Tuple, Type
 
 import torch
@@ -125,6 +126,14 @@
     return ops.gemm(keys_b, W, b, residual=R, res_mod=L)
 
 
+def _tokens_to_image_attention(attn, qp, k_img, v_img):
+    B, Lq, C = qp.shape
+    L = k_img.shape[1]
+    if (os.environ.get("MSAM2_NO_FEWQ_KEYSPLIT") != "1" and C // attn.num_heads == 16 and Lq <= 32 and 1024 <= L <= 4096):
+        return ops.attention_fewq_keysplit(qp, k_img, v_img, attn.num_heads)
+    return attn.core(qp, k_img, v_img)
+
+
 class TwoWayAttentionBlock(nn.Module):
 
     def __init__(self, embedding_dim: int, num_heads: int, mlp_dim: int = 2048, activation: Type[nn.Module] = nn.ReLU,
@@ -145,10 +154,21 @@
         n = getattr(self, name)
         return ops.layernorm(x, v_f32(self._wc, name + "w", n.weight), v_f32(self._wc, name + "b", n.bias), n.eps, out_dtype=F32)
 
-    def run(self, queries, keys, query_pe, key_pe, B, T, L, keys_b=None):
+    def tokens_fused(self, B: int, T: int, fused_tokens: bool) -> bool:
+        if not fused_tokens or os.environ.get("MSAM2_NO_FUSED_DEC_TOKENS") == "1":
+            return False
+        sa, ca, ia, mlp = self.self_attn, self.cross_attn_token_to_image, self.cross_attn_image_to_token, self.mlp
+        if not (sa.num_heads == ca.num_heads == ia.num_heads and ca.internal_dim == ia.internal_dim):
+            return False
+        return ops.decoder_tokens_supported(sa.embedding_dim, sa.num_heads, sa.internal_dim, ca.internal_dim, mlp.layers[0].out_features,
+                                            mlp.num_layers, mlp._act_code, B, T)
+
+    def run(self, queries, keys, query_pe, key_pe, B, T, L, keys_b=None, fused_tokens=False, final_q=None):
         C = queries.shape[1]
         q3 = lambda t, n: t.view(B, n, -1)
         sa, ca, ia, wc = self.self_attn, self.cross_attn_token_to_image, self.cross_attn_image_to_token, self._wc
+        if self.tokens_fused(B, T, fused_tokens):
+            return self._run_tokens_fused(queries, keys, query_pe, key_pe, B, T, L, keys_b, final_q)
         fused = B * T <= 32 and C % 32 == 0 and sa.internal_dim % 32 == 0 and ia.internal_dim % 32 == 0
         if fused:
             Ci = sa.internal_dim
@@ -192,14 +212,42 @@
             o = ia.core(q3(q_img, L), q3(ia.proj("k", qb), T), q3(ia.proj("v", to_bf16(queries)), T))
         n4 = self.norm4
         keys, keys16 = ops.layernorm_dual(ia.out(o, keys), v_f32(wc, "norm4w", n4.weight), v_f32(wc, "norm4b", n4.bias), n4.eps)
-        return queries, keys, keys16
+        return queries, keys, keys16, None
+
+    def _run_tokens_fused(self, queries, keys, query_pe, key_pe, B, T, L, keys_b, final_q):
+        q3 = lambda t, n: t.view(B, n, -1)
+        sa, ca, ia, wc = self.self_attn, self.cross_attn_token_to_image, self.cross_attn_image_to_token, self._wc
+        ln = lambda name: (v_f32(wc, name + "w", getattr(self, name).weight), v_f32(wc, name + "b", getattr(self, name).bias), getattr(self, name).eps)
+        H = sa.num_heads
+        queries, qp = ops.decoder_tokens_self(
+            queries, query_pe, self.skip_first_layer_pe, w_bf16(wc, "sqkv", sa.q_proj.weight, sa.k_proj.weight, sa.v_proj.weight),
+            v_f32(wc, "sqkvb", sa.q_proj.bias, sa.k_proj.bias, sa.v_proj.bias), w_bf16(sa._wc, "ow", sa.out_proj.weight),
+            v_f32(sa._wc, "ob", sa.out_proj.bias), *ln("norm1"), w_bf16(wc, "cqw", ca.q_proj.weight), v_f32(wc, "cqb", ca.q_proj.bias), B, T, H)
+        if keys_b is None:
+            keys_b = to_bf16(keys)
+        Cc, Ci2 = ca.internal_dim, ia.internal_dim
+        kvq = _image_side_projections(wc, "ikvq", keys_b, key_pe, L, [ca.k_proj, ca.v_proj, ia.q_proj], [True, False, True])
+        k_img, v_img, q_img = kvq[:, :Cc], kvq[:, Cc:2 * Cc], kvq[:, 2 * Cc:2 * Cc + Ci2]
+        o = _tokens_to_image_attention(ca, q3(qp, T), q3(k_img, L), q3(v_img, L))
+        l1, l2 = self.mlp.layers
+        fq_w, fq_b = final_q if final_q is not None else (None, None)
+        queries, kv, qp_final = ops.decoder_tokens_mlp(
+            o, queries, w_bf16(ca._wc, "ow", ca.out_proj.weight), v_f32(ca._wc, "ob", ca.out_proj.bias), *ln("norm2"),
+            w_bf16(wc, "m1w", l1.weight), v_f32(wc, "m1b", l1.bias), w_bf16(wc, "m2w", l2.weight), v_f32(wc, "m2b", l2.bias), *ln("norm3"),
+            query_pe, w_bf16(wc, "ikv", ia.k_proj.weight, ia.v_proj.weight), v_f32(wc, "ikvb", ia.k_proj.bias, ia.v_proj.bias), B, T, H,
+            w_fq=fq_w, b_fq=fq_b)
+        kv = kv.view(B, T, 2 * Ci2)
+        o = ia.core(q3(q_img, L), kv[:, :, :Ci2], kv[:, :, Ci2:])
+        n4 = self.norm4
+        keys, keys16 = ops.layernorm_dual(ia.out(o, keys), v_f32(wc, "norm4w", n4.weight), v_f32(wc, "norm4b", n4.bias), n4.eps)
+        return queries, keys, keys16, qp_final
 
     def forward(self, queries, keys, query_pe, key_pe):
         B, T, C = queries.shape
         L = keys.shape[1]
         assert key_pe.shape[0] == 1 or B == 1, "key_pe is the batch-shared dense position encoding"
-        q, k, _ = self.run(queries.to(F32).reshape(B * T, C).contiguous(), keys.to(F32).reshape(B * L, C).contiguous(),
-                           query_pe.to(F32).reshape(B * T, C).contiguous(), key_pe.to(F32).reshape(-1, C)[:L].contiguous(), B, T, L)
+        q, k, _, _ = self.run(queries.to(F32).reshape(B * T, C).contiguous(), keys.to(F32).reshape(B * L, C).contiguous(),
+                              query_pe.to(F32).reshape(B * T, C).contiguous(), key_pe.to(F32).reshape(-1, C)[:L].contiguous(), B, T, L)
         return q.view(B, T, C), k.view(B, L, C)
 
 
@@ -217,26 +265,41 @@
         self.norm_final_attn = nn.LayerNorm(embedding_dim)
         self._wc = WeightCache()
 
-    def run(self, keys, key_pe, tokens, B, T, L):
+    def run(self, keys, key_pe, tokens, B, T, L, fused_tokens=False):
         C = tokens.shape[1]
         queries, qpe = tokens, tokens
         keys16 = None
-        for layer in self.layers:
-            queries, keys, keys16 = layer.run(queries, keys, qpe, key_pe, B, T, L, keys16)
+        fa = self.final_attn_token_to_image
+        fused = [layer.tokens_fused(B, T, fused_tokens) for layer in self.layers]
+        fused_tail = (bool(fused) and fused[-1] and fa.num_heads == self.layers[-1].self_attn.num_heads
+                      and fa.internal_dim == self.layers[-1].cross_attn_token_to_image.internal_dim)
+        qp = None
+        for i, layer in enumerate(self.layers):
+            if fused[i]:
+                final_q = None
+                if fused_tail and i == len(self.layers) - 1:
+                    final_q = (w_bf16(self._wc, "fqw", fa.q_proj.weight), v_f32(self._wc, "fqb", fa.q_proj.bias))
+                queries, keys, keys16, qp = layer._run_tokens_fused(queries, keys, qpe, key_pe, B, T, L, keys16, final_q)
+            else:
+                queries, keys, keys16, qp = layer.run(queries, keys, qpe, key_pe, B, T, L, keys16)
         if keys16 is None:
             keys16 = to_bf16(keys)
         self._keys16 = keys16
-        fa = self.final_attn_token_to_image
         kv_img = _image_side_projections(self._wc, "fkv", keys16, key_pe, L, [fa.k_proj, fa.v_proj], [True, False])
         Cf = fa.internal_dim
         q3 = lambda t, n: t.view(B, n, -1)
+        n = self.norm_final_attn
+        if fused_tail:
+            o = _tokens_to_image_attention(fa, q3(qp, T), q3(kv_img[:, :Cf], L), q3(kv_img[:, Cf:], L))
+            queries = ops.decoder_tokens_tail(o, queries, w_bf16(fa._wc, "ow", fa.out_proj.weight), v_f32(fa._wc, "ob", fa.out_proj.bias),
+                                              v_f32(self._wc, "nw", n.weight), v_f32(self._wc, "nb", n.bias), n.eps, B, T, fa.num_heads)
+            return queries, keys
         if B * T <= 32 and fa.internal_dim % 32 == 0:
             qp = ops.gemm_tokens(queries, w_bf16(self._wc, "fqw", fa.q_proj.weight), v_f32(self._wc, "fqb", fa.q_proj.bias), addend=qpe,
                                  add_cols=fa.internal_dim)
         else:
             qp = fa.proj("q", ops.add_cast(queries.view(1, B * T, C), qpe.view(1, B * T, C), 1.0, OP16)[0])
         o = fa.core(q3(qp, T), q3(kv_img[:, :Cf], L), q3(kv_img[:, Cf:], L))
-        n = self.norm_final_attn
         queries = ops.layernorm(fa.out(o, queries), v_f32(self._wc, "nw", n.weight), v_f32(self._wc, "nb", n.bias), n.eps, out_dtype=F32)
         return queries, keys
 
@@ -288,14 +351,14 @@
         return ops.gemm(tokens_bf16, w_bf16(self._wc, f"cs{which}w", c.weight), v_f32(self._wc, f"cs{which}b", c.bias), out_dtype=out_dtype)
 
     def predict_masks_tokens(self, src_tokens: torch.Tensor, pe_tokens: torch.Tensor, sparse: torch.Tensor, feat_s0: torch.Tensor,
-                             feat_s1: torch.Tensor, B: int, h: int, w: int, shared_skips: bool = False):
+                             feat_s1: torch.Tensor, B: int, h: int, w: int, shared_skips: bool = False, fused_tokens: bool = False):
         wc = self._wc
         C = self.transformer_dim
         out_tok = wc.get("otok", [self.obj_score_token.weight, self.iou_token.weight, self.mask_tokens.weight],
                          lambda: torch.cat([self.obj_score_token.weight, self.iou_token.weight, self.mask_tokens.weight], 0).detach().float())
         T = out_tok.shape[0] + sparse.shape[1]
         tokens = torch.cat([out_tok.unsqueeze(0).expand(B, -1, -1), sparse], 1)
-        hs, keys = self.transformer.run(src_tokens, pe_tokens, tokens.view(B * T, C), B, T, h * w)
+        hs, keys = self.transformer.run(src_tokens, pe_tokens, tokens.view(B * T, C), B, T, h * w, fused_tokens=fused_tokens)
         hs = hs.view(B, T, C)
         up = self.output_upscaling
         dc1_w = wc.get("dc1", [up[0].weight], lambda: up[0].weight.detach().permute(2, 3, 1, 0).reshape(-1, C).to(OP16).contiguous())
@@ -381,7 +444,7 @@
             pe = tokens_of(image_pe.to(F32))[: h * w]
             f0, f1 = high_res_features
             skip = lambda f: tokens_of(f) if (f.dtype == F32 and f.shape[1] in (32, 64)) else to_bf16(tokens_of(f))
-            return self.predict_masks_tokens(src, pe, sparse_prompt_embeddings.to(F32), skip(f0), skip(f1), B, h, w, shared_skips=True)
+            return self.predict_masks_tokens(src, pe, sparse_prompt_embeddings.to(F32), skip(f0), skip(f1), B, h, w, shared_skips=True, fused_tokens=True)
         if image_embeddings.shape[0] != n_sets:
             if cell_nums is not None:
                 cn = torch.as_tensor(cell_nums, device=image_embeddings.device).reshape(-1).long()
@@ -418,7 +481,7 @@
         pe = tokens_of(image_pe.to(F32))[: h * w]
         f0, f1 = high_res_features
         skip = lambda f: tokens_of(f) if (f.dtype == F32 and f.shape[1] in (32, 64)) else to_bf16(tokens_of(f))
-        return self.predict_masks_tokens(src, pe, sparse_prompt_embeddings.to(F32), skip(f0), skip(f1), B, h, w)
+        return self.predict_masks_tokens(src, pe, sparse_prompt_embeddings.to(F32), skip(f0), skip(f1), B, h, w, fused_tokens=True)
 
     def forward(self, image_embeddings, image_pe, sparse_prompt_embeddings, dense_prompt_embeddings, multimask_output: bool,
                 repeat_image: bool, cell_nums=None, high_res_features: Optional[List[torch.Tensor]] = None):
diff --git a/medical-sam2_amd/ops.py b/medical-sam2_amd/ops.py
--- a/medical-sam2_amd/ops.py
+++ b/medical-sam2_amd/ops.py
@@ -70,6 +70,101 @@
     check(lib().msam2_gemm_tokens(_p(a), a.stride(0), _p(addend), add_cols if addend is not None else 0, _p(w), w.stride(0), _p(bias),
                                   _p(residual), residual.stride(0) if residual is not None else 0, _p(out), out.stride(0), _is_bf16(out),
                                   M, N, K, act, _stream()))
+    return out
+
+
+def decoder_tokens_supported(C: int, heads: int, self_dim: int, cross_dim: int, mlp_hidden: int, mlp_layers: int, mlp_act: int,
+                             B: int, T: int) -> bool:
+    return bool(lib().msam2_decoder_tokens_supported(C, heads, self_dim, cross_dim, mlp_hidden, mlp_layers, mlp_act, B, T))
+
+
+def _dec_rows(name: str, t: torch.Tensor, rows: int, cols: int, dtype: torch.dtype):
+    _req(t.dtype == dtype and t.shape == (rows, cols) and t.is_contiguous(), f"{name} must be a contiguous {dtype} [{rows}, {cols}]")
+
+
+def attention_fewq_keysplit(q: torch.Tensor, k: torch.Tensor, v: torch.Tensor, heads: int, splits: Optional[int] = None):
+    B, Lq, C = q.shape
+    Lk = k.shape[1]
+    for t in (q, k, v):
+        _req(t.dtype == OP16 and t.stride(2) == 1, "attention_fewq_keysplit tensors must be 16-bit (ops.OP16), channel-contiguous")
+    if splits is None:
+        splits = int(lib().msam2_attention_fewq_keysplit_splits(B, heads))
+    part = torch.empty(B * heads * splits, Lq, 18, dtype=F32, device=q.device)
+    check(lib().msam2_attention_fewq_keysplit(_p(q), q.stride(0), q.stride(1), _p(k), k.stride(0), k.stride(1), _p(v), v.stride(0), v.stride(1),
+                                              _p(part), B, heads, Lq, Lk, C // heads, splits, 1.0 / math.sqrt(C // heads), _stream()))
+    return part, splits
+
+
+def _dec_attn_out(name: str, o, R: int, T: int, C: int, heads: int):
+    if isinstance(o, tuple):
+        part, splits = o
+        _req(part.dtype == F32 and part.is_contiguous() and part.shape == ((R // T) * heads * splits, T, 18), f"{name}: partials must be fp32 [B*heads*splits, T, 18]")
+        return None, part, splits
+    _dec_rows(f"{name}: o", o, R, C // 2, OP16)
+    return o, None, 0
+
+
+def decoder_tokens_self(queries: torch.Tensor, query_pe: torch.Tensor, skip_first_layer_pe: bool, w_qkv: torch.Tensor, b_qkv: torch.Tensor,
+                        w_out: torch.Tensor, b_out: torch.Tensor, ln_w: torch.Tensor, ln_b: torch.Tensor, eps: float, w_cq: torch.Tensor,
+                        b_cq: torch.Tensor, B: int, T: int, heads: int):
+    R, C = B * T, queries.shape[1]
+    _dec_rows("decoder_tokens_self: queries", queries, R, C, F32)
+    _dec_rows("decoder_tokens_self: query_pe", query_pe, R, C, F32)
+    _dec_rows("decoder_tokens_self: w_qkv", w_qkv, 3 * C, C, OP16)
+    _dec_rows("decoder_tokens_self: w_out", w_out, C, C, OP16)
+    _dec_rows("decoder_tokens_self: w_cq", w_cq, C // 2, C, OP16)
+    for v, n in ((b_qkv, 3 * C), (b_out, C), (ln_w, C), (ln_b, C), (b_cq, C // 2)):
+        _req(v.dtype == F32 and v.is_contiguous() and v.numel() == n, "decoder_tokens_self: biases and LayerNorm vectors are fp32, contiguous")
+    out = torch.empty(R, C, dtype=F32, device=queries.device)
+    qp = torch.empty(R, C // 2, dtype=OP16, device=queries.device)
+    check(lib().msam2_decoder_tokens_self(_p(queries), _p(query_pe), int(bool(skip_first_layer_pe)), _p(w_qkv), _p(b_qkv), _p(w_out), _p(b_out),
+                                          _p(ln_w), _p(ln_b), eps, _p(w_cq), _p(b_cq), _p(out), _p(qp), B, T, C, heads, _stream()))
+    return out, qp
+
+
+def decoder_tokens_mlp(o, queries: torch.Tensor, w_out: torch.Tensor, b_out: torch.Tensor, ln2_w: torch.Tensor, ln2_b: torch.Tensor,
+                       eps2: float, w1: torch.Tensor, b1: torch.Tensor, w2: torch.Tensor, b2: torch.Tensor, ln3_w: torch.Tensor,
+                       ln3_b: torch.Tensor, eps3: float, query_pe: torch.Tensor, w_kv: torch.Tensor, b_kv: torch.Tensor, B: int, T: int,
+                       heads: int, w_fq: Optional[torch.Tensor] = None, b_fq: Optional[torch.Tensor] = None):
+    R, C = B * T, queries.shape[1]
+    hidden = w1.shape[0]
+    o, o_part, splits = _dec_attn_out("decoder_tokens_mlp", o, R, T, C, heads)
+    _dec_rows("decoder_tokens_mlp: queries", queries, R, C, F32)
+    _dec_rows("decoder_tokens_mlp: query_pe", query_pe, R, C, F32)
+    _dec_rows("decoder_tokens_mlp: w_out", w_out, C, C // 2, OP16)
+    _dec_rows("decoder_tokens_mlp: w1", w1, hidden, C, OP16)
+    _dec_rows("decoder_tokens_mlp: w2", w2, C, hidden, OP16)
+    _dec_rows("decoder_tokens_mlp: w_kv", w_kv, C, C, OP16)
+    vecs = [(b_out, C), (ln2_w, C), (ln2_b, C), (b1, hidden), (b2, C), (ln3_w, C), (ln3_b, C), (b_kv, C)]
+    _req((w_fq is None) == (b_fq is None), "decoder_tokens_mlp: w_fq and b_fq come together")
+    if w_fq is not None:
+        _dec_rows("decoder_tokens_mlp: w_fq", w_fq, C // 2, C, OP16)
+        vecs.append((b_fq, C // 2))
+    for v, n in vecs:
+        _req(v.dtype == F32 and v.is_contiguous() and v.numel() == n, "decoder_tokens_mlp: biases and LayerNorm vectors are fp32, contiguous")
+    dev = queries.device
+    mid = torch.empty(R, C, dtype=F32, device=dev)
+    out = torch.empty(R, C, dtype=F32, device=dev)
+    kv = torch.empty(R, C, dtype=OP16, device=dev)
+    qp = torch.empty(R, C // 2, dtype=OP16, device=dev) if w_fq is not None else None
+    nbytes = max(int(lib().msam2_decoder_tokens_workspace_bytes(B, T)), 16)
+    ws = torch.empty(nbytes, dtype=torch.uint8, device=dev)
+    check(lib().msam2_decoder_tokens_mlp(_p(o), _p(o_part), splits, _p(queries), _p(w_out), _p(b_out), _p(ln2_w), _p(ln2_b), eps2, _p(w1), _p(b1), _p(w2), _p(b2),
+                                         _p(ln3_w), _p(ln3_b), eps3, _p(query_pe), _p(w_kv), _p(b_kv), _p(w_fq), _p(b_fq), _p(mid), _p(out),
+                                         _p(kv), _p(qp), _p(ws), nbytes, B, T, C, heads, hidden, _stream()))
+    return out, kv, qp
+
+
+def decoder_tokens_tail(o, queries: torch.Tensor, w_out: torch.Tensor, b_out: torch.Tensor, ln_w: torch.Tensor, ln_b: torch.Tensor,
+                        eps: float, B: int, T: int, heads: int) -> torch.Tensor:
+    R, C = B * T, queries.shape[1]
+    o, o_part, splits = _dec_attn_out("decoder_tokens_tail", o, R, T, C, heads)
+    _dec_rows("decoder_tokens_tail: queries", queries, R, C, F32)
+    _dec_rows("decoder_tokens_tail: w_out", w_out, C, C // 2, OP16)
+    for v in (b_out, ln_w, ln_b):
+        _req(v.dtype == F32 and v.is_contiguous() and v.numel() == C, "decoder_tokens_tail: bias and LayerNorm vectors are fp32 [C], contiguous")
+    out = torch.empty(R, C, dtype=F32, device=queries.device)
+    check(lib().msam2_decoder_tokens_tail(_p(o), _p(o_part), splits, _p(queries), _p(w_out), _p(b_out), _p(ln_w), _p(ln_b), eps, _p(out), B, T, C, heads, _stream()))
     return out
 
 
```
